# Aster32/GAN-DANet

Hardware: AMD Instinct MI355X
Metric: train samples/sec (G+D step) on 256x256 tiles (higher is better)
Workload: dtype bf16; 1 GPU; full G+D train step, 8ch 256x256 -> 1024x1024 tiles, batch 32/GPU (global 32), perceptual=on, SSIM evaluated, AdamW x2; survey_config=3, per_gpu_batch=32, global_batch=32, tile=256, parallelism=dp1

## Files before the change

### gan-danet_amd/_lib.py

```python
from __future__ import annotations

import ctypes as C
import os

HERE = os.path.dirname(os.path.abspath(__file__))
LIB_PATH = os.path.join(HERE, "lib", "libgandanet_hip.so")

PREC_FP32, PREC_BF16, PREC_X3 = 0, 1, 2
PAM_BWD_K64_ATOMIC, PAM_BWD_K64_PARTS, PAM_BWD_K32_PARTS, PAM_BWD_TWO_KERNEL = 0, 1, 2, 3
ACT_NONE, ACT_RELU, ACT_LEAKY02, ACT_SIGMOID = 0, 1, 2, 3

c_fp = C.c_void_p


class ConvDesc(C.Structure):
    _fields_ = [
        ("B", C.c_int), ("M", C.c_int), ("Mstore", C.c_int), ("Ck", C.c_int), ("ks", C.c_int),
        ("stride", C.c_int), ("pad", C.c_int), ("transposed", C.c_int),
        ("Hi", C.c_int), ("Wi", C.c_int), ("Ho", C.c_int), ("Wo", C.c_int),
        ("a", c_fp), ("a_bs", C.c_long), ("a_sm", C.c_long), ("a_sc", C.c_long), ("a_st", C.c_long),
        ("x", c_fp), ("x_bs", C.c_long),
        ("in_scale", c_fp), ("in_shift", c_fp), ("in_relu", C.c_int),
        ("y", c_fp), ("y_bs", C.c_long),
        ("out_layout", C.c_int), ("out_bf16", C.c_int), ("ldo", C.c_int),
        ("alpha", c_fp), ("bias", c_fp), ("res", c_fp), ("res_bs", C.c_long),
        ("act", C.c_int), ("accumulate", C.c_int), ("precision", C.c_int),
        ("sub_oy", C.c_int), ("sub_ox", C.c_int), ("sub_step", C.c_int),
    ]


class GemmNTDesc(C.Structure):
    _fields_ = [
        ("B", C.c_int), ("M", C.c_int), ("N", C.c_int), ("kseg", C.c_int), ("klen", C.c_long),
        ("a", c_fp), ("a_bs", C.c_long), ("a_ss", C.c_long), ("lda", C.c_long),
        ("bm", c_fp), ("b_bs", C.c_long), ("b_ss", C.c_long), ("ldb", C.c_long),
        ("im2col", C.c_int), ("ks", C.c_int), ("stride", C.c_int), ("pad", C.c_int),
        ("Hi", C.c_int), ("Wi", C.c_int), ("Ho", C.c_int), ("Wo", C.c_int),
        ("in_scale", c_fp), ("in_shift", c_fp), ("in_relu", C.c_int),
        ("c", c_fp), ("c_bs", C.c_long), ("ldc", C.c_long),
        ("alpha", c_fp), ("bias", c_fp),
        ("accumulate", C.c_int), ("splits", C.c_int), ("precision", C.c_int),
    ]


_i, _l, _f, _p, _sz = C.c_int, C.c_long, C.c_float, c_fp, C.c_size_t

SIGNATURES = {
    "gd_version": (_i, []),
    "gd_set_deterministic": (None, [_i]),
    "gd_get_deterministic": (_i, []),
    "gd_set_det_reduce": (_i, [_i]),
    "gd_get_det_reduce": (_i, []),
    "gd_last_error": (_i, [C.c_char_p, _i]),
    "gd_sizeof_conv_desc": (_i, []),
    "gd_sizeof_gemm_nt_desc": (_i, []),
    "gd_conv2d": (_i, [C.POINTER(ConvDesc), _p]),
    "gd_gemm_nt": (_i, [C.POINTER(GemmNTDesc), _p]),
    "gd_gemm_nt_ws": (_i, [C.POINTER(GemmNTDesc), _p, _p, _sz]),
    "gd_gemm_nt_plan": (_i, [C.POINTER(GemmNTDesc), _sz, C.POINTER(_i), C.POINTER(_sz)]),
    "gd_conv3x3_ws_bytes": (_sz, [_i, _i]),
    "gd_conv3x3_eligible": (_i, [C.POINTER(ConvDesc)]),
    "gd_conv3x3": (_i, [C.POINTER(ConvDesc), _p, _sz, _p]),
    "gd_conv3x3_wgrad": (_i, [_p, _l, _p, _p, _l, _p, _i, _p, _p, _i, _i, _i, _i, _i, _i, _i, _i, _p, _p]),
    "gd_conv3x3_wgrad_ws": (_i, [_p, _l, _p, _p, _l, _p, _i, _p, _p, _i, _i, _i, _i, _i, _i, _i, _i, _p, _p, _p, _sz]),
    "gd_conv3x3_wgrad_plan": (_i, [_i, _i, _i, _i, _i, _i, _sz, C.POINTER(_i), C.POINTER(_sz)]),
    "gd_pack_16_split": (_i, [_p, _l, _i, _i, _i, _p, _p, _i, _p, _l, _i, _l, _i, _i, _p, _l, _i, _l, _i, _i, _p]),
    "gd_pack_16_split_masked": (_i, [_p, _l, _i, _i, _i, _p, _p, _i, _p, _l, _i, _l, _i, _i, _p, _l, _i, _l, _i, _i, _p, _l, _p]),
    "gd_split3_weights": (_i, [_p, _l, _l, _l, _p, _p]),
    "gd_bn_stats_ws_floats": (_sz, [_i, _i, _l]),
    "gd_bn_stats": (_i, [_p, _l, _i, _i, _l, _f, _f, _p, _p, _p, _p, _p, _p]),
    "gd_bn_fold": (_i, [_p, _p, _p, _p, _i, _p, _p, _p]),
    "gd_bn_fold_eval": (_i, [_p, _p, _p, _p, _f, _i, _p, _p, _p, _p]),
    "gd_affine_act": (_i, [_p, _l, _p, _p, _i, _i, _l, _i, _p, _l, _p]),
    "gd_bn_act_bwd": (_i, [_p, _l, _p, _l, _p, _p, _p, _p, _p, _i, _i, _l, _i, _i, _p, _p, _p, _l, _i, _p, _p]),
    "gd_bn_stats_local": (_i, [_p, _l, _i, _i, _l, _p, _p, _p]),
    "gd_bn_stats_merge": (_i, [_p, _i, _i, _f, _f, _p, _p, _p, _p, _p]),
    "gd_bn_act_bwd_dx": (_i, [_p, _l, _p, _l, _p, _p, _p, _p, _p, _p, _f, _i, _i, _l, _i, _p, _l, _i, _p]),
    "gd_bicubic_fwd": (_i, [_p, _i, _i, _i, _p, _i, _i, _f, _f, _p]),
    "gd_bicubic_bwd": (_i, [_p, _i, _i, _i, _p, _i, _i, _f, _f, _p]),
    "gd_bilinear_fwd": (_i, [_p, _i, _i, _i, _p, _i, _i, _i, _p, _p]),
    "gd_bilinear_bwd": (_i, [_p, _i, _i, _i, _p, _i, _i, _p]),
    "gd_maxpool2_fwd": (_i, [_p, _i, _i, _i, _p, _p]),
    "gd_maxpool2_bwd": (_i, [_p, _p, _i, _i, _i, _p, _p]),
    "gd_act_fwd": (_i, [_p, _p, _l, _i, _p]),
    "gd_act_bwd": (_i, [_p, _p, _p, _l, _i, _p]),
    "gd_axpby": (_i, [_p, _f, _p, _f, _l, _p]),
    "gd_scale_dev": (_i, [_p, _p, _p, _l, _i, _p]),
    "gd_copy_rows": (_i, [_p, _l, _l, _p, _l, _l, _i, _i, _i, _p]),
    "gd_channel_sum": (_i, [_p, _l, _i, _i, _l, _p, _i, _p, _p]),
    "gd_copy_slab": (_i, [_p, _l, _p, _l, _i, _l, _i, _p]),
    "gd_softmax_rows": (_i, [_p, _p, _l, _i, _f, _p]),
    "gd_softmax_rows_bwd": (_i, [_p, _p, _p, _l, _i, _f, _p]),
    "gd_dot": (_i, [_p, _p, _l, _p, _i, _p, _p]),
    "gd_transpose": (_i, [_p, _p, _i, _i, _i, _p]),
    "gd_add_transpose": (_i, [_p, _p, _i, _i, _p]),
    "gd_bce_logits": (_i, [_p, _l, _f, _p, _p, _p, _p]),
    "gd_bce_logits_target": (_i, [_p, _p, _l, _p, _p, _p, _p, _p]),
    "gd_leaky_fwd": (_i, [_p, _p, _l, _f, _p]),
    "gd_leaky_bwd": (_i, [_p, _p, _p, _l, _f, _p]),
    "gd_mse": (_i, [_p, _p, _l, _p, _p, _p, _p]),
    "gd_l1": (_i, [_p, _p, _l, _p, _p, _p, _p]),
    "gd_tv": (_i, [_p, _i, _i, _i, _i, _f, _p, _p, _p, _p]),
    "gd_ssim": (_i, [_p, _p, _i, _i, _i, _i, _p, _p, _p]),
    "gd_ssim_samples": (_i, [_p, _p, _i, _i, _i, _i, _i, _p, _p, _p]),
    "gd_ssim_bwd": (_i, [_p, _p, _p, _i, _i, _i, _i, _i, _p, _p, _p, _p]),
    "gd_adamw": (_i, [_p, _p, _p, _p, _l, _i, _f, _f, _f, _f, _f, _f, _p]),
    "gd_pam_flash_fwd": (_i, [_p, _p, _p, _i, _i, _i, _i, _i, _i, _i, _p, _p, _l, _p, _l, _p, _p, _p, _p]),
    "gd_pam_key_sqnorm_max": (_i, [_p, _i, _i, _i, _i, _p, _p]),
    "gd_pam_fwd_shift_ws_bytes": (_sz, [_i, _i]),
    "gd_pam_flash_fwd_shift": (_i, [_p, _p, _p, _i, _i, _i, _i, _i, _i, _p, _p, _l, _p, _l, _p, _p, _i, _p, _sz, _p]),
    "gd_pam_flash_bwd": (_i, [_p, _p, _p, _p, _p, _p, _p, _i, _i, _i, _i, _i, _i, _p, _p, _p, _l, _p, _sz, _p]),
    "gd_pam_bwd_scratch_bytes": (_sz, [_i, _i]),
    "gd_pam_wide_fwd": (_i, [_p, _p, _p, _i, _i, _i, _i, _i, _i, _i, _p, _p, _l, _p, _l, _p, _p, _p]),
    "gd_pam_wide_scratch_bytes": (_sz, [_i, _i, _i]),
    "gd_pam_wide_bwd": (_i, [_p, _p, _p, _p, _p, _p, _p, _i, _i, _i, _i, _i, _i, _i, _p, _p, _p, _p, _sz, _p]),
    "gd_pam_f32_fwd": (_i, [_p, _l, _p, _l, _p, _l, _i, _i, _i, _i, _i, _p, _p, _l, _p, _l, _p, _p, _p]),
    "gd_pam_f32_bwd": (_i, [_p, _l, _p, _l, _p, _l, _p, _l, _p, _p, _i, _i, _i, _i, _i, _p, _p, _p, _p]),
    "gd_chan_dot": (_i, [_p, _l, _p, _l, _i, _i, _i, _p, _p, _p, _p]),
    "gd_pam_f16_scale": (_i, [_p, _l, _i, _i, _i, _p, _p, _p, _p, _p]),
    "gd_conv3x3_nhwc_pack": (_i, [_p, _i, _i, _i, _p, _sz, _p]),
    "gd_conv3x3_nhwc": (_i, [_p, _p, _p, _p, _p, _p, _i, _i, _i, _i, _i, _i, _i, _p]),
    "gd_conv3x3_nhwc_f32out": (_i, [_p, _p, _p, _p, _l, _i, _i, _i, _i, _i, _i, _p]),
    "gd_disc_stem_fwd": (_i, [_p, _i, _i, _i, _i, _p, _p, _i, _f, _p, _i, _p]),
    "gd_disc_stem_wgrad": (_i, [_p, _p, _i, _i, _i, _i, _i, _p, _p, _i, _p]),
    "gd_disc_stem_wgrad_ws": (_i, [_p, _p, _i, _i, _i, _i, _i, _p, _p, _i, _p, _p, _sz]),
    "gd_disc_stem_dgrad": (_i, [_p, _i, _i, _i, _i, _p, _i, _p, _i, _p]),
    "gd_conv3x3_nhwc_s2": (_i, [_p, _p, _p, _p, _i, _i, _i, _i, _i, _i, _f, _i, _p]),
    "gd_conv3x3_nhwc_s2_dgrad": (_i, [_p, _p, _p, _f, _p, _i, _i, _i, _i, _i, _i, _p]),
    "gd_nhwc_flatten_fwd": (_i, [_p, _i, _i, _i, _p, _i, _p]),
    "gd_nhwc_flatten_bwd": (_i, [_p, _p, _f, _i, _i, _i, _p, _i, _p]),
    "gd_nhwc_to_nchw16": (_i, [_p, _i, _i, _i, _p, _p, _i, _p]),
    "gd_nhwc_to_nchw16_ws": (_i, [_p, _i, _i, _i, _p, _p, _i, _p, _p, _sz]),
    "gd_nhwc_stem_fwd": (_i, [_p, _i, _i, _i, _i, _p, _p, _i, _i, _p, _i, _p]),
    "gd_nhwc_stem_bwd": (_i, [_p, _i, _i, _i, _i, _p, _i, _p, _i, _p]),
    "gd_nhwc_maxpool2_fwd": (_i, [_p, _i, _i, _i, _i, _p, _i, _p]),
    "gd_nhwc_maxpool2_bwd": (_i, [_p, _p, _i, _i, _i, _i, _i, _p, _i, _p]),
    "gd_nhwc_l1": (_i, [_p, _p, _l, _p, _i, _p, _i, _p]),
    "gd_nhwc_l1_grad": (_i, [_p, _p, _l, _p, _i, _p, _i, _p]),
    "gd_shift_sum9_fwd": (_i, [_p, _p, _p, _i, _i, _i, _p]),
    "gd_shift_sum9_bwd": (_i, [_p, _p, _i, _i, _i, _p]),
    "gd_combine_inputs": (_i, [_p, _i, _i, _i, _f, _p, _i, _i, _i, _f, _p, _i, _i, _i, _p]),
    "gd_hist_match_ws_bytes": (_sz, [_l, _l]),
    "gd_hist_match": (_i, [_p, _p, _i, _l, _l, C.c_double, _p, _p, _sz, _p]),
    "gd_blend_region": (_i, [_p, _p, _p, _i, _i, _i, _i, _i, _i, _i, _p]),
    "gd_augment_d4": (_i, [_p, _p, _i, _i, _i, _i, _p, _p, _f, _p]),
    "gd_bcast_mul": (_i, [_p, _p, _p, _i, _i, _l, _i, _p]),
    "gd_row_dot": (_i, [_p, _p, _p, _l, _l, _p]),
    "gd_chan_maxmean_fwd": (_i, [_p, _p, _p, _i, _i, _l, _p]),
    "gd_chan_maxmean_bwd": (_i, [_p, _p, _p, _i, _i, _l, _p]),
    "gd_comm_unique_id": (_i, [C.c_char_p]),
    "gd_comm_init": (_i, [_i, _i, C.c_char_p]),
    "gd_comm_world": (_i, []),
    "gd_allreduce": (_i, [_p, _sz, _i, _p]),
    "gd_reduce_scatter": (_i, [_p, _p, _sz, _i, _p]),
    "gd_allgather": (_i, [_p, _p, _sz, _i, _p]),
    "gd_comm_destroy": (_i, []),
    "gd_pack_bf16": (_i, [_p, _l, _i, _i, _i, _p, _f, _p, _i, _i, _p, _i, _i, _i, _i, _p]),
    "gd_pack_16": (_i, [_p, _l, _i, _i, _i, _p, _f, _p, _i, _i, _p, _i, _i, _i, _i, _i, _p]),
    "gd_pack_16_affine": (_i, [_p, _l, _i, _i, _i, _p, _p, _i, _p, _i, _i, _p, _i, _i, _i, _p]),
}

_lib = None


class GandanetError(RuntimeError):
    pass


def load() -> C.CDLL:
    global _lib
    if _lib is not None:
        return _lib
    if not os.path.exists(LIB_PATH):
        raise GandanetError(
            f"{LIB_PATH} is missing: the HIP extension is not built (run __graft_entry__.build()). "
            "There is no CPU fallback.")
    lib = C.CDLL(LIB_PATH)
    for name, (res, args) in SIGNATURES.items():
        fn = getattr(lib, name)
        fn.restype = res
        fn.argtypes = args
    if lib.gd_sizeof_conv_desc() != C.sizeof(ConvDesc) or lib.gd_sizeof_gemm_nt_desc() != C.sizeof(GemmNTDesc):
        raise GandanetError("descriptor struct layout differs between _lib.py and libgandanet_hip.so")
    _lib = lib
    return lib


def last_error() -> str:
    buf = C.create_string_buffer(512)
    load().gd_last_error(buf, 512)
    return buf.value.decode()


def check(rc: int, what: str = "") -> None:
    if rc != 0:
        raise GandanetError(f"{what or 'gandanet call'} failed (rc={rc}): {last_error()}")
```

### gan-danet_amd/csrc/gemm_conv.hip

```cpp
#include <stdlib.h>

#include <type_traits>

#include "common.h"
#include "tile_mma.h"
#include "../../include/gandanet.h"

namespace {

using gd::TILE_BK;
using gd::TILE_BN;
constexpr int BN = TILE_BN;
constexpr int BK = TILE_BK;

template <int BM, int MODE>
__global__ __launch_bounds__(256) void conv_nn_kernel(const gd_conv_desc d) {
    constexpr bool BF16 = MODE != gd::MODE_F32;
    constexpr bool X3 = MODE == gd::MODE_X3;
    using P = gd::TilePol<MODE>;
    using elem = typename P::elem;
    constexpr int LD = P::LD;
    constexpr int WAVES_N = gd::TileGeom<BM>::WAVES_N;
    constexpr int TM = gd::TileGeom<BM>::TM;
    constexpr int TN = gd::TileGeom<BM>::TN;
    constexpr int KPT_A = BM / 8;
    constexpr int KPT_B = 16;

    __shared__ __attribute__((aligned(16))) elem As[P::PLANES * BM * LD];
    __shared__ __attribute__((aligned(16))) elem Bs[P::PLANES * BN * LD];

    const int tid = threadIdx.x;
    const int lane = tid & 63, wave = tid >> 6;
    const int r = lane & 31, h = lane >> 5;
    const int wm = wave / WAVES_N, wn = wave % WAVES_N;
    const int b = blockIdx.z;
    const int m0 = blockIdx.y * BM;
    const int n0 = blockIdx.x * BN;
    const long HiWi = (long)d.Hi * d.Wi;
    const int HoWo = d.Ho * d.Wo;

    const int am = tid % BM;
    const int akg = tid / BM;
    const bool a_row_ok = (m0 + am) < d.M;
    const float* a_row = d.a + (long)b * d.a_bs + (long)(m0 + am) * d.a_sm;

    const int bn = tid & (BN - 1);
    const int bkh = tid >> 7;
    const int sstep = d.sub_step > 1 ? d.sub_step : 1;
    const int Ws = (d.Wo - d.sub_ox + sstep - 1) / sstep, Hs = (d.Ho - d.sub_oy + sstep - 1) / sstep;
    const int HsWs = Hs * Ws;
    const int p = n0 + bn;
    const bool p_ok = p < HsWs;
    const int pa = p_ok ? p / Ws : 0;
    const int oy = d.sub_oy + pa * sstep;
    const int ox = d.sub_ox + (p_ok ? p - pa * Ws : 0) * sstep;
    const float* x_img = d.x + (long)b * d.x_bs;

    f32x16_t acc[TM][TN];
#pragma unroll
    for (int i = 0; i < TM; ++i)
#pragma unroll
        for (int j = 0; j < TN; ++j)
#pragma unroll
            for (int e = 0; e < 16; ++e) acc[i][j][e] = 0.f;

    const int ktiles_per_tap = (d.Ck + BK - 1) / BK;
    const int ntaps = d.ks * d.ks;
    const int T = ntaps * ktiles_per_tap;

    float ra[KPT_A];
    float rb[KPT_B];

    auto load_tile = [&](int t) {
        const int tap = t / ktiles_per_tap;
        const int c0 = (t - tap * ktiles_per_tap) * BK;
        const int kh = tap / d.ks, kw = tap - kh * d.ks;
        {
            const float* ap = a_row + (long)tap * d.a_st;
#pragma unroll
            for (int i = 0; i < KPT_A; ++i) {
                const int c = c0 + akg * KPT_A + i;
                ra[i] = (a_row_ok && c < d.Ck) ? ap[(long)c * d.a_sc] : 0.f;
            }
        }
        {
            int iy, ix;
            bool ok = p_ok;
            if (!d.transposed) {
                iy = oy * d.stride - d.pad + kh;
                ix = ox * d.stride - d.pad + kw;
            } else {
                const int ty = oy + d.pad - kh, tx = ox + d.pad - kw;
                ok = ok && ty >= 0 && tx >= 0 && (ty % d.stride == 0) && (tx % d.stride == 0);
                iy = ty / d.stride;
                ix = tx / d.stride;
            }
            ok = ok && iy >= 0 && iy < d.Hi && ix >= 0 && ix < d.Wi;
            const float* xp = x_img + (long)iy * d.Wi + ix;
#pragma unroll
            for (int i = 0; i < KPT_B; ++i) {
                const int c = c0 + bkh * KPT_B + i;
                float v = 0.f;
                if (ok && c < d.Ck) {
                    v = xp[(long)c * HiWi];
                    if (d.in_scale) {
                        v = fmaf(v, d.in_scale[c], d.in_shift[c]);
                        if (d.in_relu) v = fmaxf(v, 0.f);
                    }
                }
                rb[i] = v;
            }
        }
    };

    auto put_row = [&](elem* row, int plane_stride, const float* v, auto nc) {
        constexpr int n = decltype(nc)::value;
        if constexpr (BF16 && n % 8 == 0) {
#pragma unroll
            for (int i = 0; i < n; i += 8) {
                uint4 whi, wlo;
                if constexpr (X3) {
                    gd_split_bf2(v[i + 0], v[i + 1], whi.x, wlo.x);
                    gd_split_bf2(v[i + 2], v[i + 3], whi.y, wlo.y);
                    gd_split_bf2(v[i + 4], v[i + 5], whi.z, wlo.z);
                    gd_split_bf2(v[i + 6], v[i + 7], whi.w, wlo.w);
                    *reinterpret_cast<uint4*>(row + plane_stride + i) = wlo;
                } else {
                    whi.x = gd_pack_bf2(v[i + 0], v[i + 1]);
                    whi.y = gd_pack_bf2(v[i + 2], v[i + 3]);
                    whi.z = gd_pack_bf2(v[i + 4], v[i + 5]);
                    whi.w = gd_pack_bf2(v[i + 6], v[i + 7]);
                }
                *reinterpret_cast<uint4*>(row + i) = whi;
            }
        } else if constexpr (BF16) {
#pragma unroll
            for (int i = 0; i < n; i += 4) {
                uint2 whi, wlo;
                if constexpr (X3) {
                    gd_split_bf2(v[i + 0], v[i + 1], whi.x, wlo.x);
                    gd_split_bf2(v[i + 2], v[i + 3], whi.y, wlo.y);
                    *reinterpret_cast<uint2*>(row + plane_stride + i) = wlo;
                } else {
                    whi.x = gd_pack_bf2(v[i + 0], v[i + 1]);
                    whi.y = gd_pack_bf2(v[i + 2], v[i + 3]);
                }
                *reinterpret_cast<uint2*>(row + i) = whi;
            }
        } else {
#pragma unroll
            for (int i = 0; i < n; ++i) row[i] = v[i];
        }
    };
    auto store_tile = [&]() {
        put_row(As + am * LD + akg * KPT_A, BM * LD, ra, std::integral_constant<int, KPT_A>{});
        put_row(Bs + bn * LD + bkh * KPT_B, BN * LD, rb, std::integral_constant<int, KPT_B>{});
    };

    auto compute_tile = [&]() { gd::tile_mma<BM, MODE>(As, Bs, wm, wn, r, h, acc); };

    auto tile_live = [&](int t) -> bool {
        if (!d.transposed || sstep == 1) return true;
        const int tap = t / ktiles_per_tap;
        const int kh = tap / d.ks, kw = tap - kh * d.ks;
        return ((d.sub_oy + d.pad - kh) % d.stride == 0) && ((d.sub_ox + d.pad - kw) % d.stride == 0);
    };
    auto next_live = [&](int t) -> int {
        while (t < T && !tile_live(t)) ++t;
        return t;
    };
    int t = next_live(0);
    if (t < T) {
        load_tile(t);
        store_tile();
    }
    __syncthreads();
    while (t < T) {
        const int tn = next_live(t + 1);
        if (tn < T) load_tile(tn);
        compute_tile();
        __syncthreads();
        if (tn < T) {
            store_tile();
            __syncthreads();
        }
        t = tn;
    }

    const float alpha = d.alpha ? *d.alpha : 1.f;
#pragma unroll
    for (int i = 0; i < TM; ++i) {
#pragma unroll
        for (int j = 0; j < TN; ++j) {
            const int ps = n0 + wn * TN * 32 + j * 32 + r;
            if (ps >= HsWs) continue;
            const int qa = ps / Ws;
            const int pn = (d.sub_oy + qa * sstep) * d.Wo + d.sub_ox + (ps - qa * Ws) * sstep;
            float rsv[16], oldv[16];
#pragma unroll
            for (int e = 0; e < 16; ++e) {
                const int m = m0 + wm * TM * 32 + i * 32 + gd::acc_row(e, h);
                rsv[e] = (d.res && m < d.M) ? d.res[(long)b * d.res_bs + (long)m * HoWo + pn] : 0.f;
            }
#pragma unroll
            for (int e = 0; e < 16; ++e) {
                const int m = m0 + wm * TM * 32 + i * 32 + gd::acc_row(e, h);
                const long idx = d.out_layout == 0 ? (long)b * d.y_bs + (long)m * HoWo + pn
                                                   : (long)b * d.y_bs + (long)pn * d.ldo + m;
                oldv[e] = (d.accumulate && !d.out_bf16 && m < d.Mstore) ? reinterpret_cast<const float*>(d.y)[idx] : 0.f;
            }
#pragma unroll
            for (int e = 0; e < 16; ++e) {
                const int m = m0 + wm * TM * 32 + i * 32 + gd::acc_row(e, h);
                if (m >= d.Mstore) continue;
                float v = acc[i][j][e] * alpha;
                if (m < d.M) {
                    if (d.bias) v += d.bias[m];
                    v += rsv[e];
                }
                if (d.act == GD_ACT_RELU) v = fmaxf(v, 0.f);
                else if (d.act == GD_ACT_LEAKY02) v = v >= 0.f ? v : 0.2f * v;
                const long idx = d.out_layout == 0 ? (long)b * d.y_bs + (long)m * HoWo + pn
                                                   : (long)b * d.y_bs + (long)pn * d.ldo + m;
                if (d.out_bf16) reinterpret_cast<unsigned short*>(d.y)[idx] = gd_f2bf(v);
                else reinterpret_cast<float*>(d.y)[idx] = v + oldv[e];
            }
        }
    }
}

typedef short s16x4_t __attribute__((ext_vector_type(4)));
constexpr int XLD = BN + 32;

template <int BM, int NS, bool X3 = false>
__global__ __launch_bounds__(256) void conv1x1_tr_kernel(const gd_conv_desc d) {
    constexpr int LDA = BK + 8;
    constexpr int PL = X3 ? 2 : 1, A_PL = BM * LDA, X_PL = NS * BK * XLD;
    constexpr int WAVES_N = gd::TileGeom<BM>::WAVES_N;
    constexpr int TM = gd::TileGeom<BM>::TM;
    constexpr int TN = gd::TileGeom<BM>::TN;
    constexpr int KPT_A = BM / 8;
    __shared__ __attribute__((aligned(16))) unsigned short As[PL * A_PL];
    __shared__ __attribute__((aligned(16))) unsigned short Xs[PL * X_PL];

    const int tid = threadIdx.x, lane = tid & 63, wave = tid >> 6;
    const int r = lane & 31, h = lane >> 5;
    const int wm = wave / WAVES_N, wn = wave % WAVES_N;
    const int b = blockIdx.z, m0 = blockIdx.y * BM, n0 = blockIdx.x * (BN * NS);
    const int HW = d.Ho * d.Wo;

    const int am = tid % BM, akg = tid / BM;
    const bool a_row_ok = (m0 + am) < d.M;
    const float* a_row = d.a + (long)b * d.a_bs + (long)(m0 + am) * d.a_sm;

    const int xq = tid & 31, xr0 = tid >> 5;
    const float* x_img = d.x + (long)b * d.x_bs;

    f32x16_t acc[NS][TM][TN];
#pragma unroll
    for (int sb = 0; sb < NS; ++sb)
#pragma unroll
        for (int i = 0; i < TM; ++i)
#pragma unroll
            for (int j = 0; j < TN; ++j)
#pragma unroll
                for (int e = 0; e < 16; ++e) acc[sb][i][j][e] = 0.f;

    float ra[KPT_A];
    float4 rx[NS][4];
    const int T = (d.Ck + BK - 1) / BK;
    auto load_tile = [&](int t) {
        const int c0 = t * BK;
#pragma unroll
        for (int i = 0; i < KPT_A; ++i) {
            const int c = c0 + akg * KPT_A + i;
            ra[i] = (a_row_ok && c < d.Ck) ? a_row[(long)c * d.a_sc] : 0.f;
        }
#pragma unroll
        for (int i = 0; i < 4; ++i) {
            const int c = c0 + xr0 + 8 * i;
            float sc = 1.f, sh = 0.f;
            if (d.in_scale && c < d.Ck) { sc = d.in_scale[c]; sh = d.in_shift[c]; }
#pragma unroll
            for (int sb = 0; sb < NS; ++sb) {
                const int pq = n0 + sb * BN + xq * 4;
                const bool q_full = pq + 3 < HW;
                float4 v = make_float4(0.f, 0.f, 0.f, 0.f);
                if (c < d.Ck && pq < HW) {
                    const float* p = x_img + (long)c * HW + pq;
                    if (q_full) {
                        v = *reinterpret_cast<const float4*>(p);
                    } else {
                        if (pq + 0 < HW) v.x = p[0];
                        if (pq + 1 < HW) v.y = p[1];
                        if (pq + 2 < HW) v.z = p[2];
                    }
                    if (d.in_scale) {
                        v.x = fmaf(v.x, sc, sh); v.y = fmaf(v.y, sc, sh); v.z = fmaf(v.z, sc, sh); v.w = fmaf(v.w, sc, sh);
                        if (d.in_relu) {
                            v.x = fmaxf(v.x, 0.f); v.y = fmaxf(v.y, 0.f); v.z = fmaxf(v.z, 0.f); v.w = fmaxf(v.w, 0.f);
                        }
                        if (!q_full) {
                            if (pq + 0 >= HW) v.x = 0.f;
                            if (pq + 1 >= HW) v.y = 0.f;
                            if (pq + 2 >= HW) v.z = 0.f;
                            v.w = 0.f;
                        }
                    }
                }
                rx[sb][i] = v;
            }
        }
    };
    auto store_tile = [&]() {
        if constexpr (X3) {
        unsigned short* ap = As + am * LDA + akg * KPT_A;
        if constexpr (KPT_A >= 8) {
#pragma unroll
            for (int i = 0; i < KPT_A; i += 8) {
                uint4 whi, wlo;
                if constexpr (X3) {
                    gd_split_bf2(ra[i + 0], ra[i + 1], whi.x, wlo.x);
                    gd_split_bf2(ra[i + 2], ra[i + 3], whi.y, wlo.y);
                    gd_split_bf2(ra[i + 4], ra[i + 5], whi.z, wlo.z);
                    gd_split_bf2(ra[i + 6], ra[i + 7], whi.w, wlo.w);
                    *reinterpret_cast<uint4*>(ap + A_PL + i) = wlo;
                } else {
                    whi.x = gd_pack_bf2(ra[i + 0], ra[i + 1]);
                    whi.y = gd_pack_bf2(ra[i + 2], ra[i + 3]);
                    whi.z = gd_pack_bf2(ra[i + 4], ra[i + 5]);
                    whi.w = gd_pack_bf2(ra[i + 6], ra[i + 7]);
                }
                *reinterpret_cast<uint4*>(ap + i) = whi;
            }
        } else {
            uint2 whi, wlo;
            if constexpr (X3) {
                gd_split_bf2(ra[0], ra[1], whi.x, wlo.x);
                gd_split_bf2(ra[2], ra[3], whi.y, wlo.y);
                *reinterpret_cast<uint2*>(ap + A_PL) = wlo;
            } else {
                whi.x = gd_pack_bf2(ra[0], ra[1]);
                whi.y = gd_pack_bf2(ra[2], ra[3]);
            }
            *reinterpret_cast<uint2*>(ap) = whi;
        }
#pragma unroll
        for (int sb = 0; sb < NS; ++sb)
#pragma unroll
            for (int i = 0; i < 4; ++i) {
                uint2 whi, wlo;
                unsigned short* xp = Xs + sb * (BK * XLD) + (xr0 + 8 * i) * XLD + xq * 4;
                if constexpr (X3) {
                    gd_split_bf2(rx[sb][i].x, rx[sb][i].y, whi.x, wlo.x);
                    gd_split_bf2(rx[sb][i].z, rx[sb][i].w, whi.y, wlo.y);
                    *reinterpret_cast<uint2*>(xp + X_PL) = wlo;
                } else {
                    whi.x = gd_pack_bf2(rx[sb][i].x, rx[sb][i].y);
                    whi.y = gd_pack_bf2(rx[sb][i].z, rx[sb][i].w);
                }
                *reinterpret_cast<uint2*>(xp) = whi;
            }
        } else {
        unsigned short* ap = As + am * LDA + akg * KPT_A;
        if constexpr (KPT_A >= 8) {
#pragma unroll
            for (int i = 0; i < KPT_A; i += 8) {
                uint4 w;
                w.x = gd_pack_bf2(ra[i + 0], ra[i + 1]);
                w.y = gd_pack_bf2(ra[i + 2], ra[i + 3]);
                w.z = gd_pack_bf2(ra[i + 4], ra[i + 5]);
                w.w = gd_pack_bf2(ra[i + 6], ra[i + 7]);
                *reinterpret_cast<uint4*>(ap + i) = w;
            }
        } else {
            uint2 w;
            w.x = gd_pack_bf2(ra[0], ra[1]);
            w.y = gd_pack_bf2(ra[2], ra[3]);
            *reinterpret_cast<uint2*>(ap) = w;
        }
#pragma unroll
        for (int sb = 0; sb < NS; ++sb)
#pragma unroll
            for (int i = 0; i < 4; ++i) {
                uint2 w;
                w.x = gd_pack_bf2(rx[sb][i].x, rx[sb][i].y);
                w.y = gd_pack_bf2(rx[sb][i].z, rx[sb][i].w);
                *reinterpret_cast<uint2*>(Xs + sb * (BK * XLD) + (xr0 + 8 * i) * XLD + xq * 4) = w;
            }
        }
    };
    const int li = lane & 15, tq = li >> 2, tp = li & 3, tg = (lane >> 4) & 1;
    auto mma = [&](f32x16_t& c, const bf16x8_t& a, const bf16x8_t& bb) {
        c = __builtin_amdgcn_mfma_f32_32x32x16_bf16(__builtin_bit_cast(gd::bf16x8_native_t, a),
                                                    __builtin_bit_cast(gd::bf16x8_native_t, bb), c, 0, 0, 0);
    };
    auto compute_tile = [&]() {
        if constexpr (X3) {
#pragma unroll
        for (int ks = 0; ks < BK / 16; ++ks) {
            bf16x8_t fa[PL][TM];
#pragma unroll
            for (int pl = 0; pl < PL; ++pl)
#pragma unroll
                for (int i = 0; i < TM; ++i)
                    fa[pl][i] = *reinterpret_cast<const bf16x8_t*>(As + pl * A_PL + (wm * TM * 32 + i * 32 + r) * LDA + ks * 16 + 8 * h);
#pragma unroll
            for (int sb = 0; sb < NS; ++sb) {
                bf16x8_t fb[PL][TN];
#pragma unroll
                for (int pl = 0; pl < PL; ++pl)
#pragma unroll
                    for (int j = 0; j < TN; ++j) {
                        const unsigned short* p = Xs + pl * X_PL + sb * (BK * XLD) + (ks * 16 + 8 * h + tq) * XLD + (wn * TN + j) * 32 + 16 * tg + 4 * tp;
                        const s16x4_t lo = __builtin_amdgcn_ds_read_tr16_b64_v4i16((__attribute__((address_space(3))) s16x4_t*)p);
                        const s16x4_t hi = __builtin_amdgcn_ds_read_tr16_b64_v4i16(
                            (__attribute__((address_space(3))) s16x4_t*)(p + 4 * XLD));
                        fb[pl][j] = bf16x8_t{lo.x, lo.y, lo.z, lo.w, hi.x, hi.y, hi.z, hi.w};
                    }
#pragma unroll
                for (int i = 0; i < TM; ++i)
#pragma unroll
                    for (int j = 0; j < TN; ++j) {
                        if constexpr (X3) {
                            mma(acc[sb][i][j], fa[1][i], fb[0][j]);
                            mma(acc[sb][i][j], fa[0][i], fb[1][j]);
                        }
                        mma(acc[sb][i][j], fa[0][i], fb[0][j]);
                    }
            }
        }
        } else {
#pragma unroll
        for (int ks = 0; ks < BK / 16; ++ks) {
            bf16x8_t fa[TM];
#pragma unroll
            for (int i = 0; i < TM; ++i)
                fa[i] = *reinterpret_cast<const bf16x8_t*>(As + (wm * TM * 32 + i * 32 + r) * LDA + ks * 16 + 8 * h);
#pragma unroll
            for (int sb = 0; sb < NS; ++sb) {
                bf16x8_t fb[TN];
#pragma unroll
                for (int j = 0; j < TN; ++j) {
                    const unsigned short* p = Xs + sb * (BK * XLD) + (ks * 16 + 8 * h + tq) * XLD + (wn * TN + j) * 32 + 16 * tg + 4 * tp;
                    const s16x4_t lo = __builtin_amdgcn_ds_read_tr16_b64_v4i16((__attribute__((address_space(3))) s16x4_t*)p);
                    const s16x4_t hi = __builtin_amdgcn_ds_read_tr16_b64_v4i16(
                        (__attribute__((address_space(3))) s16x4_t*)(p + 4 * XLD));
                    fb[j] = bf16x8_t{lo.x, lo.y, lo.z, lo.w, hi.x, hi.y, hi.z, hi.w};
                }
#pragma unroll
                for (int i = 0; i < TM; ++i)
#pragma unroll
                    for (int j = 0; j < TN; ++j)
                        acc[sb][i][j] = __builtin_amdgcn_mfma_f32_32x32x16_bf16(
                            __builtin_bit_cast(gd::bf16x8_native_t, fa[i]), __builtin_bit_cast(gd::bf16x8_native_t, fb[j]),
                            acc[sb][i][j], 0, 0, 0);
            }
        }
        }
    };

    load_tile(0);
    store_tile();
    __syncthreads();
    for (int t = 0; t < T; ++t) {
        if (t + 1 < T) load_tile(t + 1);
        compute_tile();
        __syncthreads();
        if (t + 1 < T) {
            store_tile();
            __syncthreads();
        }
    }

    const float alpha = d.alpha ? *d.alpha : 1.f;
#pragma unroll
    for (int sb = 0; sb < NS; ++sb)
#pragma unroll
    for (int i = 0; i < TM; ++i)
#pragma unroll
        for (int j = 0; j < TN; ++j) {
            const int pn = n0 + sb * BN + wn * TN * 32 + j * 32 + r;
            if (pn >= HW) continue;
            float rsv[16], oldv[16];
#pragma unroll
            for (int e = 0; e < 16; ++e) {
                const int m = m0 + wm * TM * 32 + i * 32 + gd::acc_row(e, h);
                rsv[e] = (d.res && m < d.M) ? d.res[(long)b * d.res_bs + (long)m * HW + pn] : 0.f;
            }
#pragma unroll
            for (int e = 0; e < 16; ++e) {
                const int m = m0 + wm * TM * 32 + i * 32 + gd::acc_row(e, h);
                oldv[e] = (d.accumulate && m < d.M) ? reinterpret_cast<const float*>(d.y)[(long)b * d.y_bs + (long)m * HW + pn] : 0.f;
            }
#pragma unroll
            for (int e = 0; e < 16; ++e) {
                const int m = m0 + wm * TM * 32 + i * 32 + gd::acc_row(e, h);
                if (m >= d.M) continue;
                float v = acc[sb][i][j][e] * alpha + rsv[e];
                if (d.bias) v += d.bias[m];
                if (d.act == GD_ACT_RELU) v = fmaxf(v, 0.f);
                else if (d.act == GD_ACT_LEAKY02) v = v >= 0.f ? v : 0.2f * v;
                reinterpret_cast<float*>(d.y)[(long)b * d.y_bs + (long)m * HW + pn] = v + oldv[e];
            }
        }
}

template <int BM, bool X3 = false>
__global__ __launch_bounds__(256) void conv1x1_tr_plain_kernel(const gd_conv_desc d) {
    constexpr int LDA = BK + 8;
    constexpr int A_PL = BM * LDA, X_PL = BK * XLD;
    constexpr int WAVES_N = gd::TileGeom<BM>::WAVES_N;
    constexpr int TM = gd::TileGeom<BM>::TM;
    constexpr int TN = gd::TileGeom<BM>::TN;
    constexpr int KPT_A = BM / 8;
    __shared__ __attribute__((aligned(16))) unsigned short As[(X3 ? 2 : 1) * BM * LDA];
    __shared__ __attribute__((aligned(16))) unsigned short Xs[(X3 ? 2 : 1) * BK * XLD];

    const int tid = threadIdx.x, lane = tid & 63, wave = tid >> 6;
    const int r = lane & 31, h = lane >> 5;
    const int wm = wave / WAVES_N, wn = wave % WAVES_N;
    const int b = blockIdx.z, m0 = blockIdx.y * BM, n0 = blockIdx.x * BN;
    const int HW = d.Ho * d.Wo;

    const int am = tid % BM, akg = tid / BM;
    const bool a_row_ok = (m0 + am) < d.M;
    const float* a_row = d.a + (long)b * d.a_bs + (long)(m0 + am) * d.a_sm;

    const int xq = tid & 31, xr0 = tid >> 5;
    const float* x_img = d.x + (long)b * d.x_bs;
    const int pq = n0 + xq * 4;
    const bool q_full = pq + 3 < HW;

    f32x16_t acc[TM][TN];
#pragma unroll
    for (int i = 0; i < TM; ++i)
#pragma unroll
        for (int j = 0; j < TN; ++j)
#pragma unroll
            for (int e = 0; e < 16; ++e) acc[i][j][e] = 0.f;

    float ra[KPT_A];
    float4 rx[4];
    const int T = (d.Ck + BK - 1) / BK;
    auto load_tile = [&](int t) {
        const int c0 = t * BK;
#pragma unroll
        for (int i = 0; i < KPT_A; ++i) {
            const int c = c0 + akg * KPT_A + i;
            ra[i] = (a_row_ok && c < d.Ck) ? a_row[(long)c * d.a_sc] : 0.f;
        }
#pragma unroll
        for (int i = 0; i < 4; ++i) {
            const int c = c0 + xr0 + 8 * i;
            float4 v = make_float4(0.f, 0.f, 0.f, 0.f);
            if (c < d.Ck) {
                const float* p = x_img + (long)c * HW + pq;
                if (q_full) {
                    v = *reinterpret_cast<const float4*>(p);
                } else {
                    if (pq + 0 < HW) v.x = p[0];
                    if (pq + 1 < HW) v.y = p[1];
                    if (pq + 2 < HW) v.z = p[2];
                }
                if (d.in_scale) {
                    const float sc = d.in_scale[c], sh = d.in_shift[c];
                    v.x = fmaf(v.x, sc, sh); v.y = fmaf(v.y, sc, sh); v.z = fmaf(v.z, sc, sh); v.w = fmaf(v.w, sc, sh);
                    if (d.in_relu) {
                        v.x = fmaxf(v.x, 0.f); v.y = fmaxf(v.y, 0.f); v.z = fmaxf(v.z, 0.f); v.w = fmaxf(v.w, 0.f);
                    }
                    if (!q_full) {
                        if (pq + 0 >= HW) v.x = 0.f;
                        if (pq + 1 >= HW) v.y = 0.f;
                        if (pq + 2 >= HW) v.z = 0.f;
                        v.w = 0.f;
                    }
                }
            }
            rx[i] = v;
        }
    };
    auto store_tile = [&]() {
        unsigned short* ap = As + am * LDA + akg * KPT_A;
        if constexpr (X3) {
#pragma unroll
            for (int i = 0; i < KPT_A; i += 4) {
                uint2 whi, wlo;
                gd_split_bf2(ra[i + 0], ra[i + 1], whi.x, wlo.x);
                gd_split_bf2(ra[i + 2], ra[i + 3], whi.y, wlo.y);
                *reinterpret_cast<uint2*>(ap + i) = whi;
                *reinterpret_cast<uint2*>(ap + A_PL + i) = wlo;
            }
#pragma unroll
            for (int i = 0; i < 4; ++i) {
                uint2 whi, wlo;
                gd_split_bf2(rx[i].x, rx[i].y, whi.x, wlo.x);
                gd_split_bf2(rx[i].z, rx[i].w, whi.y, wlo.y);
                *reinterpret_cast<uint2*>(Xs + (xr0 + 8 * i) * XLD + xq * 4) = whi;
                *reinterpret_cast<uint2*>(Xs + X_PL + (xr0 + 8 * i) * XLD + xq * 4) = wlo;
            }
            return;
        }
        if constexpr (KPT_A >= 8) {
#pragma unroll
            for (int i = 0; i < KPT_A; i += 8) {
                uint4 w;
                w.x = gd_pack_bf2(ra[i + 0], ra[i + 1]);
                w.y = gd_pack_bf2(ra[i + 2], ra[i + 3]);
                w.z = gd_pack_bf2(ra[i + 4], ra[i + 5]);
                w.w = gd_pack_bf2(ra[i + 6], ra[i + 7]);
                *reinterpret_cast<uint4*>(ap + i) = w;
            }
        } else {
            uint2 w;
            w.x = gd_pack_bf2(ra[0], ra[1]);
            w.y = gd_pack_bf2(ra[2], ra[3]);
            *reinterpret_cast<uint2*>(ap) = w;
        }
#pragma unroll
        for (int i = 0; i < 4; ++i) {
            uint2 w;
            w.x = gd_pack_bf2(rx[i].x, rx[i].y);
            w.y = gd_pack_bf2(rx[i].z, rx[i].w);
            *reinterpret_cast<uint2*>(Xs + (xr0 + 8 * i) * XLD + xq * 4) = w;
        }
    };
    const int li = lane & 15, tq = li >> 2, tp = li & 3, tg = (lane >> 4) & 1;
    auto compute_tile = [&]() {
        if constexpr (X3) {
#pragma unroll
            for (int ks = 0; ks < BK / 16; ++ks) {
                bf16x8_t fa[2][TM], fb[2][TN];
#pragma unroll
                for (int pl = 0; pl < 2; ++pl) {
#pragma unroll
                    for (int i = 0; i < TM; ++i)
                        fa[pl][i] = *reinterpret_cast<const bf16x8_t*>(As + pl * A_PL + (wm * TM * 32 + i * 32 + r) * LDA + ks * 16 + 8 * h);
#pragma unroll
                    for (int j = 0; j < TN; ++j) {
                        const unsigned short* p = Xs + pl * X_PL + (ks * 16 + 8 * h + tq) * XLD + (wn * TN + j) * 32 + 16 * tg + 4 * tp;
                        const s16x4_t lo = __builtin_amdgcn_ds_read_tr16_b64_v4i16((__attribute__((address_space(3))) s16x4_t*)p);
                        const s16x4_t hi = __builtin_amdgcn_ds_read_tr16_b64_v4i16(
                            (__attribute__((address_space(3))) s16x4_t*)(p + 4 * XLD));
                        fb[pl][j] = bf16x8_t{lo.x, lo.y, lo.z, lo.w, hi.x, hi.y, hi.z, hi.w};
                    }
                }
#pragma unroll
                for (int i = 0; i < TM; ++i)
#pragma unroll
                    for (int j = 0; j < TN; ++j) {
                        acc[i][j] = __builtin_amdgcn_mfma_f32_32x32x16_bf16(__builtin_bit_cast(gd::bf16x8_native_t, fa[1][i]),
                                                                           __builtin_bit_cast(gd::bf16x8_native_t, fb[0][j]), acc[i][j], 0, 0, 0);
                        acc[i][j] = __builtin_amdgcn_mfma_f32_32x32x16_bf16(__builtin_bit_cast(gd::bf16x8_native_t, fa[0][i]),
                                                                           __builtin_bit_cast(gd::bf16x8_native_t, fb[1][j]), acc[i][j], 0, 0, 0);
                        acc[i][j] = __builtin_amdgcn_mfma_f32_32x32x16_bf16(__builtin_bit_cast(gd::bf16x8_native_t, fa[0][i]),
                                                                           __builtin_bit_cast(gd::bf16x8_native_t, fb[0][j]), acc[i][j], 0, 0, 0);
                    }
            }
            return;
        }
#pragma unroll
        for (int ks = 0; ks < BK / 16; ++ks) {
            bf16x8_t fa[TM], fb[TN];
#pragma unroll
            for (int i = 0; i < TM; ++i)
                fa[i] = *reinterpret_cast<const bf16x8_t*>(As + (wm * TM * 32 + i * 32 + r) * LDA + ks * 16 + 8 * h);
#pragma unroll
            for (int j = 0; j < TN; ++j) {
                const unsigned short* p = Xs + (ks * 16 + 8 * h + tq) * XLD + (wn * TN + j) * 32 + 16 * tg + 4 * tp;
                const s16x4_t lo = __builtin_amdgcn_ds_read_tr16_b64_v4i16((__attribute__((address_space(3))) s16x4_t*)p);
                const s16x4_t hi = __builtin_amdgcn_ds_read_tr16_b64_v4i16(
                    (__attribute__((address_space(3))) s16x4_t*)(p + 4 * XLD));
                fb[j] = bf16x8_t{lo.x, lo.y, lo.z, lo.w, hi.x, hi.y, hi.z, hi.w};
            }
#pragma unroll
            for (int i = 0; i < TM; ++i)
#pragma unroll
                for (int j = 0; j < TN; ++j)
                    acc[i][j] = __builtin_amdgcn_mfma_f32_32x32x16_bf16(
                        __builtin_bit_cast(gd::bf16x8_native_t, fa[i]), __builtin_bit_cast(gd::bf16x8_native_t, fb[j]),
                        acc[i][j], 0, 0, 0);
        }
    };

    load_tile(0);
    store_tile();
    __syncthreads();
    for (int t = 0; t < T; ++t) {
        if (t + 1 < T) load_tile(t + 1);
        compute_tile();
        __syncthreads();
        if (t + 1 < T) {
            store_tile();
            __syncthreads();
        }
    }

    const float alpha = d.alpha ? *d.alpha : 1.f;
#pragma unroll
    for (int i = 0; i < TM; ++i)
#pragma unroll
        for (int j = 0; j < TN; ++j) {
            const int pn = n0 + wn * TN * 32 + j * 32 + r;
            if (pn >= HW) continue;
            float rsv[16], oldv[16];
#pragma unroll
            for (int e = 0; e < 16; ++e) {
                const int m = m0 + wm * TM * 32 + i * 32 + gd::acc_row(e, h);
                rsv[e] = (d.res && m < d.M) ? d.res[(long)b * d.res_bs + (long)m * HW + pn] : 0.f;
            }
#pragma unroll
            for (int e = 0; e < 16; ++e) {
                const int m = m0 + wm * TM * 32 + i * 32 + gd::acc_row(e, h);
                oldv[e] = (d.accumulate && m < d.M) ? reinterpret_cast<const float*>(d.y)[(long)b * d.y_bs + (long)m * HW + pn] : 0.f;
            }
#pragma unroll
            for (int e = 0; e < 16; ++e) {
                const int m = m0 + wm * TM * 32 + i * 32 + gd::acc_row(e, h);
                if (m >= d.M) continue;
                float v = acc[i][j][e] * alpha + rsv[e];
                if (d.bias) v += d.bias[m];
                if (d.act == GD_ACT_RELU) v = fmaxf(v, 0.f);
                else if (d.act == GD_ACT_LEAKY02) v = v >= 0.f ? v : 0.2f * v;
                reinterpret_cast<float*>(d.y)[(long)b * d.y_bs + (long)m * HW + pn] = v + oldv[e];
            }
        }
}

static bool conv1x1_tr_eligible(const gd_conv_desc& d) {
    const long HW = (long)d.Ho * d.Wo;
    return d.ks == 1 && d.stride == 1 && d.pad == 0 && (d.precision == GD_PREC_BF16 || d.precision == GD_PREC_X3) && d.out_layout == 0 && !d.out_bf16 &&
           (d.Mstore == 0 || d.Mstore == d.M) && d.Hi == d.Ho && d.Wi == d.Wo && HW % 4 == 0 && d.x_bs % 4 == 0 &&
           ((uintptr_t)d.x % 16) == 0;
}

template <int BM>
int launch(const gd_conv_desc& d, hipStream_t s) {
    const int sstep = d.sub_step > 1 ? d.sub_step : 1;
    const long hs = (d.Ho - d.sub_oy + sstep - 1) / sstep, ws = (d.Wo - d.sub_ox + sstep - 1) / sstep;
    if (hs <= 0 || ws <= 0) return 0;
    dim3 grid(gd_cdiv(hs * ws, BN), gd_cdiv(d.Mstore, BM), d.B);
    if (d.precision == GD_PREC_BF16)
        hipLaunchKernelGGL((conv_nn_kernel<BM, gd::MODE_BF16>), grid, dim3(256), 0, s, d);
    else if (d.precision == GD_PREC_X3)
        hipLaunchKernelGGL((conv_nn_kernel<BM, gd::MODE_X3>), grid, dim3(256), 0, s, d);
    else
        hipLaunchKernelGGL((conv_nn_kernel<BM, gd::MODE_F32>), grid, dim3(256), 0, s, d);
    GD_LAUNCH_CHECK();
    return 0;
}

}

extern "C" int gd_conv2d(const gd_conv_desc* dp, void* stream) {
    GD_CHECK_ARG(dp != nullptr, "gd_conv2d: null descriptor");
    gd_conv_desc d = *dp;
    if (d.Mstore < d.M) d.Mstore = d.M;
    GD_CHECK_ARG(d.B > 0 && d.M > 0 && d.Ck > 0 && d.ks > 0 && d.stride > 0 && d.pad >= 0, "gd_conv2d: bad sizes");
    GD_CHECK_ARG(d.Hi > 0 && d.Wi > 0 && d.Ho > 0 && d.Wo > 0, "gd_conv2d: bad spatial sizes");
    GD_CHECK_ARG(d.a && d.x && d.y, "gd_conv2d: null tensor");
    GD_CHECK_ARG((d.in_scale == nullptr) == (d.in_shift == nullptr), "gd_conv2d: in_scale/in_shift must come together");
    GD_CHECK_ARG(d.precision == GD_PREC_FP32 || d.precision == GD_PREC_BF16 || d.precision == GD_PREC_X3, "gd_conv2d: bad precision");
    GD_CHECK_ARG(d.out_layout == 0 || (d.out_layout == 1 && d.ldo >= d.Mstore), "gd_conv2d: bad output layout");
    GD_CHECK_ARG(!(d.out_bf16 && d.accumulate), "gd_conv2d: accumulate needs an fp32 output");
    GD_CHECK_ARG((long)d.Ho * d.Wo < (1L << 31) && d.B <= 65535, "gd_conv2d: image too large for one launch");
    GD_CHECK_ARG(d.sub_step >= 0 && d.sub_oy >= 0 && d.sub_ox >= 0 && (d.sub_step > 1 || (d.sub_oy == 0 && d.sub_ox == 0)),
                 "gd_conv2d: bad output sub-lattice");
    if (!d.transposed) {
        GD_CHECK_ARG((d.Hi + 2 * d.pad - d.ks) / d.stride + 1 == d.Ho && (d.Wi + 2 * d.pad - d.ks) / d.stride + 1 == d.Wo,
                     "gd_conv2d: Ho/Wo do not match Hi/Wi, ks, stride, pad");
    } else {
        GD_CHECK_ARG((d.Ho + 2 * d.pad - d.ks) / d.stride + 1 == d.Hi && (d.Wo + 2 * d.pad - d.ks) / d.stride + 1 == d.Wi,
                     "gd_conv2d: transposed geometry mismatch");
    }
    hipStream_t s = (hipStream_t)stream;
    static const int tr_env = getenv("GD_CONV1X1_TR") ? atoi(getenv("GD_CONV1X1_TR")) : 1;
    if (tr_env && conv1x1_tr_eligible(d)) {
        const int bm = d.M <= 32 ? 32 : (d.M <= 64 || (d.M % 128 != 0 && d.M % 128 <= 64)) ? 64 : 128;
        static const int ns_env = getenv("GD_CONV1X1_NS") ? atoi(getenv("GD_CONV1X1_NS")) : 1;
        const long HWl = (long)d.Ho * d.Wo;
        int ns = (HWl * d.B >= (1L << 18) && d.precision == GD_PREC_BF16) ? ns_env : 1;
        if (bm == 128 && ns > 2) ns = 2;
        if (ns != 1 && ns != 2 && ns != 4) ns = 1;
        dim3 grid(gd_cdiv(HWl, BN * ns), gd_cdiv(d.M, bm), d.B);
#define GD_C1X1(BM_, NS_) hipLaunchKernelGGL((conv1x1_tr_kernel<BM_, NS_>), grid, dim3(256), 0, s, d)
        if (d.precision == GD_PREC_X3) {
            if (bm == 32) hipLaunchKernelGGL((conv1x1_tr_plain_kernel<32, true>), grid, dim3(256), 0, s, d);
            else if (bm == 64) hipLaunchKernelGGL((conv1x1_tr_plain_kernel<64, true>), grid, dim3(256), 0, s, d);
            else hipLaunchKernelGGL((conv1x1_tr_plain_kernel<128, true>), grid, dim3(256), 0, s, d);
        } else if (ns == 1) {
            if (bm == 32) hipLaunchKernelGGL((conv1x1_tr_plain_kernel<32>), grid, dim3(256), 0, s, d);
            else if (bm == 64) hipLaunchKernelGGL((conv1x1_tr_plain_kernel<64>), grid, dim3(256), 0, s, d);
            else hipLaunchKernelGGL((conv1x1_tr_plain_kernel<128>), grid, dim3(256), 0, s, d);
        } else
        if (bm == 32) { if (ns == 4) GD_C1X1(32, 4); else if (ns == 2) GD_C1X1(32, 2); else GD_C1X1(32, 1); }
        else if (bm == 64) { if (ns == 4) GD_C1X1(64, 4); else if (ns == 2) GD_C1X1(64, 2); else GD_C1X1(64, 1); }
        else { if (ns == 2) GD_C1X1(128, 2); else GD_C1X1(128, 1); }
#undef GD_C1X1
        GD_LAUNCH_CHECK();
        return 0;
    }
    auto run = [&](const gd_conv_desc& dd) -> int {
        if (dd.Mstore <= 32) return launch<32>(dd, s);
        if (dd.Mstore <= 64 || (dd.Mstore % 128 != 0 && dd.Mstore % 128 <= 64)) return launch<64>(dd, s);
        return launch<128>(dd, s);
    };
    if (d.transposed && d.stride > 1 && d.sub_step <= 1) {
        for (int py = 0; py < d.stride; ++py)
            for (int px = 0; px < d.stride; ++px) {
                gd_conv_desc dd = d;
                dd.sub_oy = py; dd.sub_ox = px; dd.sub_step = d.stride;
                const int rc = run(dd);
                if (rc) return rc;
            }
        return 0;
    }
    return run(d);
}
```

### gan-danet_amd/csrc/pointwise.hip

```cpp
#include "common.h"
#include "../../include/gandanet.h"

#include <math.h>

namespace {

constexpr int RED_BLOCKS = 1024;

static inline int grid_for(long n, int per_block = 256 * 4) {
    long g = (n + per_block - 1) / per_block;
    if (g < 1) g = 1;
    if (g > 8192) g = 8192;
    return (int)g;
}

__device__ __forceinline__ float act_f(float v, int act) {
    if (act == GD_ACT_RELU) return fmaxf(v, 0.f);
    if (act == GD_ACT_LEAKY02) return v >= 0.f ? v : 0.2f * v;
    if (act == GD_ACT_SIGMOID) return 1.f / (1.f + __expf(-v));
    return v;
}

__global__ void act_fwd_kernel(const float* __restrict__ x, float* __restrict__ y, long n, int act) {
    for (long i = (long)blockIdx.x * blockDim.x + threadIdx.x; i < n; i += (long)gridDim.x * blockDim.x)
// ... 272 lines not shown
                    const float a = row_scale[r], sh = row_shift[r];
                    v.x = fmaf(v.x, a, sh); v.y = fmaf(v.y, a, sh); v.z = fmaf(v.z, a, sh); v.w = fmaf(v.w, a, sh);
                }
                if (relu) { v.x = fmaxf(v.x, 0.f); v.y = fmaxf(v.y, 0.f); v.z = fmaxf(v.z, 0.f); v.w = fmaxf(v.w, 0.f); }
                if (mp) {
                    const float4 m = *reinterpret_cast<const float4*>(mp + (long)r * Cc + c);
                    v.x = m.x > 0.f ? v.x : 0.f; v.y = m.y > 0.f ? v.y : 0.f; v.z = m.z > 0.f ? v.z : 0.f; v.w = m.w > 0.f ? v.w : 0.f;
                }
            }
            uint2 hi;
            hi.x = gd_pack_bf2(v.x, v.y);
            hi.y = gd_pack_bf2(v.z, v.w);
            uint2 lo;
            lo.x = gd_pack_bf2(v.x - gd_bf2f((unsigned short)(hi.x & 0xFFFFu)), v.y - gd_bf2f((unsigned short)(hi.x >> 16)));
            lo.y = gd_pack_bf2(v.z - gd_bf2f((unsigned short)(hi.y & 0xFFFFu)), v.w - gd_bf2f((unsigned short)(hi.y >> 16)));
            *reinterpret_cast<uint2*>(tile[0] + rl * TLD + cg) = hi;
            *reinterpret_cast<uint2*>(tile[1] + rl * TLD + cg) = lo;
        }
    }
    __syncthreads();
    if (plain) {
#pragma unroll
        for (int kk = 0; kk < 2; ++kk) {
            const int it = tid + 256 * kk;
            const int rl = it >> 3, g = it & 7;
            const int r = r0 + rl, c = c0 + 8 * g;
            if (r < R && c < ldp) {
                for (int j = 0; j < p_n; ++j) {
                    const uint4 o = *reinterpret_cast<const uint4*>(tile[(p_pat >> j) & 1] + rl * TLD + 8 * g);
                    *reinterpret_cast<uint4*>(plain + (long)j * p_cs + (long)b * p_bs + (long)r * ldp + c) = o;
                }
            }
        }
    }
    if (tr) {
#pragma unroll
        for (int kk = 0; kk < 2; ++kk) {
            const int it = tid + 256 * kk;
            const int cl = it >> 3, rg = (it & 7) * 8;
            const int c = c0 + cl, r = r0 + rg;
            if (c < Cc && r < R) {
                for (int j = 0; j < t_n; ++j) {
                    const unsigned short* tl = tile[(t_pat >> j) & 1];
                    unsigned int w[4];
#pragma unroll
                    for (int q = 0; q < 4; ++q)
                        w[q] = (unsigned int)tl[(rg + 2 * q) * TLD + cl] | ((unsigned int)tl[(rg + 2 * q + 1) * TLD + cl] << 16);
                    *reinterpret_cast<uint4*>(tr + (long)j * t_cs + (long)b * t_bs + (long)c * ldt + r) = make_uint4(w[0], w[1], w[2], w[3]);
                }
            }
        }
    }
}
__global__ __launch_bounds__(256) void split3_weights_kernel(const float* __restrict__ w, long A, long Bn, long Cn,
                                                            float* __restrict__ out) {
    const long total = A * Bn * Cn;
    for (long i = (long)blockIdx.x * 256 + threadIdx.x; i < total; i += (long)gridDim.x * 256) {
        const long a = i / (Bn * Cn), rem = i - a * (Bn * Cn);
        const float v = w[i];
        const float hi = gd_bf2f((unsigned short)(gd_pack_bf2(v, 0.f) & 0xFFFFu));
        float* o = out + a * 3 * Bn * Cn + rem;
        o[0] = hi;
        o[Bn * Cn] = hi;
        o[2 * Bn * Cn] = v - hi;
    }
}

__global__ void augment_d4_kernel(const float* __restrict__ src, float* __restrict__ dst, int C, int H, int W,
                                  const int* __restrict__ ops, const float* __restrict__ noise, float scale, long total) {
#pragma clang fp contract(off)
    const long plane = (long)H * W;
    for (long i = (long)blockIdx.x * blockDim.x + threadIdx.x; i < total; i += (long)gridDim.x * blockDim.x) {
        const long bc = i / plane;
        const int rem = (int)(i - bc * plane);
        const int op = ops[bc / C];
        const int k = (op >> 2) & 3;
        const int y = rem / W, x = rem - y * W;
        int ry, rx;
        if (k == 0) { ry = y; rx = x; }
        else if (k == 1) { ry = x; rx = W - 1 - y; }
        else if (k == 2) { ry = H - 1 - y; rx = W - 1 - x; }
        else { ry = H - 1 - x; rx = y; }
        if (op & 2) ry = H - 1 - ry;
        if (op & 1) rx = W - 1 - rx;
        float v = src[bc * plane + (long)ry * W + rx];
        if (noise && (op & 16)) v = v + scale * noise[i];
        dst[i] = v;
    }
}

__global__ void bcast_mul_kernel(const float* __restrict__ x, const float* __restrict__ att, float* __restrict__ y, int C,
                                 long HW, int mode, long total) {
    for (long i = (long)blockIdx.x * blockDim.x + threadIdx.x; i < total; i += (long)gridDim.x * blockDim.x) {
        const long bc = i / HW;
        const float a = mode == 0 ? att[bc] : att[(bc / C) * HW + (i - bc * HW)];
        y[i] = x[i] * a;
    }
}
__global__ __launch_bounds__(256) void row_dot_kernel(const float* __restrict__ a, const float* __restrict__ b,
                                                     float* __restrict__ out, long rows, long n) {
    __shared__ float red[4];
    for (long row = blockIdx.x; row < rows; row += gridDim.x) {
        const float* ap = a + row * n;
        const float* bp = b + row * n;
        float s = 0.f;
        for (long j = threadIdx.x; j < n; j += 256) s = fmaf(ap[j], bp[j], s);
        s = gd_block_sum(s, red);
        if (threadIdx.x == 0) out[row] = s;
    }
}
__global__ void chan_maxmean_fwd_kernel(const float* __restrict__ x, float* __restrict__ y, int* __restrict__ idx, int C,
                                        long HW, long total) {
    for (long i = (long)blockIdx.x * blockDim.x + threadIdx.x; i < total; i += (long)gridDim.x * blockDim.x) {
        const long b = i / HW, p = i - b * HW;
        const float* xp = x + b * C * HW + p;
        float mx = xp[0], sum = xp[0];
        int am = 0;
        for (int c = 1; c < C; ++c) {
            const float v = xp[(long)c * HW];
            sum += v;
            if (v > mx) { mx = v; am = c; }
        }
        y[b * 2 * HW + p] = mx;
        y[b * 2 * HW + HW + p] = sum / (float)C;
        idx[i] = am;
    }
}
__global__ void chan_maxmean_bwd_kernel(const float* __restrict__ dy, const int* __restrict__ idx, float* __restrict__ dx,
                                        int C, long HW, long total) {
    const float inv_c = 1.f / (float)C;
    for (long i = (long)blockIdx.x * blockDim.x + threadIdx.x; i < total; i += (long)gridDim.x * blockDim.x) {
        const long bc = i / HW, p = i - bc * HW;
        const long b = bc / C;
        const int c = (int)(bc - b * C);
        const float gmax = dy[b * 2 * HW + p], gmean = dy[b * 2 * HW + HW + p];
        dx[i] = gmean * inv_c + (idx[b * HW + p] == c ? gmax : 0.f);
    }
}

__global__ __launch_bounds__(256) void chan_dot_kernel(const float* __restrict__ a, long a_bs, const float* __restrict__ o,
                                                      long o_bs, int C, int N, const float* __restrict__ gamma,
                                                      float* __restrict__ draw, float* __restrict__ delta) {
    const int b = blockIdx.y;
    const int i = blockIdx.x * 256 + threadIdx.x;
    if (i >= N) return;
    const float* ap = a + (long)b * a_bs + i;
    const float* op = o + (long)b * o_bs + i;
    float s = 0.f;
    for (int c = 0; c < C; ++c) s = fmaf(ap[(long)c * N], op[(long)c * N], s);
    draw[(long)b * N + i] = s;
    delta[(long)b * N + i] = s * (*gamma);
}

__global__ __launch_bounds__(256) void absmax_kernel(const float* __restrict__ a, long a_bs, long chw, float* __restrict__ ws) {
    __shared__ float red[8];
    const float* ap = a + (long)blockIdx.y * a_bs;
    float m = 0.f;
    for (long i = (long)blockIdx.x * 256 + threadIdx.x; i < chw; i += (long)gridDim.x * 256) {
        const float v = fabsf(ap[i]);
        m = v > m ? v : m;
    }
    m = gd_block_max(m, red);
    if (threadIdx.x == 0) ws[blockIdx.y * gridDim.x + blockIdx.x] = m;
}
__global__ __launch_bounds__(256) void f16_scale_kernel(const float* __restrict__ ws, int nparts, const float* __restrict__ gamma,
                                                       float* __restrict__ delta, long n, float* __restrict__ scales) {
    __shared__ float red[8];
    __shared__ float s_up;
    float m = 0.f;
    for (int i = threadIdx.x; i < nparts; i += 256) m = fmaxf(m, ws[i]);
    m = gd_block_max(m, red);
    if (threadIdx.x == 0) {
        const float g = *gamma;
        const float t = m * fabsf(g);
        int e = 0;
        if (t > 0.f && t < 3.0e38f) frexpf(t, &e);
        e = e > 100 ? 100 : (e < -100 ? -100 : e);
        s_up = ldexpf(1.f, -e);
        if (blockIdx.x == 0) {
            scales[0] = g * s_up;
            scales[1] = ldexpf(1.f, e);
        }
    }
    __syncthreads();
    const float up = s_up;
    for (long i = (long)blockIdx.x * 256 + threadIdx.x; i < n; i += (long)gridDim.x * 256) delta[i] *= up;
}

__global__ __launch_bounds__(256) void bce_kernel(const float* __restrict__ z, long n, float label, float inv_n,
                                                 float* __restrict__ dz, float* __restrict__ ws) {
    __shared__ float red[8];
    float s = 0.f;
    for (long i = (long)blockIdx.x * 256 + threadIdx.x; i < n; i += (long)gridDim.x * 256) {
        const float v = z[i];
        s += fmaxf(v, 0.f) - v * label + log1pf(expf(-fabsf(v)));
        if (dz) dz[i] = (1.f / (1.f + expf(-v)) - label) * inv_n;
    }
    s = gd_block_sum(s, red);
    if (threadIdx.x == 0) ws[blockIdx.x] = s;
}
__global__ __launch_bounds__(256) void bce_target_kernel(const float* __restrict__ z, const float* __restrict__ t, long n,
                                                        float inv_n, float* __restrict__ dz, float* __restrict__ dt,
                                                        float* __restrict__ ws) {
    __shared__ float red[8];
    float s = 0.f;
    for (long i = (long)blockIdx.x * 256 + threadIdx.x; i < n; i += (long)gridDim.x * 256) {
        const float v = z[i], y = t[i];
        s += fmaxf(v, 0.f) - v * y + log1pf(expf(-fabsf(v)));
        if (dz) dz[i] = (1.f / (1.f + expf(-v)) - y) * inv_n;
        if (dt) dt[i] = -v * inv_n;
    }
    s = gd_block_sum(s, red);
    if (threadIdx.x == 0) ws[blockIdx.x] = s;
}
__global__ void leaky_fwd_kernel(const float* __restrict__ x, float* __restrict__ y, long n, float slope) {
    for (long i = (long)blockIdx.x * blockDim.x + threadIdx.x; i < n; i += (long)gridDim.x * blockDim.x) {
        const float v = x[i];
        y[i] = v >= 0.f ? v : slope * v;
    }
}
__global__ void leaky_bwd_kernel(const float* __restrict__ x, const float* __restrict__ dy, float* __restrict__ dx, long n,
                                 float slope) {
    for (long i = (long)blockIdx.x * blockDim.x + threadIdx.x; i < n; i += (long)gridDim.x * blockDim.x)
        dx[i] = x[i] >= 0.f ? dy[i] : slope * dy[i];
}
template <bool L1>
__global__ __launch_bounds__(256) void diff_loss_kernel(const float* __restrict__ a, const float* __restrict__ b, long n,
                                                       float inv_n, float* __restrict__ da, float* __restrict__ ws) {
    __shared__ float red[8];
    float s = 0.f;
    for (long i = (long)blockIdx.x * 256 + threadIdx.x; i < n; i += (long)gridDim.x * 256) {
        const float dv = a[i] - b[i];
        if (L1) {
            s += fabsf(dv);
            if (da) da[i] = dv > 0.f ? inv_n : (dv < 0.f ? -inv_n : 0.f);
        } else {
            s = fmaf(dv, dv, s);
            if (da) da[i] = 2.f * dv * inv_n;
        }
    }
    s = gd_block_sum(s, red);
    if (threadIdx.x == 0) ws[blockIdx.x] = s;
}
__global__ __launch_bounds__(256) void tv_kernel(const float* __restrict__ x, long planes, int H, int W, float kh, float kw,
                                                float* __restrict__ dx, float* __restrict__ ws_h, float* __restrict__ ws_w) {
    __shared__ float red[8];
    const long total = planes * H * W;
    float sh = 0.f, sw = 0.f;
    for (long i = (long)blockIdx.x * 256 + threadIdx.x; i < total; i += (long)gridDim.x * 256) {
        const int xx = (int)(i % W);
        const int yy = (int)((i / W) % H);
        const float v = x[i];
        float g = 0.f;
        if (yy + 1 < H) { const float d = x[i + W] - v; sh = fmaf(d, d, sh); g -= 2.f * kh * d; }
        if (yy > 0) { const float d = v - x[i - W]; g += 2.f * kh * d; }
        if (xx + 1 < W) { const float d = x[i + 1] - v; sw = fmaf(d, d, sw); g -= 2.f * kw * d; }
        if (xx > 0) { const float d = v - x[i - 1]; g += 2.f * kw * d; }
        if (dx) dx[i] = g;
    }
    sh = gd_block_sum(sh, red);
    sw = gd_block_sum(sw, red);
    if (threadIdx.x == 0) { ws_h[blockIdx.x] = sh; ws_w[blockIdx.x] = sw; }
}
__global__ __launch_bounds__(256) void tv_final_kernel(const float* __restrict__ ws_h, const float* __restrict__ ws_w,
                                                      int nparts, float kh, float kw, float* __restrict__ out) {
    __shared__ double redd[8];
    double a = 0, b = 0;
    for (int i = threadIdx.x; i < nparts; i += 256) { a += ws_h[i]; b += ws_w[i]; }
    a = gd_wave_sum_d(a);
    b = gd_wave_sum_d(b);
    if ((threadIdx.x & 63) == 0) { redd[threadIdx.x >> 6] = a; redd[4 + (threadIdx.x >> 6)] = b; }
    __syncthreads();
    if (threadIdx.x == 0)
        out[0] = (float)((redd[0] + redd[1] + redd[2] + redd[3]) * (double)kh + (redd[4] + redd[5] + redd[6] + redd[7]) * (double)kw);
}

struct SsimWin { float g[16]; int n; };
__global__ __launch_bounds__(256) void ssim_kernel(const float* __restrict__ a, const float* __restrict__ b, int H, int W,
                                                  SsimWin win, float* __restrict__ ws) {
    __shared__ float red[8];
    const long plane = blockIdx.y;
    const float* pa = a + plane * (long)H * W;
    const float* pb = b + plane * (long)H * W;
    const int half = win.n / 2;
    float s = 0.f;
    for (long i = (long)blockIdx.x * 256 + threadIdx.x; i < (long)H * W; i += (long)gridDim.x * 256) {
        const int yy = (int)(i / W), xx = (int)(i - (long)yy * W);
        float m1 = 0, m2 = 0, s11 = 0, s22 = 0, s12 = 0;
        for (int dy = 0; dy < win.n; ++dy) {
            const int y2 = yy + dy - half;
            if (y2 < 0 || y2 >= H) continue;
            for (int dx = 0; dx < win.n; ++dx) {
                const int x2 = xx + dx - half;
                if (x2 < 0 || x2 >= W) continue;
                const float w = win.g[dy] * win.g[dx];
                const float u = pa[(long)y2 * W + x2], v = pb[(long)y2 * W + x2];
                m1 = fmaf(w, u, m1); m2 = fmaf(w, v, m2);
                s11 = fmaf(w, u * u, s11); s22 = fmaf(w, v * v, s22); s12 = fmaf(w, u * v, s12);
            }
        }
        const float c1 = 0.01f * 0.01f, c2 = 0.03f * 0.03f;
        const float m1s = m1 * m1, m2s = m2 * m2, m12 = m1 * m2;
        const float v1 = s11 - m1s, v2 = s22 - m2s, v12 = s12 - m12;
        s += ((2.f * m12 + c1) * (2.f * v12 + c2)) / ((m1s + m2s + c1) * (v1 + v2 + c2));
    }
    s = gd_block_sum(s, red);
// ... 161 lines not shown
    hipLaunchKernelGGL(softmax_rows_bwd_kernel, dim3((unsigned)rows), dim3(256), 0, GD_S, p, dp, dx, cols, sign);
    GD_LAUNCH_CHECK();
    return 0;
}
extern "C" int gd_dot(const float* a, const float* b, long n, float* out, int accumulate, float* ws, void* stream) {
    GD_CHECK_ARG(a && out && ws && n > 0, "gd_dot: bad arguments");
    const int g = grid_for(n) > RED_BLOCKS ? RED_BLOCKS : grid_for(n);
    hipLaunchKernelGGL(dot_kernel, dim3(g), dim3(256), 0, GD_S, a, b, n, ws);
    hipLaunchKernelGGL(reduce_final_kernel, dim3(1), dim3(256), 0, GD_S, ws, g, 1.f, out, accumulate);
    GD_LAUNCH_CHECK();
    return 0;
}
extern "C" int gd_transpose(const float* s, float* t, int B, int R, int Cc, void* stream) {
    GD_CHECK_ARG(s && t && B > 0 && B <= 65535 && R > 0 && Cc > 0, "gd_transpose: bad arguments");
    GD_CHECK_ARG(gd_cdiv(R, 32) <= 65535, "gd_transpose: too many rows");
    hipLaunchKernelGGL(transpose_kernel, dim3(gd_cdiv(Cc, 32), gd_cdiv(R, 32), B), dim3(256), 0, GD_S, s, t, R, Cc);
    GD_LAUNCH_CHECK();
    return 0;
}
extern "C" int gd_add_transpose(const float* a, float* out, int B, int n, void* stream) {
    GD_CHECK_ARG(a && out && a != out && B > 0 && B <= 65535 && n > 0, "gd_add_transpose: bad arguments");
    hipLaunchKernelGGL(add_transpose_kernel, dim3(grid_for((long)n * n), B), dim3(256), 0, GD_S, a, out, n);
    GD_LAUNCH_CHECK();
    return 0;
}
extern "C" int gd_pack_16(const float* s, long s_bs, int B, int R, int Cc, const float* scale_dev, float scale_imm,
                          void* plain, int Rp_plain, int ld_plain, void* transposed, int Ccp_t, int ld_t, int perm16,
                          int ones_row, int f16, void* stream) {
    GD_CHECK_ARG(s && (plain || transposed) && B > 0 && B <= 65535 && R > 0 && Cc > 0, "gd_pack_16: bad arguments");
    GD_CHECK_ARG(!plain || (Rp_plain >= R && ld_plain >= Cc), "gd_pack_16: plain padding smaller than the data");
    GD_CHECK_ARG(!perm16 || (plain && ld_plain % 16 == 0), "gd_pack_16: perm16 needs a plain output with ld % 16 == 0");
    GD_CHECK_ARG(!transposed || (Ccp_t >= Cc && ld_t >= R), "gd_pack_16: transposed padding smaller than the data");
    GD_CHECK_ARG(ones_row < 0 || (ones_row >= R && (!plain || ones_row < Rp_plain) && (!transposed || ones_row < ld_t)),
                 "gd_pack_16: ones_row must be a padding row");
    int rows = R, cols = Cc;
    if (plain) { rows = rows > Rp_plain ? rows : Rp_plain; cols = cols > ld_plain ? cols : ld_plain; }
    if (transposed) { rows = rows > ld_t ? rows : ld_t; cols = cols > Ccp_t ? cols : Ccp_t; }
    GD_CHECK_ARG(gd_cdiv(rows, 32) <= 65535, "gd_pack_16: too many rows");
    const bool aligned = Cc % 4 == 0 && s_bs % 4 == 0 && ((uintptr_t)s % 16) == 0 && (!plain || (ld_plain % 8 == 0 && (uintptr_t)plain % 16 == 0)) &&
                         (!transposed || (ld_t % 8 == 0 && (uintptr_t)transposed % 16 == 0));
    if (aligned)
        hipLaunchKernelGGL(pack16_tile64_kernel, dim3(gd_cdiv(cols, 64), gd_cdiv(rows, 64), B), dim3(256), 0, GD_S, s, s_bs, R, Cc,
                           scale_dev, scale_imm, (const float*)nullptr, (const float*)nullptr, 0, (unsigned short*)plain, Rp_plain,
                           ld_plain, (unsigned short*)transposed, Ccp_t, ld_t, perm16, ones_row, f16);
    else
        hipLaunchKernelGGL(pack_bf16_kernel, dim3(gd_cdiv(cols, 32), gd_cdiv(rows, 32), B), dim3(256), 0, GD_S, s, s_bs, R, Cc,
                           scale_dev, scale_imm, (unsigned short*)plain, Rp_plain, ld_plain, (unsigned short*)transposed, Ccp_t,
                           ld_t, perm16, ones_row, f16);
    GD_LAUNCH_CHECK();
    return 0;
}
extern "C" int gd_pack_16_affine(const float* s, long s_bs, int B, int R, int Cc, const float* row_scale, const float* row_shift,
                                 int relu, void* plain, int Rp_plain, int ld_plain, void* transposed, int Ccp_t, int ld_t,
                                 int f16, void* stream) {
    GD_CHECK_ARG(s && (plain || transposed) && B > 0 && B <= 65535 && R > 0 && Cc > 0, "gd_pack_16_affine: bad arguments");
    GD_CHECK_ARG((row_scale == nullptr) == (row_shift == nullptr), "gd_pack_16_affine: row_scale / row_shift come together");
    GD_CHECK_ARG(!plain || (Rp_plain >= R && ld_plain >= Cc), "gd_pack_16_affine: plain padding smaller than the data");
    GD_CHECK_ARG(!transposed || (Ccp_t >= Cc && ld_t >= R), "gd_pack_16_affine: transposed padding smaller than the data");
    GD_CHECK_ARG(Cc % 4 == 0 && s_bs % 4 == 0 && ((uintptr_t)s % 16) == 0 && (!plain || (ld_plain % 8 == 0 && (uintptr_t)plain % 16 == 0)) &&
                     (!transposed || (ld_t % 8 == 0 && (uintptr_t)transposed % 16 == 0)),
                 "gd_pack_16_affine: needs Cc % 4 == 0, leading dimensions % 8 == 0 and 16-byte aligned pointers");
    int rows = R, cols = Cc;
    if (plain) { rows = rows > Rp_plain ? rows : Rp_plain; cols = cols > ld_plain ? cols : ld_plain; }
    if (transposed) { rows = rows > ld_t ? rows : ld_t; cols = cols > Ccp_t ? cols : Ccp_t; }
    GD_CHECK_ARG(gd_cdiv(rows, 64) <= 65535, "gd_pack_16_affine: too many rows");
    hipLaunchKernelGGL(pack16_tile64_kernel, dim3(gd_cdiv(cols, 64), gd_cdiv(rows, 64), B), dim3(256), 0, GD_S, s, s_bs, R, Cc,
                       (const float*)nullptr, 1.f, row_scale, row_shift, relu, (unsigned short*)plain, Rp_plain, ld_plain,
                       (unsigned short*)transposed, Ccp_t, ld_t, 0, -1, f16);
    GD_LAUNCH_CHECK();
    return 0;
}
extern "C" int gd_pack_16_split_masked(const float* s, long s_bs, int B, int R, int Cc, const float* row_scale, const float* row_shift,
                                       int relu, void* plain, long p_bs, int ldp, long p_cs, int p_ncopy, int p_pattern, void* tr,
                                       long t_bs, int ldt, long t_cs, int t_ncopy, int t_pattern, const float* mask, long m_bs,
                                       void* stream) {
    GD_CHECK_ARG(s && (plain || tr) && B > 0 && B <= 65535 && R > 0 && Cc > 0, "gd_pack_16_split: bad arguments");
    GD_CHECK_ARG((row_scale == nullptr) == (row_shift == nullptr), "gd_pack_16_split: row_scale / row_shift come together");
    GD_CHECK_ARG(Cc % 8 == 0 && R % 8 == 0 && s_bs % 4 == 0 && ((uintptr_t)s % 16) == 0, "gd_pack_16_split: R, Cc must be multiples of 8");
    GD_CHECK_ARG(!plain || (ldp == Cc && p_ncopy >= 1 && p_ncopy <= 3 && p_cs % 8 == 0 && p_bs % 8 == 0 && (uintptr_t)plain % 16 == 0),
                 "gd_pack_16_split: plain output needs ldp == Cc, 1..3 copies, 16-byte aligned strides");
    GD_CHECK_ARG(!tr || (ldt >= R && ldt % 8 == 0 && t_ncopy >= 1 && t_ncopy <= 3 && t_cs % 8 == 0 && t_bs % 8 == 0 && (uintptr_t)tr % 16 == 0),
                 "gd_pack_16_split: transposed output needs ldt >= R, ldt % 8 == 0, 1..3 copies, 16-byte aligned strides");
    GD_CHECK_ARG(gd_cdiv(R, 64) <= 65535, "gd_pack_16_split: too many rows");
    GD_CHECK_ARG(!mask || (m_bs % 4 == 0 && ((uintptr_t)mask % 16) == 0), "gd_pack_16_split: mask must be 16-byte aligned");
    hipLaunchKernelGGL(pack16_split_kernel, dim3(gd_cdiv(Cc, 64), gd_cdiv(R, 64), B), dim3(256), 0, GD_S, s, s_bs, R, Cc, row_scale,
                       row_shift, relu, (unsigned short*)plain, p_bs, ldp, p_cs, p_ncopy, p_pattern, (unsigned short*)tr, t_bs, ldt,
                       t_cs, t_ncopy, t_pattern, mask, m_bs);
    GD_LAUNCH_CHECK();
    return 0;
}
extern "C" int gd_pack_16_split(const float* s, long s_bs, int B, int R, int Cc, const float* row_scale, const float* row_shift,
                                int relu, void* plain, long p_bs, int ldp, long p_cs, int p_ncopy, int p_pattern, void* tr,
                                long t_bs, int ldt, long t_cs, int t_ncopy, int t_pattern, void* stream) {
    return gd_pack_16_split_masked(s, s_bs, B, R, Cc, row_scale, row_shift, relu, plain, p_bs, ldp, p_cs, p_ncopy, p_pattern, tr,
                                   t_bs, ldt, t_cs, t_ncopy, t_pattern, nullptr, 0, stream);
}
extern "C" int gd_split3_weights(const float* w, long A, long Bn, long Cn, float* out, void* stream) {
    GD_CHECK_ARG(w && out && A > 0 && Bn > 0 && Cn > 0, "gd_split3_weights: bad arguments");
    const long total = A * Bn * Cn;
    hipLaunchKernelGGL(split3_weights_kernel, dim3(grid_for(total) > 4096 ? 4096 : grid_for(total)), dim3(256), 0, GD_S, w, A, Bn, Cn, out);
    GD_LAUNCH_CHECK();
    return 0;
}
extern "C" int gd_pack_bf16(const float* s, long s_bs, int B, int R, int Cc, const float* scale_dev, float scale_imm,
                            void* plain, int Rp_plain, int ld_plain, void* transposed, int Ccp_t, int ld_t, int perm16,
                            int ones_row, void* stream) {
    return gd_pack_16(s, s_bs, B, R, Cc, scale_dev, scale_imm, plain, Rp_plain, ld_plain, transposed, Ccp_t, ld_t, perm16,
                      ones_row, 0, stream);
}
extern "C" int gd_augment_d4(const float* src, float* dst, int B, int C, int H, int W, const int* ops, const float* noise,
                             float noise_scale, void* stream) {
    GD_CHECK_ARG(src && dst && ops && src != dst && B > 0 && C > 0 && H > 0 && W > 0, "gd_augment_d4: bad arguments");
    const long total = (long)B * C * H * W;
    hipLaunchKernelGGL(augment_d4_kernel, dim3(grid_for(total)), dim3(256), 0, GD_S, src, dst, C, H, W, ops, noise,
                       noise_scale, total);
    GD_LAUNCH_CHECK();
    return 0;
}
extern "C" int gd_bcast_mul(const float* x, const float* att, float* y, int B, int C, long HW, int mode, void* stream) {
    GD_CHECK_ARG(x && att && y && B > 0 && C > 0 && HW > 0 && (mode == 0 || mode == 1), "gd_bcast_mul: bad arguments");
    const long total = (long)B * C * HW;
    hipLaunchKernelGGL(bcast_mul_kernel, dim3(grid_for(total)), dim3(256), 0, GD_S, x, att, y, C, HW, mode, total);
    GD_LAUNCH_CHECK();
    return 0;
}
extern "C" int gd_row_dot(const float* a, const float* b, float* out, long rows, long n, void* stream) {
    GD_CHECK_ARG(a && b && out && rows > 0 && n > 0, "gd_row_dot: bad arguments");
    hipLaunchKernelGGL(row_dot_kernel, dim3((unsigned)(rows < 8192 ? rows : 8192)), dim3(256), 0, GD_S, a, b, out, rows, n);
    GD_LAUNCH_CHECK();
    return 0;
}
extern "C" int gd_chan_maxmean_fwd(const float* x, float* y, int* idx, int B, int C, long HW, void* stream) {
    GD_CHECK_ARG(x && y && idx && B > 0 && C > 0 && HW > 0, "gd_chan_maxmean_fwd: bad arguments");
    const long total = (long)B * HW;
    hipLaunchKernelGGL(chan_maxmean_fwd_kernel, dim3(grid_for(total, 256)), dim3(256), 0, GD_S, x, y, idx, C, HW, total);
    GD_LAUNCH_CHECK();
    return 0;
}
extern "C" int gd_chan_maxmean_bwd(const float* dy, const int* idx, float* dx, int B, int C, long HW, void* stream) {
    GD_CHECK_ARG(dy && idx && dx && B > 0 && C > 0 && HW > 0, "gd_chan_maxmean_bwd: bad arguments");
    const long total = (long)B * C * HW;
    hipLaunchKernelGGL(chan_maxmean_bwd_kernel, dim3(grid_for(total)), dim3(256), 0, GD_S, dy, idx, dx, C, HW, total);
    GD_LAUNCH_CHECK();
    return 0;
}
extern "C" int gd_chan_dot(const float* a, long a_bs, const float* o, long o_bs, int B, int C, int N, const float* gamma,
                           float* d_raw, float* delta, void* stream) {
    GD_CHECK_ARG(a && o && gamma && d_raw && delta && B > 0 && B <= 65535 && C > 0 && N > 0, "gd_chan_dot: bad arguments");
    hipLaunchKernelGGL(chan_dot_kernel, dim3(gd_cdiv(N, 256), B), dim3(256), 0, GD_S, a, a_bs, o, o_bs, C, N, gamma, d_raw,
                       delta);
    GD_LAUNCH_CHECK();
    return 0;
}

extern "C" int gd_pam_f16_scale(const float* dout, long dout_bs, int B, int C, int N, const float* gamma, float* delta,
                                float* scales, float* ws, void* stream) {
    GD_CHECK_ARG(dout && gamma && delta && scales && ws && B > 0 && B <= 65535 && C > 0 && N > 0, "gd_pam_f16_scale: bad arguments");
    const long chw = (long)C * N;
    int g = grid_for(chw);
    g = g > RED_BLOCKS / B ? RED_BLOCKS / B : g;
    g = g < 1 ? 1 : g;
    GD_CHECK_ARG((long)g * B <= RED_BLOCKS, "gd_pam_f16_scale: batch larger than the reduction workspace (1024 parts)");
    hipLaunchKernelGGL(absmax_kernel, dim3(g, B), dim3(256), 0, GD_S, dout, dout_bs, chw, ws);
    const long n = (long)B * N;
    hipLaunchKernelGGL(f16_scale_kernel, dim3(grid_for(n) > 256 ? 256 : grid_for(n)), dim3(256), 0, GD_S, ws, g * B, gamma, delta, n,
                       scales);
    GD_LAUNCH_CHECK();
    return 0;
}

extern "C" int gd_bce_logits(const float* z, long n, float label, float* out, float* dz, float* ws, void* stream) {
    GD_CHECK_ARG(z && out && ws && n > 0, "gd_bce_logits: bad arguments");
    const int g = grid_for(n) > RED_BLOCKS ? RED_BLOCKS : grid_for(n);
    hipLaunchKernelGGL(bce_kernel, dim3(g), dim3(256), 0, GD_S, z, n, label, 1.f / (float)n, dz, ws);
    hipLaunchKernelGGL(reduce_final_kernel, dim3(1), dim3(256), 0, GD_S, ws, g, 1.f / (float)n, out, 0);
    GD_LAUNCH_CHECK();
    return 0;
}
extern "C" int gd_bce_logits_target(const float* z, const float* t, long n, float* out, float* dz, float* dt, float* ws,
                                    void* stream) {
    GD_CHECK_ARG(z && t && out && ws && n > 0, "gd_bce_logits_target: bad arguments");
    const int g = grid_for(n) > RED_BLOCKS ? RED_BLOCKS : grid_for(n);
    hipLaunchKernelGGL(bce_target_kernel, dim3(g), dim3(256), 0, GD_S, z, t, n, 1.f / (float)n, dz, dt, ws);
    hipLaunchKernelGGL(reduce_final_kernel, dim3(1), dim3(256), 0, GD_S, ws, g, 1.f / (float)n, out, 0);
    GD_LAUNCH_CHECK();
    return 0;
}
extern "C" int gd_leaky_fwd(const float* x, float* y, long n, float slope, void* stream) {
    GD_CHECK_ARG(x && y && n > 0, "gd_leaky_fwd: bad arguments");
    hipLaunchKernelGGL(leaky_fwd_kernel, dim3(grid_for(n)), dim3(256), 0, GD_S, x, y, n, slope);
    GD_LAUNCH_CHECK();
    return 0;
}
extern "C" int gd_leaky_bwd(const float* x, const float* dy, float* dx, long n, float slope, void* stream) {
    GD_CHECK_ARG(x && dy && dx && n > 0, "gd_leaky_bwd: bad arguments");
    hipLaunchKernelGGL(leaky_bwd_kernel, dim3(grid_for(n)), dim3(256), 0, GD_S, x, dy, dx, n, slope);
    GD_LAUNCH_CHECK();
    return 0;
}
extern "C" int gd_mse(const float* a, const float* b, long n, float* out, float* da, float* ws, void* stream) {
    GD_CHECK_ARG(a && b && out && ws && n > 0, "gd_mse: bad arguments");
    const int g = grid_for(n) > RED_BLOCKS ? RED_BLOCKS : grid_for(n);
    hipLaunchKernelGGL((diff_loss_kernel<false>), dim3(g), dim3(256), 0, GD_S, a, b, n, 1.f / (float)n, da, ws);
    hipLaunchKernelGGL(reduce_final_kernel, dim3(1), dim3(256), 0, GD_S, ws, g, 1.f / (float)n, out, 0);
    GD_LAUNCH_CHECK();
    return 0;
}
extern "C" int gd_l1(const float* a, const float* b, long n, float* out, float* da, float* ws, void* stream) {
    GD_CHECK_ARG(a && b && out && ws && n > 0, "gd_l1: bad arguments");
    const int g = grid_for(n) > RED_BLOCKS ? RED_BLOCKS : grid_for(n);
    hipLaunchKernelGGL((diff_loss_kernel<true>), dim3(g), dim3(256), 0, GD_S, a, b, n, 1.f / (float)n, da, ws);
    hipLaunchKernelGGL(reduce_final_kernel, dim3(1), dim3(256), 0, GD_S, ws, g, 1.f / (float)n, out, 0);
    GD_LAUNCH_CHECK();
    return 0;
}
extern "C" int gd_tv(const float* x, int B, int C, int H, int W, float weight, float* out, float* dx, float* ws,
                     void* stream) {
    GD_CHECK_ARG(x && out && ws && B > 0 && C > 0 && H > 1 && W > 1, "gd_tv: bad arguments");
    const long planes = (long)B * C;
    const double count_h = (double)planes * (H - 1) * W, count_w = (double)planes * H * (W - 1);
    const float kh = (float)(weight * 2.0 / count_h / B), kw = (float)(weight * 2.0 / count_w / B);
    const long n = planes * H * W;
    const int g = grid_for(n) > RED_BLOCKS ? RED_BLOCKS : grid_for(n);
    hipLaunchKernelGGL(tv_kernel, dim3(g), dim3(256), 0, GD_S, x, planes, H, W, kh, kw, dx, ws, ws + RED_BLOCKS);
    hipLaunchKernelGGL(tv_final_kernel, dim3(1), dim3(256), 0, GD_S, ws, ws + RED_BLOCKS, g, kh, kw, out);
    GD_LAUNCH_CHECK();
    return 0;
}
static int ssim_window(int window, SsimWin* win) {
    if (!(window > 0 && window <= 15 && (window & 1))) return -1;
    win->n = window;
    float tmp[16], sum = 0.f;
    for (int i = 0; i < window; ++i) {
        const float d = (float)(i - window / 2);
        tmp[i] = expf(-(d * d) / (2.f * 1.5f * 1.5f));
        sum += tmp[i];
    }
    for (int i = 0; i < 16; ++i) win->g[i] = i < window ? tmp[i] / sum : 0.f;
    return 0;
}
static int ssim_gx(int H, int W, int BC) {
    int gx = (int)(((long)H * W + 255) / 256);
    if (gx > 64) gx = 64;
    while ((long)gx * BC > 2048 && gx > 1) gx >>= 1;
    return gx;
}
extern "C" int gd_ssim(const float* a, const float* b, int BC, int H, int W, int window, float* out, float* ws,
                       void* stream) {
    GD_CHECK_ARG(a && b && out && ws && BC > 0 && H > 0 && W > 0, "gd_ssim: bad arguments");
    SsimWin win;
    GD_CHECK_ARG(ssim_window(window, &win) == 0, "gd_ssim: window must be odd and <= 15");
    const int gx = ssim_gx(H, W, BC);
    GD_CHECK_ARG((long)gx * BC <= 2048 && BC <= 65535, "gd_ssim: too many planes for the workspace");
    hipLaunchKernelGGL(ssim_kernel, dim3(gx, BC), dim3(256), 0, GD_S, a, b, H, W, win, ws);
    hipLaunchKernelGGL(reduce_final_kernel, dim3(1), dim3(256), 0, GD_S, ws, gx * BC, 1.f / ((float)BC * (float)H * (float)W),
                       out, 0);
    GD_LAUNCH_CHECK();
    return 0;
}
extern "C" int gd_ssim_samples(const float* a, const float* b, int B, int C, int H, int W, int window, float* out,
                               float* ws, void* stream) {
    GD_CHECK_ARG(a && b && out && ws && B > 0 && C > 0 && H > 0 && W > 0, "gd_ssim_samples: bad arguments");
    SsimWin win;
    GD_CHECK_ARG(ssim_window(window, &win) == 0, "gd_ssim_samples: window must be odd and <= 15");
    const int BC = B * C, gx = ssim_gx(H, W, BC);
    GD_CHECK_ARG((long)gx * BC <= 2048 && BC <= 65535, "gd_ssim_samples: too many planes for the workspace");
    hipLaunchKernelGGL(ssim_kernel, dim3(gx, BC), dim3(256), 0, GD_S, a, b, H, W, win, ws);
    hipLaunchKernelGGL(reduce_rows_kernel, dim3(B), dim3(256), 0, GD_S, ws, gx * C, 1.f / ((float)C * (float)H * (float)W), out);
    GD_LAUNCH_CHECK();
    return 0;
}
extern "C" int gd_ssim_bwd(const float* a, const float* b, const float* gscale, int B, int C, int H, int W, int window,
                           float* coef_ws, float* da, float* db, void* stream) {
    GD_CHECK_ARG(a && b && gscale && coef_ws && (da || db) && B > 0 && C > 0 && H > 0 && W > 0, "gd_ssim_bwd: bad arguments");
    SsimWin win;
    GD_CHECK_ARG(ssim_window(window, &win) == 0, "gd_ssim_bwd: window must be odd and <= 15");
    GD_CHECK_ARG((long)B * C <= 65535, "gd_ssim_bwd: too many planes");
    int gx = (int)(((long)H * W + 255) / 256);
    if (gx > 256) gx = 256;
    hipLaunchKernelGGL(ssim_bwd_coef_kernel, dim3(gx, B * C), dim3(256), 0, GD_S, a, b, C, H, W, win, gscale, coef_ws);
    hipLaunchKernelGGL(ssim_bwd_filter_kernel, dim3(gx, B * C), dim3(256), 0, GD_S, a, b, H, W, win, coef_ws, da, db);
    GD_LAUNCH_CHECK();
    return 0;
}
extern "C" int gd_blend_region(float* gen, const float* grace, const float* mask, int BC, int H, int W, int sr, int er,
                               int sc, int ec, void* stream) {
    GD_CHECK_ARG(gen && grace && mask && BC > 0 && H > 0 && W > 0, "gd_blend_region: bad arguments");
    GD_CHECK_ARG(0 <= sr && sr < er && er <= H && 0 <= sc && sc < ec && ec <= W, "gd_blend_region: region outside the image");
    const long total = (long)BC * (er - sr) * (ec - sc);
    hipLaunchKernelGGL(blend_region_kernel, dim3(grid_for(total)), dim3(256), 0, GD_S, gen, grace, mask, H, W, sr, sc, er - sr,
                       ec - sc, total);
    GD_LAUNCH_CHECK();
    return 0;
}
extern "C" int gd_adamw(float* p, const float* g, float* m, float* v, long n, int step, float lr, float beta1,
                        float beta2, float eps, float weight_decay, float grad_scale, void* stream) {
    GD_CHECK_ARG(p && g && m && v && n > 0 && step >= 1, "gd_adamw: bad arguments");
    const double bc1 = 1.0 - pow((double)beta1, step), bc2 = 1.0 - pow((double)beta2, step);
    hipLaunchKernelGGL(adamw_kernel, dim3(grid_for(n)), dim3(256), 0, GD_S, p, g, m, v, n, lr, beta1, beta2, eps,
                       weight_decay, grad_scale, (float)(1.0 / bc1), (float)(1.0 / sqrt(bc2)));
    GD_LAUNCH_CHECK();
    return 0;
}
```

### gan-danet_amd/kern.py

```python
from __future__ import annotations

import ctypes as C
import math
import os
from typing import Optional, Tuple

import torch

from . import _lib as L

Tensor = torch.Tensor


def _stream() -> int:
    return torch.cuda.current_stream().cuda_stream


def _ptr(t: Optional[Tensor]):
    return None if t is None else t.data_ptr()


def _chk(t: Tensor, name: str = "tensor", dtype=torch.float32) -> None:
    if not t.is_cuda:
        raise L.GandanetError(f"{name}: expected a GPU tensor (there is no CPU fallback in the product path)")
    if t.dtype != dtype:
        raise L.GandanetError(f"{name}: expected {dtype}, got {t.dtype}")


def _dense(t: Tensor, name: str = "tensor") -> Tensor:
    _chk(t, name)
    if not t.is_contiguous():
        raise L.GandanetError(f"{name}: expected a contiguous tensor, got strides {t.stride()}")
    return t


def _bview(t: Tensor, name: str = "tensor") -> int:
    _chk(t, name)
    if t.dim() == 4:
        b, c, h, w = t.shape
        ok = t.stride(3) == 1 and t.stride(2) == w and t.stride(1) == h * w
        inner = c * h * w
    elif t.dim() == 3:
        b, c, n = t.shape
        ok = t.stride(2) == 1 and t.stride(1) == n
        inner = c * n
    else:
        raise L.GandanetError(f"{name}: expected a 3-D or 4-D tensor")
    if not ok:
        raise L.GandanetError(f"{name}: per-image block must be dense, got strides {t.stride()}")
    bs = t.stride(0) if b > 1 else inner
    if b > 1 and bs < inner:
        raise L.GandanetError(f"{name}: overlapping batch stride")
    return bs


def lib():
    return L.load()


WGRAD_X_NHWC = os.environ.get("GD_WGRAD_X_NHWC", "1") != "0"
USE_CONV3X3_FAST = True


PROFILE_ON = False
PROFILE_CONV = os.environ.get("GD_PROFILE_CONV", "0") == "1"
PROFILE: list = []


class _Bracket:

    def __init__(self, name: str, flops: float, nbytes: float = 0.0):
        self.name, self.flops, self.nbytes = name, flops, nbytes

    def __enter__(self):
        if PROFILE_ON:
            self.e0 = torch.cuda.Event(enable_timing=True)
            self.e1 = torch.cuda.Event(enable_timing=True)
            self.e0.record()
        return self

    def __exit__(self, *exc):
        if PROFILE_ON:
            self.e1.record()
            PROFILE.append((self.name, self.e0, self.e1, self.flops, self.nbytes))
        return False


class _ConvBracket(_Bracket):

    def __init__(self, kind, k, stride, cin, cout, ho, wo, b):
        super().__init__(f"conv_{kind}_k{k}s{stride}_{cin}->{cout}@{ho}x{wo}", 2.0 * k * k * cin * cout * ho * wo * b)

    def __enter__(self):
        return super().__enter__() if PROFILE_CONV else self

    def __exit__(self, *exc):
        return super().__exit__(*exc) if PROFILE_CONV else False


def profile_summary():
    torch.cuda.synchronize()
    agg = {}
    for name, e0, e1, fl, nb in PROFILE:
        a = agg.setdefault(name, [0, 0.0, 0.0, 0.0])
        a[0] += 1
        a[1] += e0.elapsed_time(e1)
        a[2] += fl
        a[3] += nb
    return {k: (v[0], v[1] / v[0], v[2] / v[0], v[3] / v[0]) for k, v in agg.items()}


def conv_nn(*, B: int, M: int, Ck: int, ks: int, stride: int, pad: int, transposed: bool, Hi: int, Wi: int,
            Ho: int, Wo: int, a: Tensor, a_bs: int, a_sm: int, a_sc: int, a_st: int, x: Tensor, x_bs: int,
            y: Tensor, y_bs: int, precision: int, Mstore: int = 0, in_scale: Optional[Tensor] = None,
            in_shift: Optional[Tensor] = None, in_relu: bool = False, out_layout: int = 0, out_bf16: bool = False,
            ldo: int = 0, alpha: Optional[Tensor] = None, bias: Optional[Tensor] = None,
            res: Optional[Tensor] = None, res_bs: int = 0, act: int = 0, accumulate: bool = False) -> None:
    d = L.ConvDesc()
    d.B, d.M, d.Mstore, d.Ck, d.ks, d.stride, d.pad = B, M, max(M, Mstore), Ck, ks, stride, pad
    d.transposed = int(transposed)
    d.Hi, d.Wi, d.Ho, d.Wo = Hi, Wi, Ho, Wo
    d.a, d.a_bs, d.a_sm, d.a_sc, d.a_st = _ptr(a), a_bs, a_sm, a_sc, a_st
    d.x, d.x_bs = _ptr(x), x_bs
    d.in_scale, d.in_shift, d.in_relu = _ptr(in_scale), _ptr(in_shift), int(in_relu)
    d.y, d.y_bs = _ptr(y), y_bs
    d.out_layout, d.out_bf16, d.ldo = out_layout, int(out_bf16), ldo
    d.alpha, d.bias, d.res, d.res_bs = _ptr(alpha), _ptr(bias), _ptr(res), res_bs
    d.act, d.accumulate, d.precision = act, int(accumulate), precision
    if USE_CONV3X3_FAST and lib().gd_conv3x3_eligible(C.byref(d)):
        nbytes = int(lib().gd_conv3x3_ws_bytes(M, Ck))
        ws = torch.empty(nbytes // 2, device=x.device, dtype=torch.bfloat16)
        L.check(lib().gd_conv3x3(C.byref(d), _ptr(ws), nbytes, _stream()), "gd_conv3x3")
        return
    L.check(lib().gd_conv2d(C.byref(d), _stream()), "gd_conv2d")


def conv_out_size(h: int, k: int, stride: int, pad: int) -> int:
    return (h + 2 * pad - k) // stride + 1


def conv2d_fwd(x: Tensor, w: Tensor, bias: Optional[Tensor], stride: int, pad: int, precision: int, *,
               act: int = 0, out: Optional[Tensor] = None, in_scale=None, in_shift=None, in_relu=False,
               accumulate: bool = False) -> Tensor:
    xbs = _bview(x, "conv input")
    _dense(w, "conv weight")
    B, Cin, Hi, Wi = x.shape
    Cout, Cin_w, k, k2 = w.shape
    if Cin_w != Cin or k != k2:
        raise L.GandanetError(f"conv2d: weight {tuple(w.shape)} does not match input {tuple(x.shape)}")
    Ho, Wo = conv_out_size(Hi, k, stride, pad), conv_out_size(Wi, k, stride, pad)
    if out is None:
        out = torch.empty(B, Cout, Ho, Wo, device=x.device, dtype=torch.float32)
    elif tuple(out.shape) != (B, Cout, Ho, Wo):
        raise L.GandanetError("conv2d: bad out shape")
    with _ConvBracket("fwd", k, stride, Cin, Cout, Ho, Wo, B):
        conv_nn(B=B, M=Cout, Ck=Cin, ks=k, stride=stride, pad=pad, transposed=False, Hi=Hi, Wi=Wi, Ho=Ho, Wo=Wo,
                a=w, a_bs=0, a_sm=Cin * k * k, a_sc=k * k, a_st=1, x=x, x_bs=xbs, y=out, y_bs=_bview(out, "conv out"),
                precision=precision, in_scale=in_scale, in_shift=in_shift, in_relu=in_relu, bias=bias, act=act,
                accumulate=accumulate)
    return out


def conv2d_dgrad(dy: Tensor, w: Tensor, in_hw: Tuple[int, int], stride: int, pad: int, precision: int, *,
                 out: Optional[Tensor] = None, accumulate: bool = False, alpha: Optional[Tensor] = None) -> Tensor:
    dbs = _bview(dy, "conv dy")
    B, Cout, Ho, Wo = dy.shape
    Cout_w, Cin, k, _ = w.shape
    Hi, Wi = in_hw
    if Cout_w != Cout:
        raise L.GandanetError("conv2d_dgrad: weight/out-channel mismatch")
    if out is None:
        out = torch.empty(B, Cin, Hi, Wi, device=dy.device, dtype=torch.float32)
    with _ConvBracket("dgrad", k, stride, Cin, Cout, Ho, Wo, B):
        conv_nn(B=B, M=Cin, Ck=Cout, ks=k, stride=stride, pad=pad, transposed=True, Hi=Ho, Wi=Wo, Ho=Hi, Wo=Wi,
                a=w, a_bs=0, a_sm=k * k, a_sc=Cin * k * k, a_st=1, x=dy, x_bs=dbs, y=out, y_bs=_bview(out, "conv dx"),
                precision=precision, accumulate=accumulate, alpha=alpha)
    return out


def gemm_nt(*, B: int, M: int, N: int, kseg: int, klen: int, a: Tensor, a_bs: int, a_ss: int, lda: int,
            bm: Tensor, b_bs: int, b_ss: int, ldb: int, c: Tensor, c_bs: int, ldc: int, precision: int,
            im2col=None, in_scale=None, in_shift=None, in_relu=False, alpha=None, bias=None,
            accumulate: bool = False, splits: int = 0) -> None:
    d = L.GemmNTDesc()
    d.B, d.M, d.N, d.kseg, d.klen = B, M, N, kseg, klen
    d.a, d.a_bs, d.a_ss, d.lda = _ptr(a), a_bs, a_ss, lda
    d.bm, d.b_bs, d.b_ss, d.ldb = _ptr(bm), b_bs, b_ss, ldb
    if im2col is not None:
        d.im2col = 1
        d.ks, d.stride, d.pad, d.Hi, d.Wi, d.Ho, d.Wo = im2col
    d.in_scale, d.in_shift, d.in_relu = _ptr(in_scale), _ptr(in_shift), int(in_relu)
    d.c, d.c_bs, d.ldc = _ptr(c), c_bs, ldc
    d.alpha, d.bias = _ptr(alpha), _ptr(bias)
    d.accumulate, d.splits, d.precision = int(accumulate), splits, precision
    L.check(lib().gd_gemm_nt_ws(C.byref(d), _stream(), *det_ws()), "gd_gemm_nt")


def conv2d_wgrad(dy: Tensor, x: Tensor, k: int, stride: int, pad: int, precision: int, *, in_scale=None,
                 in_shift=None, in_relu=False, alpha: Optional[Tensor] = None, splits: int = 0) -> Tensor:
    if alpha is not None and not (k == 1 and stride == 1 and pad == 0):
        raise L.GandanetError("conv2d_wgrad: alpha is supported for 1x1 convs only")
    dbs, xbs = _bview(dy, "wgrad dy"), _bview(x, "wgrad x")
    B, Cout, Ho, Wo = dy.shape
    _, Cin, Hi, Wi = x.shape
    dw = torch.empty(Cout, Cin, k, k, device=dy.device, dtype=torch.float32)
    with _ConvBracket("wgrad", k, stride, Cin, Cout, Ho, Wo, B):
        return _conv2d_wgrad(dy, x, k, stride, pad, precision, in_scale, in_shift, in_relu, dw, dbs, xbs, B, Cout, Cin, Hi,
                             Wi, Ho, Wo, alpha, splits)


def _conv2d_wgrad(dy, x, k, stride, pad, precision, in_scale, in_shift, in_relu, dw, dbs, xbs, B, Cout, Cin, Hi, Wi, Ho, Wo,
                  alpha=None, splits=0):
    if USE_CONV3X3_FAST and k == 3 and stride in (1, 2) and pad == 1 and precision == L.PREC_BF16:
        dy16 = x16 = None
        x_ld = 0
        if Cout > 32 and Cin >= 4 * 32:
            dy16, _ = pack_bf16(dy.view(B, Cout, Ho * Wo), Cout, Ho * Wo, plain_shape=(Cout, Ho * Wo))
            if WGRAD_X_NHWC and in_scale is None and x.dim() == 4:
                x_ld = (Cin + 7) // 8 * 8
                _, x16 = pack_bf16(x, Cin, Hi * Wi, t_shape=(Hi * Wi, x_ld))
        L.check(lib().gd_conv3x3_wgrad_ws(_ptr(dy), dbs, _ptr(dy16), _ptr(x), xbs, _ptr(x16), x_ld, _ptr(in_scale),
                                       _ptr(in_shift), int(in_relu), B, Cout, Cin, Hi, Wi, stride, 0, _ptr(dw), _stream(),
                                          *det_ws()), "gd_conv3x3_wgrad")
        return dw
    if k == 1 and stride == 1 and pad == 0:
        gemm_nt(B=1, M=Cout, N=Cin, kseg=B, klen=Ho * Wo, a=dy, a_bs=0, a_ss=dbs, lda=Ho * Wo, bm=x, b_bs=0, b_ss=xbs,
                ldb=Hi * Wi, c=dw, c_bs=0, ldc=Cin, precision=precision, in_scale=in_scale, in_shift=in_shift,
                in_relu=in_relu, alpha=alpha, splits=splits)
        return dw
    gemm_nt(B=1, M=Cout, N=Cin * k * k, kseg=B, klen=Ho * Wo, a=dy, a_bs=0, a_ss=dbs, lda=Ho * Wo, bm=x, b_bs=0,
            b_ss=xbs, ldb=0, c=dw, c_bs=0, ldc=Cin * k * k, precision=precision,
            im2col=(k, stride, pad, Hi, Wi, Ho, Wo), in_scale=in_scale, in_shift=in_shift, in_relu=in_relu)
    return dw


def bn_ws(B: int, Cn: int, HW: int, device) -> Tensor:
    n = lib().gd_bn_stats_ws_floats(B, Cn, HW)
    return torch.empty(max(int(n), 1), device=device, dtype=torch.float32)


def channel_sum(x: Tensor, out: Optional[Tensor] = None, accumulate: bool = False) -> Tensor:
    bs = _bview(x, "channel_sum input")
    B, Cn = x.shape[0], x.shape[1]
    HW = x[0, 0].numel()
    if out is None:
        out = torch.empty(Cn, device=x.device, dtype=torch.float32)
    L.check(lib().gd_channel_sum(_ptr(x), bs, B, Cn, HW, _ptr(out), int(accumulate), _ptr(bn_ws(B, Cn, HW, x.device)),
                                 _stream()), "gd_channel_sum")
    return out


def bn_stats(x: Tensor, eps: float, momentum: float, running_mean: Optional[Tensor],
             running_var: Optional[Tensor]) -> Tuple[Tensor, Tensor]:
    bs = _bview(x, "bn input")
    B, Cn = x.shape[0], x.shape[1]
    HW = x[0, 0].numel()
    mean = torch.empty(Cn, device=x.device, dtype=torch.float32)
    invstd = torch.empty_like(mean)
    L.check(lib().gd_bn_stats(_ptr(x), bs, B, Cn, HW, eps, momentum, _ptr(mean), _ptr(invstd), _ptr(running_mean),
                              _ptr(running_var), _ptr(bn_ws(B, Cn, HW, x.device)), _stream()), "gd_bn_stats")
    return mean, invstd


def bn_stats_local(x: Tensor) -> Tensor:
    bs = _bview(x, "bn input")
    B, Cn = x.shape[0], x.shape[1]
    HW = x[0, 0].numel()
    stats = torch.empty(Cn, 3, device=x.device, dtype=torch.float32)
    L.check(lib().gd_bn_stats_local(_ptr(x), bs, B, Cn, HW, _ptr(stats), _ptr(bn_ws(B, Cn, HW, x.device)), _stream()),
            "gd_bn_stats_local")
    return stats


def bn_stats_merge(stats_all: Tensor, eps: float, momentum: float, running_mean: Optional[Tensor],
                   running_var: Optional[Tensor]) -> Tuple[Tensor, Tensor]:
    _dense(stats_all, "gathered BN records")
    world, Cn, _ = stats_all.shape
    mean = torch.empty(Cn, device=stats_all.device, dtype=torch.float32)
    invstd = torch.empty_like(mean)
    L.check(lib().gd_bn_stats_merge(_ptr(stats_all), world, Cn, eps, momentum, _ptr(mean), _ptr(invstd), _ptr(running_mean),
                                    _ptr(running_var), _stream()), "gd_bn_stats_merge")
# ... 294 lines not shown
def leaky_bwd(x: Tensor, dy: Tensor, slope: float) -> Tensor:
    _dense(x), _dense(dy)
    dx = torch.empty_like(x)
    L.check(lib().gd_leaky_bwd(_ptr(x), _ptr(dy), _ptr(dx), x.numel(), float(slope), _stream()), "gd_leaky_bwd")
    return dx


def diff_loss(kind: str, a: Tensor, b: Tensor, want_grad: bool):
    _dense(a), _dense(b)
    if a.shape != b.shape:
        raise L.GandanetError(f"{kind}: shape mismatch {tuple(a.shape)} vs {tuple(b.shape)}")
    out = torch.empty(1, device=a.device, dtype=torch.float32)
    da = torch.empty_like(a) if want_grad else None
    fn = lib().gd_mse if kind == "mse" else lib().gd_l1
    L.check(fn(_ptr(a), _ptr(b), a.numel(), _ptr(out), _ptr(da), _ptr(_red_ws(a.device)), _stream()), f"gd_{kind}")
    return out, da


def tv(x: Tensor, weight: float, want_grad: bool):
    _dense(x)
    B, Cn, H, W = x.shape
    out = torch.empty(1, device=x.device, dtype=torch.float32)
    dx = torch.empty_like(x) if want_grad else None
    L.check(lib().gd_tv(_ptr(x), B, Cn, H, W, weight, _ptr(out), _ptr(dx), _ptr(_red_ws(x.device)), _stream()), "gd_tv")
    return out, dx


def ssim(a: Tensor, b: Tensor, window: int) -> Tensor:
    _dense(a), _dense(b)
    B, Cn, H, W = a.shape
    out = torch.empty(1, device=a.device, dtype=torch.float32)
    L.check(lib().gd_ssim(_ptr(a), _ptr(b), B * Cn, H, W, window, _ptr(out), _ptr(_red_ws(a.device)), _stream()),
            "gd_ssim")
    return out


def ssim_samples(a: Tensor, b: Tensor, window: int) -> Tensor:
    _dense(a), _dense(b)
    B, Cn, H, W = a.shape
    out = torch.empty(B, device=a.device, dtype=torch.float32)
    L.check(lib().gd_ssim_samples(_ptr(a), _ptr(b), B, Cn, H, W, window, _ptr(out), _ptr(_red_ws(a.device)), _stream()),
            "gd_ssim_samples")
    return out


def ssim_bwd(a: Tensor, b: Tensor, gscale: Tensor, window: int, need_a: bool = True, need_b: bool = True):
    _dense(a), _dense(b), _dense(gscale)
    B, Cn, H, W = a.shape
    coef = torch.empty(4 * a.numel(), device=a.device, dtype=torch.float32)
    da = torch.empty_like(a) if need_a else None
    db = torch.empty_like(b) if need_b else None
    L.check(lib().gd_ssim_bwd(_ptr(a), _ptr(b), _ptr(gscale), B, Cn, H, W, window, _ptr(coef), _ptr(da), _ptr(db),
                              _stream()), "gd_ssim_bwd")
    return da, db


def adamw(p: Tensor, g: Tensor, m: Tensor, v: Tensor, step: int, lr: float, beta1: float, beta2: float, eps: float,
          weight_decay: float, grad_scale: float = 1.0) -> None:
    for t in (p, g, m, v):
        _dense(t, "adamw tensor")
    L.check(lib().gd_adamw(_ptr(p), _ptr(g), _ptr(m), _ptr(v), p.numel(), step, lr, beta1, beta2, eps, weight_decay,
                           grad_scale, _stream()), "gd_adamw")


LOG2E = 1.4426950408889634


def pack_bf16(s: Tensor, R: int, Cc: int, *, scale: Optional[Tensor] = None, scale_imm: float = 1.0, plain_shape=None,
              t_shape=None, perm16: bool = False, ones_row: int = -1, f16: bool = False):
    sbs = _bview(s, "pack input")
    B = s.shape[0]
    plain = tr = None
    rp = ldp = ccp = ldt = 0
    dt = torch.float16 if f16 else torch.bfloat16
    if plain_shape is not None:
        rp, ldp = plain_shape
        plain = torch.empty(B, rp, ldp, device=s.device, dtype=dt)
    if t_shape is not None:
        ccp, ldt = t_shape
        tr = torch.empty(B, ccp, ldt, device=s.device, dtype=dt)
    L.check(lib().gd_pack_16(_ptr(s), sbs, B, R, Cc, _ptr(scale), float(scale_imm), _ptr(plain), rp, ldp, _ptr(tr),
                             ccp, ldt, int(perm16), int(ones_row), int(f16), _stream()), "gd_pack_16")
    return plain, tr


def pack_nhwc16_affine(x: Tensor, scale: Optional[Tensor], shift: Optional[Tensor], relu: bool) -> Tensor:
    sbs = _bview(x, "pack input")
    B, Cn, H, W = x.shape
    out = torch.empty(B, H * W, Cn, device=x.device, dtype=torch.bfloat16)
    L.check(lib().gd_pack_16_affine(_ptr(x), sbs, B, Cn, H * W, _ptr(scale), _ptr(shift), int(relu), None, 0, 0, _ptr(out),
                                    H * W, Cn, 0, _stream()), "gd_pack_16_affine")
    return out


def augment_d4(x: Tensor, ops: Tensor, noise: Optional[Tensor] = None, noise_scale: float = 0.05) -> Tensor:
    _dense(x, "augment input")
    _chk(ops, "augment ops", torch.int32)
    B, Cn, H, W = x.shape
    if ops.numel() != B or (noise is not None and _dense(noise, "noise").shape != x.shape):
        raise L.GandanetError("augment_d4: ops must hold one word per sample and noise must match the batch")
    y = torch.empty_like(x)
    L.check(lib().gd_augment_d4(_ptr(x), _ptr(y), B, Cn, H, W, _ptr(ops), _ptr(noise), float(noise_scale), _stream()),
            "gd_augment_d4")
    return y


def bcast_mul(x: Tensor, att: Tensor, mode: int) -> Tensor:
    _dense(x), _dense(att)
    B, Cn = x.shape[0], x.shape[1]
    HW = x[0, 0].numel()
    if att.numel() != (B * Cn if mode == 0 else B * HW):
        raise L.GandanetError(f"bcast_mul: gate of {att.numel()} elements does not match x {tuple(x.shape)} (mode {mode})")
    y = torch.empty_like(x)
    L.check(lib().gd_bcast_mul(_ptr(x), _ptr(att), _ptr(y), B, Cn, HW, mode, _stream()), "gd_bcast_mul")
    return y


def row_dot(a: Tensor, b: Tensor, rows: int) -> Tensor:
    _dense(a), _dense(b)
    n = a.numel() // rows
    out = torch.empty(rows, device=a.device, dtype=torch.float32)
    L.check(lib().gd_row_dot(_ptr(a), _ptr(b), _ptr(out), rows, n, _stream()), "gd_row_dot")
    return out


def chan_maxmean_fwd(x: Tensor):
    _dense(x)
    B, Cn, H, W = x.shape
    y = torch.empty(B, 2, H, W, device=x.device, dtype=torch.float32)
    idx = torch.empty(B, H * W, device=x.device, dtype=torch.int32)
    L.check(lib().gd_chan_maxmean_fwd(_ptr(x), _ptr(y), _ptr(idx), B, Cn, H * W, _stream()), "gd_chan_maxmean_fwd")
    return y, idx


def chan_maxmean_bwd(dy: Tensor, idx: Tensor, Cn: int) -> Tensor:
    _dense(dy)
    B, _, H, W = dy.shape
    dx = torch.empty(B, Cn, H, W, device=dy.device, dtype=torch.float32)
    L.check(lib().gd_chan_maxmean_bwd(_ptr(dy), _ptr(idx), _ptr(dx), B, Cn, H * W, _stream()), "gd_chan_maxmean_bwd")
    return dx


def chan_dot(a: Tensor, o: Tensor, gamma: Tensor):
    abs_, obs = _bview(a), _bview(o)
    B, Cn = a.shape[0], a.shape[1]
    N = a[0, 0].numel()
    d_raw = torch.empty(B, N, device=a.device, dtype=torch.float32)
    delta = torch.empty_like(d_raw)
    L.check(lib().gd_chan_dot(_ptr(a), abs_, _ptr(o), obs, B, Cn, N, _ptr(gamma), _ptr(d_raw), _ptr(delta), _stream()),
            "gd_chan_dot")
    return d_raw, delta


def pam_f16_scale(dout: Tensor, gamma: Tensor, delta: Tensor) -> Tensor:
    bs = _bview(dout, "dOut")
    B, Cn = dout.shape[0], dout.shape[1]
    N = dout[0, 0].numel()
    scales = torch.empty(2, device=dout.device, dtype=torch.float32)
    L.check(lib().gd_pam_f16_scale(_ptr(dout), bs, B, Cn, N, _ptr(gamma), _ptr(_dense(delta)), _ptr(scales),
                                   _ptr(_red_ws(dout.device)), _stream()), "gd_pam_f16_scale")
    return scales


PAM_NOMAX = os.environ.get("GD_PAM_NOMAX", "1") != "0"


def pam_key_sqnorm_max(kt: Tensor, N: int, f16: bool = False) -> Tensor:
    B, Npad = kt.shape[0], kt.shape[1]
    out = torch.empty(B, device=kt.device, dtype=torch.float32)
    L.check(lib().gd_pam_key_sqnorm_max(_ptr(kt), B, N, Npad, int(f16), _ptr(out), _stream()), "gd_pam_key_sqnorm_max")
    return out


def pam_flash_fwd(qt, kt, v, B, N, Npad, Cn, Cp, gamma, x, out, o_attn, lse, r_alg: int = 32, v_ones: bool = False,
                  f16: bool = False, k_sqmax: Optional[Tensor] = None):
    with _Bracket("pam_flash_fwd", 2.0 * N * N * (r_alg + Cn) * B):
        L.check(lib().gd_pam_flash_fwd(_ptr(qt), _ptr(kt), _ptr(v), B, N, Npad, Cn, Cp, int(v_ones), int(f16),
                                       _ptr(gamma), _ptr(x), _bview(x), _ptr(out), _bview(out), _ptr(o_attn), _ptr(lse),
                                       _ptr(k_sqmax), _stream()), "gd_pam_flash_fwd")


PAM_SHIFT = os.environ.get("GD_PAM_SHIFT", "0") != "0"
PAM_SHIFT_SAMPLES = int(os.environ.get("GD_PAM_SHIFT_SAMPLES", "256"))


def pam_flash_fwd_shift(qt, kt, v, B, N, Npad, Cn, Cp, gamma, x, out, o_attn, lse, r_alg: int = 32, v_ones: bool = False,
                        nsample: Optional[int] = None, return_flags: bool = False):
    _bf(qt, "qt"), _bf(kt, "kt")
    nbytes = int(lib().gd_pam_fwd_shift_ws_bytes(B, Npad))
    ws = torch.empty(nbytes // 4, device=qt.device, dtype=torch.int32)
    with _Bracket("pam_flash_fwd", 2.0 * N * N * (r_alg + Cn) * B):
        L.check(lib().gd_pam_flash_fwd_shift(_ptr(qt), _ptr(kt), _ptr(v), B, N, Npad, Cn, Cp, int(v_ones), _ptr(gamma), _ptr(x),
                                             _bview(x), _ptr(out), _bview(out), _ptr(o_attn), _ptr(lse),
                                             int(nsample or PAM_SHIFT_SAMPLES), _ptr(ws), nbytes, _stream()),
                "gd_pam_flash_fwd_shift")
    if return_flags:
        return ws[B * Npad:].clone()
    return None


PAM_BWD_FORM = int(os.environ.get("GD_PAM_BWD", "0"))
PAM_SCRATCH_CAP = 40 << 30
DETERMINISTIC = False
DET_REDUCE = "unsplit"
_DET_REDUCE_MODES = {"unsplit": 0, "ordered": 1}
DET_WS_BYTES: Optional[int] = None
_DET_WS: dict = {}


def set_deterministic(on: bool, reduce: Optional[str] = None) -> None:
    global DETERMINISTIC, DET_REDUCE
    if reduce is not None and reduce not in _DET_REDUCE_MODES:
        raise L.GandanetError(f"set_deterministic: reduce must be one of {sorted(_DET_REDUCE_MODES)}, got {reduce!r}")
    DETERMINISTIC = bool(on)
    lib().gd_set_deterministic(int(DETERMINISTIC))
    if reduce is not None:
        L.check(lib().gd_set_det_reduce(_DET_REDUCE_MODES[reduce]), "gd_set_det_reduce")
        DET_REDUCE = reduce


def det_ws_bytes() -> int:
    return int(DET_WS_BYTES) if DET_WS_BYTES is not None else int(os.environ.get("GD_DET_WS_MB", "256")) << 20


def det_ws() -> Tuple[Optional[int], int]:
    if not (DETERMINISTIC and DET_REDUCE == "ordered"):
        return None, 0
    nbytes = det_ws_bytes()
    if nbytes <= 0:
        return None, 0
    key = (torch.cuda.current_device(), _stream())
    t = _DET_WS.get(key)
    if t is None or t.numel() != nbytes:
        t = _DET_WS[key] = torch.empty(nbytes, device=torch.device("cuda", key[0]), dtype=torch.uint8)
    return t.data_ptr(), nbytes


def conv3x3_wgrad_plan(B: int, Cout: int, Cin: int, H: int, W: int, stride: int = 1, ws_bytes: Optional[int] = None):
    sp, need = C.c_int(0), C.c_size_t(0)
    nb = det_ws_bytes() if ws_bytes is None else ws_bytes
    L.check(lib().gd_conv3x3_wgrad_plan(B, Cout, Cin, H, W, stride, nb, C.byref(sp), C.byref(need)), "gd_conv3x3_wgrad_plan")
    return sp.value, need.value


def gemm_nt_plan(*, B: int, M: int, N: int, kseg: int, klen: int, splits: int = 0, precision: int = L.PREC_FP32,
                 ws_bytes: Optional[int] = None):
    d = L.GemmNTDesc()
    d.B, d.M, d.N, d.kseg, d.klen, d.splits, d.precision = B, M, N, kseg, klen, splits, precision
    sp, need = C.c_int(0), C.c_size_t(0)
    nb = det_ws_bytes() if ws_bytes is None else ws_bytes
    L.check(lib().gd_gemm_nt_plan(C.byref(d), nb, C.byref(sp), C.byref(need)), "gd_gemm_nt_plan")
    return sp.value, need.value


def pam_bwd_form() -> int:
    return L.PAM_BWD_K64_PARTS if (DETERMINISTIC and PAM_BWD_FORM == 0) else PAM_BWD_FORM


def pam_flash_bwd(qt, kt, kn, vt, dot_, lse, delta, B, N, Npad, Cp, dqn, dkn, dv, r_alg: int = 32, c_alg: int = 0,
                  f16: bool = False, form: Optional[int] = None, out_bs: int = 0):
    form = pam_bwd_form() if form is None else form
    scratch, scratch_bytes = None, 0
    per_image = int(lib().gd_pam_bwd_scratch_bytes(Npad, form))
    if per_image:
        nslices = -(-(B * per_image) // PAM_SCRATCH_CAP)
        images = max(1, -(-B // nslices))
        scratch_bytes = per_image * images
        scratch = torch.empty(scratch_bytes, device=dqn.device, dtype=torch.uint8)
    with _Bracket("pam_flash_bwd", 4.0 * N * N * (r_alg + (c_alg or Cp)) * B):
        L.check(lib().gd_pam_flash_bwd(_ptr(qt), _ptr(kt), _ptr(kn), _ptr(vt), _ptr(dot_), _ptr(lse), _ptr(delta), B,
                                       N, Npad, Cp, int(f16), int(form), _ptr(dqn), _ptr(dkn), _ptr(dv), int(out_bs),
                                       _ptr(scratch), scratch_bytes, _stream()), "gd_pam_flash_bwd")


PAM_WIDE = os.environ.get("GD_PAM_WIDE", "1") != "0"


def pam_wide_slots(r: int) -> int:
    return 32 if r <= 31 else 64


def pam_wide_fwd(qt, kt, v, B, N, Npad, Cn, Cp, D, gamma, x, out, o_attn, lse, r_alg: int, f16: bool = False):
    with _Bracket("pam_wide_fwd", 2.0 * N * N * (r_alg + Cn) * B):
        L.check(lib().gd_pam_wide_fwd(_ptr(qt), _ptr(kt), _ptr(v), B, N, Npad, Cn, Cp, D, int(f16), _ptr(gamma), _ptr(x),
                                      _bview(x), _ptr(out), _bview(out), _ptr(o_attn), _ptr(lse), _stream()),
                "gd_pam_wide_fwd")


def pam_wide_bwd(qt, kt, kn, vt, dot_, lse, delta, B, N, Npad, Cp, D, dqn, dkn, dv, r_alg: int, c_alg: int,
                 f16: bool = False, deterministic: Optional[bool] = None):
    det = DETERMINISTIC if deterministic is None else bool(deterministic)
    scratch, scratch_bytes = None, 0
    per_image = int(lib().gd_pam_wide_scratch_bytes(Npad, D, int(det)))
    if per_image:
        nslices = -(-(B * per_image) // PAM_SCRATCH_CAP)
        scratch_bytes = per_image * max(1, -(-B // nslices))
        scratch = torch.empty(scratch_bytes, device=dqn.device, dtype=torch.uint8)
    with _Bracket("pam_wide_bwd", 4.0 * N * N * (r_alg + c_alg) * B):
        L.check(lib().gd_pam_wide_bwd(_ptr(qt), _ptr(kt), _ptr(kn), _ptr(vt), _ptr(dot_), _ptr(lse), _ptr(delta), B, N,
                                      Npad, Cp, D, int(f16), int(det), _ptr(dqn), _ptr(dkn), _ptr(dv), _ptr(scratch),
                                      scratch_bytes, _stream()), "gd_pam_wide_bwd")


_f32_flash = os.environ.get("GD_PAM_F32_FLASH", "")
PAM_F32_FLASH: Optional[bool] = True if _f32_flash == "1" else False if _f32_flash == "0" else None
PAM_F32_AUTO_ELEMS = 1 << 31
# ... 293 lines not shown
```

### gan-danet_amd/ops.py

```python
from __future__ import annotations

import os
from typing import List, Optional

import torch
from torch.autograd import Function

from . import _lib as L
from . import kern as K
from .config import config, operand_mode, sixteen_bit

ACT_NONE, ACT_RELU, ACT_LEAKY, ACT_SIGMOID = L.ACT_NONE, L.ACT_RELU, L.ACT_LEAKY02, L.ACT_SIGMOID


def _prec(layer: str = "other") -> int:
    mode = operand_mode(layer)
    return L.PREC_BF16 if mode == "16" else L.PREC_X3 if mode == "x3" else L.PREC_FP32


def _x3(layer: str) -> bool:
    return operand_mode(layer) == "x3"


def _x3_eligible(x, w, stride, pad, act) -> bool:
    return (x.dim() == 4 and tuple(w.shape[2:]) == (3, 3) and stride == 1 and pad == 1 and act in (ACT_NONE, ACT_RELU)
            and w.shape[1] >= 32 and w.shape[1] % 8 == 0 and w.shape[0] % 8 == 0 and (x.shape[2] * x.shape[3]) % 8 == 0
            and x.shape[2] * x.shape[3] * 3 * max(w.shape[0], w.shape[1]) < (1 << 31))


def _pam_f16() -> bool:
    return config.precision in ("fp16", "mixed")


def _c(t: torch.Tensor) -> torch.Tensor:
    return t if t.is_contiguous() else t.contiguous()


DISC_NHWC = os.environ.get("GD_DISC_NHWC", "1") != "0"


def disc1_trunk_eligible(x: torch.Tensor, ws) -> bool:
    return (DISC_NHWC and (sixteen_bit("disc") or _x3("disc")) and (not K.DETERMINISTIC or K.DET_REDUCE == "ordered")
            and x.dim() == 4 and x.shape[1] <= 4
            and ws[0].shape[0] == 64 and all(w.shape[0] % 8 == 0 and w.shape[2:] == (3, 3) for w in ws))


class Disc1TrunkFn(Function):

    SLOPE = 0.2

    @staticmethod
    def forward(ctx, x, w1, b1, w2, b2, w3, b3, w4, b4):
        x = _c(x)
        sp = _x3("disc")
        ws, bs = (w1, w2, w3, w4), (b1, b2, b3, b4)
        acts = [K.disc_stem_fwd(x, _c(w1), b1, Disc1TrunkFn.SLOPE, split=sp)]
        for w, b in zip(ws[1:], bs[1:]):
            acts.append(K.conv3x3_nhwc_s2(acts[-1], K.conv3x3_operator(_c(w), "fwd", sp), b, w.shape[0], 2, Disc1TrunkFn.SLOPE,
                                          split=sp))
        ctx.save_for_backward(x, *ws, *acts)
        ctx.has_bias = tuple(b is not None for b in bs)
        ctx.split = sp
        return K.nhwc_flatten_fwd(acts[-1], split=sp)

    @staticmethod
    def backward(ctx, df):
        x, *rest = ctx.saved_tensors
        ws, acts = rest[:4], rest[4:]
        need = ctx.needs_input_grad
        sp = ctx.split
        grads = [None] * 9
        g = K.nhwc_flatten_bwd(_c(df), acts[3], Disc1TrunkFn.SLOPE, split=sp)
        for l in (3, 2, 1):
            if need[1 + 2 * l] or need[2 + 2 * l]:
                dw, db = K.conv3x3_wgrad_nhwc(g, acts[l - 1], 2, ctx.has_bias[l] and need[2 + 2 * l], split=sp)
                grads[1 + 2 * l], grads[2 + 2 * l] = (dw if need[1 + 2 * l] else None), db
            g = K.conv3x3_nhwc_s2_dgrad(g, K.conv3x3_operator(_c(ws[l]), "dgrad_s2", sp), acts[l - 1], Disc1TrunkFn.SLOPE,
                                        split=sp)
        if need[1] or need[2]:
            dw, db = K.disc_stem_wgrad(g, x, ctx.has_bias[0] and need[2], split=sp)
            grads[1], grads[2] = (dw if need[1] else None), db
        if need[0]:
            grads[0] = K.disc_stem_dgrad(g, _c(ws[0]), x.shape[2], x.shape[3], split=sp)
        return tuple(grads)


CONV_WIDE_NHWC = os.environ.get("GD_CONV_WIDE_NHWC", "1") != "0"
DENSE_NHWC = os.environ.get("GD_DENSE_NHWC", "1") != "0"
PAM_CAT = os.environ.get("GD_PAM_CAT", "1") != "0"
WIDE_MIN_CIN = int(os.environ.get("GD_WIDE_MIN_CIN", "128"))


def _wide3x3(x, w, stride, pad, act, prec) -> bool:
    return (CONV_WIDE_NHWC and prec == L.PREC_BF16 and x.dim() == 4 and tuple(w.shape[2:]) == (3, 3) and stride == 1
            and pad == 1 and act in (ACT_NONE, ACT_RELU) and w.shape[1] >= WIDE_MIN_CIN and w.shape[1] % 8 == 0 and w.shape[0] > 32
            and w.shape[0] % 8 == 0 and (x.shape[2] * x.shape[3]) % 8 == 0)


def _pack3x3_x(x, split, scale=None, shift=None, relu=False):
    if split:
        return K.pack_split(x, scale=scale, shift=shift, relu=relu)[1]
    if scale is not None:
        return K.pack_nhwc16_affine(x, scale, shift, relu)
    B, Cin, H, W = x.shape
    return K.pack_bf16(x, Cin, H * W, t_shape=(H * W, Cin))[1]


def _packed3x3_fwd(x16, w, bias, H, W, split, relu=False, out=None):
    return K.conv3x3_nhwc_f32out(x16, K.conv3x3_operator(_c(w), "fwd", split), bias, w.shape[0], H, W, relu=relu, out=out)


def _packed3x3_bwd(dy, x16, w, H, W, split, need_dx, need_dw, mask=None, dw_first=False):
    if not (need_dx or need_dw):
        return None, None
    Cout, N = dy.shape[1], H * W
    if split:
        dyp, dyt = K.pack_split(_as3(dy), want_plain=need_dw, want_tr=need_dx, mask=None if mask is None else _as3(mask))
    else:
        dyp, dyt = K.pack_bf16(_as3(dy), Cout, N, plain_shape=(Cout, N) if need_dw else None,
                               t_shape=(N, Cout) if need_dx else None)

    def wgrad():
        return K.conv3x3_wgrad16(dyp, x16, H, W, split=split, tag="wgrad_x3" if split else "wgrad_packed")

    dx = dw = None
    if need_dw and dw_first:
        dw = wgrad()
    if need_dx:
        dx = K.conv3x3_nhwc_f32out(dyt, K.conv3x3_operator(_c(w), "dgrad", split), None, w.shape[1], H, W)
    if need_dw and not dw_first:
        dw = wgrad()
    return dx, dw


class Conv2dFn(Function):
    @staticmethod
    def forward(ctx, x, w, bias, stride: int, pad: int, act: int, prec=None, layer: str = "other"):
        split = prec is None and _x3(layer) and _x3_eligible(x, w, stride, pad, act)
        prec = _prec(layer) if prec is None else prec
        if split or _wide3x3(x, w, stride, pad, act, prec):
            H, W = x.shape[2:]
            x = _pack3x3_x(x, split)
            y = _packed3x3_fwd(x, w, bias, H, W, split, relu=act == ACT_RELU)
            ctx.packed = (H, W, split)
        else:
            y = K.conv2d_fwd(x, w, bias, stride, pad, prec, act=act)
            ctx.packed = None
        ctx.save_for_backward(x, w, y if act != ACT_NONE else None)
        ctx.cfg = (stride, pad, act, prec, bias is not None)
        return y

    @staticmethod
    def backward(ctx, dy):
        x, w, y = ctx.saved_tensors
        stride, pad, act, prec, has_bias = ctx.cfg
        need_dx, need_dw = ctx.needs_input_grad[:2]
        need_db = has_bias and ctx.needs_input_grad[2]
        dy = _c(dy)
        fuse_mask = ctx.packed is not None and ctx.packed[2] and act == ACT_RELU and not need_dw and not need_db
        if act != ACT_NONE and not fuse_mask:
            dy = K.act_bwd(y, dy, act)
        dx = dw = None
        if ctx.packed is not None:
            dx, dw = _packed3x3_bwd(dy, x, w, *ctx.packed, need_dx, need_dw, mask=y if fuse_mask else None)
        else:
            if need_dx:
                dx = K.conv2d_dgrad(dy, w, (x.shape[2], x.shape[3]), stride, pad, prec)
            if need_dw:
                dw = K.conv2d_wgrad(dy, x, w.shape[2], stride, pad, prec)
        db = K.channel_sum(dy) if need_db else None
        return dx, dw, db, None, None, None, None, None


def conv2d(x, w, bias=None, stride=1, pad=0, act=ACT_NONE, prec=None, layer="other"):
    return Conv2dFn.apply(x, w, bias, stride, pad, act, prec, layer)


class ActFn(Function):

    @staticmethod
    def forward(ctx, x, act: int):
        y = K.act_fwd(_c(x), act)
        ctx.save_for_backward(y)
        ctx.act = act
        return y

    @staticmethod
    def backward(ctx, dy):
        (y,) = ctx.saved_tensors
        return K.act_bwd(y, _c(dy), ctx.act), None


def activation(x, act: int):
    return ActFn.apply(x, act)


def _sync_bn_active() -> bool:
    if not config.sync_bn:
        return False
    from .parallel import is_distributed
    return is_distributed()


def _all_gather_records(stats: torch.Tensor) -> torch.Tensor:
    import torch.distributed as dist
    world = dist.get_world_size()
    out = torch.empty((world,) + tuple(stats.shape), device=stats.device, dtype=stats.dtype)
    if dist.get_backend() == "gloo":
        dist.all_gather([out[r] for r in range(world)], stats)
    else:
        dist.all_gather_into_tensor(out, stats)
    return out


def _bn_prepare(x, gamma, beta, rmean, rvar, training, momentum, eps):
    if training and _sync_bn_active():
        mean, invstd = K.bn_stats_merge(_all_gather_records(K.bn_stats_local(x)), eps, momentum, rmean, rvar)
        scale, shift = K.bn_fold(gamma, beta, mean, invstd)
    elif training:
        mean, invstd = K.bn_stats(x, eps, momentum, rmean, rvar)
        scale, shift = K.bn_fold(gamma, beta, mean, invstd)
    else:
        scale, shift, invstd = K.bn_fold_eval(gamma, beta, rmean, rvar, eps)
        mean = rmean
    return scale, shift, mean, invstd


def _bn_bwd(dy, x, scale, shift, mean, invstd, act, training, sync, dx=None, accumulate_dx=False):
    if not (sync and training):
        return K.bn_act_bwd(dy, x, scale, shift, mean, invstd, act, training, dx=dx, accumulate_dx=accumulate_dx)
    import torch.distributed as dist
    Cn = x.shape[1]
    sums = torch.empty(2, Cn, device=x.device, dtype=torch.float32)
    K.bn_act_bwd(dy, x, scale, shift, mean, invstd, act, training, want_dx=False, sums_out=sums)
    local = torch.empty_like(sums)
    K.copy_slab(sums.view(1, 2 * Cn, 1), local.view(1, 2 * Cn, 1))
    dist.all_reduce(sums, op=dist.ReduceOp.SUM)
    n_global = x.shape[0] * x[0, 0].numel() * dist.get_world_size()
    dx = K.bn_act_bwd_dx(dy, x, scale, shift, mean, invstd, sums[0], sums[1], 1.0 / n_global, act, dx=dx,
                         accumulate_dx=accumulate_dx)
    return local[0], local[1], dx

# ... 5 lines not shown
        y = K.affine_act(x, scale, shift, act)
        ctx.save_for_backward(x, scale, shift, mean, invstd)
        ctx.cfg = (act, training, training and _sync_bn_active())
        return y

    @staticmethod
    def backward(ctx, dy):
        x, scale, shift, mean, invstd = ctx.saved_tensors
        act, training, sync = ctx.cfg
        dgamma, dbeta, dx = _bn_bwd(_c(dy), x, scale, shift, mean, invstd, act, training, sync)
        return dx, dgamma, dbeta, None, None, None, None, None, None


def batch_norm_act(x, gamma, beta, rmean, rvar, training, momentum, eps, act=ACT_NONE):
    return BnActFn.apply(x, gamma, beta, rmean, rvar, training, momentum, eps, act)


class BnReluConvFn(Function):

    @staticmethod
    def forward(ctx, x, gamma, beta, rmean, rvar, w, bias, training, momentum, eps, pad):
        prec = _prec("conv1x1" if w.shape[2] == 1 else "other")
        scale, shift, mean, invstd = _bn_prepare(x, gamma, beta, rmean, rvar, training, momentum, eps)
        y = K.conv2d_fwd(x, w, bias, 1, pad, prec, in_scale=scale, in_shift=shift, in_relu=True)
        ctx.save_for_backward(x, scale, shift, mean, invstd, w)
        ctx.cfg = (training, prec, pad, bias is not None, training and _sync_bn_active())
        return y

    @staticmethod
    def backward(ctx, dy):
        x, scale, shift, mean, invstd, w = ctx.saved_tensors
        training, prec, pad, has_bias, sync = ctx.cfg
        dy = _c(dy)
        dw = K.conv2d_wgrad(dy, x, w.shape[2], 1, pad, prec, in_scale=scale, in_shift=shift, in_relu=True)
        db = K.channel_sum(dy) if has_bias else None
        dxt = K.conv2d_dgrad(dy, w, (x.shape[2], x.shape[3]), 1, pad, prec)
        dgamma, dbeta, dx = _bn_bwd(dxt, x, scale, shift, mean, invstd, ACT_RELU, training, sync)
        return dx, dgamma, dbeta, None, None, dw, db, None, None, None, None


class DenseBlockFn(Function):

    @staticmethod
    def forward(ctx, x, training: bool, momentum: float, eps: float, *params):
        prec = _prec("dense3x3")
        nl = len(params) // 6
        B, C0, H, W = x.shape
        g = params[4].shape[0]
        slab = torch.empty(B, C0 + nl * g, H, W, device=x.device, dtype=torch.float32)
        K.copy_slab(x, slab[:, :C0])
        saved: List[torch.Tensor] = []
        aligned = ((H * W) % 8 == 0 and g % 8 == 0 and all((C0 + l * g) % 8 == 0 for l in range(nl))
                   and tuple(params[4].shape[2:]) == (3, 3))
        split = prec == L.PREC_X3 and aligned and C0 >= 32 and H * W * 3 * (C0 + nl * g) < (1 << 31)
        packed = split or (DENSE_NHWC and prec == L.PREC_BF16 and aligned)
        packs: List[torch.Tensor] = []
        for l in range(nl):
            bw, bb, rm, rv, cw, cb = params[6 * l: 6 * l + 6]
            cl = C0 + l * g
            xin = slab[:, :cl]
            scale, shift, mean, invstd = _bn_prepare(xin, bw, bb, rm, rv, training, momentum, eps)
            if packed:
                packs.append(_pack3x3_x(xin, split, scale, shift, relu=True))
                _packed3x3_fwd(packs[-1], cw, cb, H, W, split, out=slab[:, cl:cl + g])
            else:
                K.conv2d_fwd(xin, cw, cb, 1, 1, prec, in_scale=scale, in_shift=shift, in_relu=True,
                             out=slab[:, cl:cl + g])
            saved += [scale, shift, mean, invstd, cw]
        ctx.save_for_backward(slab, *saved, *packs)
        ctx.cfg = (nl, C0, g, training, prec, [p is not None for p in params[5::6]], packed, split, training and _sync_bn_active())
        return slab

    @staticmethod
    def backward(ctx, dslab_in):
        slab, *saved = ctx.saved_tensors
        nl, C0, g, training, prec, has_bias, packed, split, sync = ctx.cfg
        packs = saved[5 * nl:]
        B, _, H, W = slab.shape
        dslab = torch.empty(slab.shape, device=slab.device, dtype=torch.float32)
        K.copy_slab(_c(dslab_in), dslab)
        grads: List[Optional[torch.Tensor]] = [None] * (6 * nl)
        for l in reversed(range(nl)):
            scale, shift, mean, invstd, cw = saved[5 * l: 5 * l + 5]
            cl = C0 + l * g
            xin = slab[:, :cl]
            dy = dslab[:, cl:cl + g]
            if packed:
                dxt, grads[6 * l + 4] = _packed3x3_bwd(dy, packs[l], cw, H, W, split, True, True, dw_first=True)
            else:
                grads[6 * l + 4] = K.conv2d_wgrad(dy, xin, 3, 1, 1, prec, in_scale=scale, in_shift=shift, in_relu=True)
                dxt = K.conv2d_dgrad(dy, cw, (H, W), 1, 1, prec)
            if has_bias[l]:
                grads[6 * l + 5] = K.channel_sum(dy)
            dgamma, dbeta, _ = _bn_bwd(dxt, xin, scale, shift, mean, invstd, ACT_RELU, training, sync,
                                       dx=dslab[:, :cl], accumulate_dx=True)
            grads[6 * l + 0], grads[6 * l + 1] = dgamma, dbeta
        dx = torch.empty(B, C0, H, W, device=slab.device, dtype=torch.float32)
        K.copy_slab(dslab[:, :C0], dx)
        return (dx, None, None, None, *grads)


def _npad(n: int) -> int:
    return (n + 255) // 256 * 256


def _cp(c: int) -> int:
    return (c + 31) // 32 * 32


def _pam_wide(Cn: int, r: int) -> bool:
    return K.PAM_WIDE and sixteen_bit("pam") and 192 < Cn <= 511 and r <= 63


def _pam_f32(B: int, Cn: int, r: int, N: int) -> bool:
    if operand_mode("pam") != "exact" or not (1 <= Cn <= 511 and 1 <= r <= 63):
        return False
    if K.PAM_F32_FLASH is None:
        return B * N * N > K.PAM_F32_AUTO_ELEMS
    return bool(K.PAM_F32_FLASH)


def _pad_plane(t: torch.Tensor, N: int, Np: int) -> torch.Tensor:
    if N == Np:
        return t
    B, R = t.shape[0], t.shape[1]
    out = torch.zeros(B, R, Np, device=t.device, dtype=torch.float32)
    K.copy_rows(t, K._bview(t), N, out, R * Np, Np, B, R, N)
    return out


def _pam_pack16(q, k, v, r, Cn, N, D, ones_row, f16):
    Np, Cp = _npad(N), _cp(Cn)
    _, qt = K.pack_bf16(q, r, N, scale_imm=K.LOG2E, t_shape=(Np, D), f16=f16)
    kn, kt = K.pack_bf16(k, r, N, plain_shape=(D, Np), t_shape=(Np, D), perm16=True, ones_row=D - 1, f16=f16)
    vn, vt = K.pack_bf16(v, Cn, N, plain_shape=(Cp, Np), t_shape=(Np, Cp), perm16=True, ones_row=ones_row, f16=f16)
    return qt, kt, kn, vn, vt


def _pam_route(B: int, Cn: int, r: int, N: int) -> str:
    if sixteen_bit("pam") and Cn <= 192 and r <= 31:
        return "narrow"
    if _pam_wide(Cn, r):
        return "wide"
    return "f32" if _pam_f32(B, Cn, r, N) else "chain"


def _pam_forward(x, wq, bq, wk, bk, wv, bv, gamma_p, out3, prec):
    B, Cn, H, W = x.shape
    N = H * W
    r = wq.shape[0]
    x3 = x.view(B, Cn, N)
    route = _pam_route(B, Cn, r, N)
    if route != "chain" and PAM_CAT and (bq is None) == (bk is None) == (bv is None):
        wc = torch.empty(2 * r + Cn, Cn, 1, 1, device=x.device, dtype=torch.float32)
        for w_, lo in ((wq, 0), (wk, r), (wv, 2 * r)):
            K.copy_slab(_c(w_).view(1, w_.shape[0], Cn), wc.view(1, 2 * r + Cn, Cn)[:, lo:lo + w_.shape[0]])
        bc = None
        if bq is not None:
            bc = torch.empty(2 * r + Cn, device=x.device, dtype=torch.float32)
            for b_, lo in ((bq, 0), (bk, r), (bv, 2 * r)):
                K.copy_slab(b_.view(1, -1, 1), bc.view(1, -1, 1)[:, lo:lo + b_.numel()])
        y3 = K.conv2d_fwd(x, wc, bc, 1, 0, prec).view(B, 2 * r + Cn, N)
        q, k, v = y3[:, :r], y3[:, r:2 * r], y3[:, 2 * r:]
    else:
        q = K.conv2d_fwd(x, wq, bq, 1, 0, prec).view(B, r, N)
        k = K.conv2d_fwd(x, wk, bk, 1, 0, prec).view(B, r, N)
        v = K.conv2d_fwd(x, wv, bv, 1, 0, prec).view(B, Cn, N)
    if route in ("narrow", "wide"):
        Np, Cp = _npad(N), _cp(Cn)
        f16 = _pam_f16()
        D = 32 if route == "narrow" else K.pam_wide_slots(r)
        ones = Cp - 1 if route == "narrow" and Cn < Cp else -1
        qt, kt, kn, vn, vt = _pam_pack16(q, k, v, r, Cn, N, D, ones, f16)
        del q, k, v
        y3 = None
        o_attn = torch.empty(B, Cn, N, device=x.device, dtype=torch.float32)
        lse = torch.empty(B, N, device=x.device, dtype=torch.float32)
        if route == "wide":
            K.pam_wide_fwd(qt, kt, vn, B, N, Np, Cn, Cp, D, gamma_p, x3, out3, o_attn, lse, r_alg=r, f16=f16)
        elif K.PAM_SHIFT and not f16:
            K.pam_flash_fwd_shift(qt, kt, vn, B, N, Np, Cn, Cp, gamma_p, x3, out3, o_attn, lse, r_alg=r, v_ones=ones >= 0)
        else:
            k_sqmax = K.pam_key_sqnorm_max(kt, N, f16) if K.PAM_NOMAX else None
            K.pam_flash_fwd(qt, kt, vn, B, N, Np, Cn, Cp, gamma_p, x3, out3, o_attn, lse, r_alg=r, v_ones=ones >= 0, f16=f16,
                            k_sqmax=k_sqmax)
        return route, (qt, kt, kn, vt, o_attn, lse)
    if route == "f32":
        Np = _npad(N)
        q, k, v = _pad_plane(q, N, Np), _pad_plane(k, N, Np), _pad_plane(v, N, Np)
        o_attn = torch.empty(B, Cn, N, device=x.device, dtype=torch.float32)
        lse = torch.empty(B, N, device=x.device, dtype=torch.float32)
        K.pam_f32_fwd(q, k, v, B, N, Np, Cn, r, gamma_p, x3, out3, o_attn, lse)
        return route, (q, k, v, o_attn, lse)
    prec = prec if sixteen_bit("pam") else L.PREC_FP32
    return route, _pam_chain_fwd(q, k, v, x3, gamma_p, out3, prec)


def _pam_chain_fwd(q, k, v, x3, gamma_p, out3, prec):
    B, r, N = q.shape
    Cn = v.shape[1]
    qt_, kt_ = K.transpose(q), K.transpose(k)
    s = torch.empty(B, N, N, device=q.device, dtype=torch.float32)
    K.gemm_nt(B=B, M=N, N=N, kseg=1, klen=r, a=qt_, a_bs=N * r, a_ss=0, lda=r, bm=kt_, b_bs=N * r, b_ss=0,
              ldb=r, c=s, c_bs=N * N, ldc=N, precision=prec, splits=1)
    p = K.softmax_rows(s, 1.0, out=s)
    o_attn = torch.empty(B, Cn, N, device=q.device, dtype=torch.float32)
    K.gemm_nt(B=B, M=Cn, N=N, kseg=1, klen=N, a=v, a_bs=Cn * N, a_ss=0, lda=N, bm=p, b_bs=N * N, b_ss=0,
              ldb=N, c=o_attn, c_bs=Cn * N, ldc=N, precision=prec, splits=1)
    K.copy_slab(x3, out3)
    _axpy_dev3(o_attn, gamma_p, out3)
    return qt_, kt_, v, p, o_attn


def _pam_chain_bwd(pam_saved, gamma_p, d_pam, pprec):
    qt_, kt_, v, p, o_attn = pam_saved
    B, N, r = qt_.shape
    Cn = v.shape[1]
    dev = v.device
    dop = torch.empty(B, Cn, N, device=dev, dtype=torch.float32)
    K.copy_slab(d_pam, dop)
    dgamma_p = K.dot(dop, o_attn)
    K.scale_dev(dop, gamma_p, out=dop)
    dp = torch.empty(B, N, N, device=dev, dtype=torch.float32)
    K.conv_nn(B=B, M=N, Ck=Cn, ks=1, stride=1, pad=0, transposed=False, Hi=1, Wi=N, Ho=1, Wo=N, a=dop,
              a_bs=Cn * N, a_sm=1, a_sc=N, a_st=0, x=v, x_bs=Cn * N, y=dp, y_bs=N * N, precision=pprec)
    ds = K.softmax_rows_bwd(p, dp, 1.0)
    del dp
    dv = torch.empty(B, Cn, N, device=dev, dtype=torch.float32)
    K.conv_nn(B=B, M=Cn, Ck=N, ks=1, stride=1, pad=0, transposed=False, Hi=1, Wi=N, Ho=1, Wo=N, a=dop,
              a_bs=Cn * N, a_sm=N, a_sc=1, a_st=0, x=p, x_bs=N * N, y=dv, y_bs=Cn * N, precision=pprec)
    dqt = torch.empty(B, N, r, device=dev, dtype=torch.float32)
    dkt = torch.empty(B, N, r, device=dev, dtype=torch.float32)
    K.conv_nn(B=B, M=N, Ck=N, ks=1, stride=1, pad=0, transposed=False, Hi=1, Wi=r, Ho=1, Wo=r, a=ds,
              a_bs=N * N, a_sm=N, a_sc=1, a_st=0, x=kt_, x_bs=N * r, y=dqt, y_bs=N * r, precision=pprec)
    K.conv_nn(B=B, M=N, Ck=N, ks=1, stride=1, pad=0, transposed=False, Hi=1, Wi=r, Ho=1, Wo=r, a=ds,
              a_bs=N * N, a_sm=1, a_sc=N, a_st=0, x=qt_, x_bs=N * r, y=dkt, y_bs=N * r, precision=pprec)
    return K.transpose(dqt), K.transpose(dkt), dv, dgamma_p


def _pam_backward(route, pam_saved, x, wq, wk, wv, gamma_p, d_pam, dx, prec, has_bias):
    B, Cn, H, W = x.shape
    N = H * W
    r = wq.shape[0]
    if route == "f32":
        q, k, v, o_attn, lse = pam_saved
        Np = q.shape[2]
        d_raw, delta = K.chan_dot(d_pam, o_attn, gamma_p)
        dgamma_p = K.dot(d_raw, None)
        if Np == N:
            gdo = torch.empty(B, Cn, N, device=x.device, dtype=torch.float32)
            K.copy_slab(d_pam, gdo)
        else:
            gdo = _pad_plane(d_pam, N, Np)
        K.scale_dev(gdo, gamma_p, out=gdo)
        dq = torch.empty(B, r, N, device=x.device, dtype=torch.float32)
        dk = torch.empty(B, r, N, device=x.device, dtype=torch.float32)
        dv = torch.empty(B, Cn, N, device=x.device, dtype=torch.float32)
        K.pam_f32_bwd(q, k, v, gdo, lse, delta, B, N, Np, Cn, r, dq, dk, dv)
    elif route in ("narrow", "wide"):
        qt, kt, kn, vt, o_attn, lse = pam_saved
        Np, Cp = _npad(N), _cp(Cn)
        d_raw, delta = K.chan_dot(d_pam, o_attn, gamma_p)
        dgamma_p = K.dot(d_raw, None)
        f16 = qt.dtype == torch.float16
        s_up, s_inv = gamma_p, None
        if f16:
            scales = K.pam_f16_scale(d_pam, gamma_p, delta)
            s_up, s_inv = scales[0:1], scales[1:2]
        _, dot_ = K.pack_bf16(d_pam, Cn, N, scale=s_up, t_shape=(Np, Cp), f16=f16)
        if route == "wide":
            D = qt.shape[2]
            dqn = torch.empty(B, D, Np, device=x.device, dtype=torch.float32)
            dkn = torch.empty(B, D, Np, device=x.device, dtype=torch.float32)
            dvp = torch.empty(B, Cp, Np, device=x.device, dtype=torch.float32)
            K.pam_wide_bwd(qt, kt, kn, vt, dot_, lse, delta, B, N, Np, Cp, D, dqn, dkn, dvp, r_alg=r, c_alg=Cn, f16=f16)
        elif PAM_CAT and Np == N and K.pam_bwd_form() == L.PAM_BWD_K64_ATOMIC:
            R = 64 + Cp
            dcat = torch.empty(B, R, Np, device=x.device, dtype=torch.float32)
            K.pam_flash_bwd(qt, kt, kn, vt, dot_, lse, delta, B, N, Np, Cp, dcat[:, 0:32], dcat[:, 32:64], dcat[:, 64:],
                            r_alg=r, c_alg=Cn, f16=f16, out_bs=R * Np)
            wcat = torch.zeros(R, Cn, 1, 1, device=x.device, dtype=torch.float32)
            for w_, lo in ((wq, 0), (wk, 32), (wv, 64)):
                K.copy_slab(_c(w_).view(1, w_.shape[0], Cn), wcat.view(1, R, Cn)[:, lo:lo + w_.shape[0]])
            dcat4 = dcat.view(B, R, H, W)
            dwc = K.conv2d_wgrad(dcat4, x, 1, 1, 0, prec, alpha=s_inv)
            dbc = K.channel_sum(dcat4) if any(has_bias) else None
            if dbc is not None and s_inv is not None:
                K.scale_dev(dbc, s_inv, out=dbc)
            K.conv2d_dgrad(dcat4, wcat, (H, W), 1, 0, prec, out=dx.view(B, Cn, H, W), accumulate=True, alpha=s_inv)
            grads = []
            for (lo, n), hb in zip(((0, r), (32, r), (64, Cn)), has_bias):
                grads.append(dwc[lo:lo + n])
                grads.append(dbc[lo:lo + n] if hb else None)
            return (*grads, dgamma_p)
        else:
            dqn = torch.empty(B, 32, Np, device=x.device, dtype=torch.float32)
            dkn = torch.empty(B, 32, Np, device=x.device, dtype=torch.float32)
            dvp = torch.empty(B, Cp, Np, device=x.device, dtype=torch.float32)
            K.pam_flash_bwd(qt, kt, kn, vt, dot_, lse, delta, B, N, Np, Cp, dqn, dkn, dvp, r_alg=r, c_alg=Cn, f16=f16)
        if s_inv is not None:
            for t in (dqn, dkn, dvp):
                K.scale_dev(t, s_inv, out=t)
        dq, dk, dv = _compact(dqn, r, N), _compact(dkn, r, N), _compact(dvp, Cn, N)
    else:
        pprec = prec if sixteen_bit("pam") else L.PREC_FP32
        dq, dk, dv, dgamma_p = _pam_chain_bwd(pam_saved, gamma_p, d_pam, pprec)
    grads = []
    splits = 1 if route == "f32" else 0
    for dy3, w, hb in ((dq, wq, has_bias[0]), (dk, wk, has_bias[1]), (dv, wv, has_bias[2])):
        dy4 = dy3.view(B, dy3.shape[1], H, W)
        grads.append(K.conv2d_wgrad(dy4, x, 1, 1, 0, prec, splits=splits))
        grads.append(K.channel_sum(dy4) if hb else None)
        K.conv2d_dgrad(dy4, w, (H, W), 1, 0, prec, out=dx.view(B, Cn, H, W), accumulate=True)
    return (*grads, dgamma_p)


def _cam_forward(x, gamma_c, out3, prec=L.PREC_FP32):
    B, Cn, H, W = x.shape
    N = H * W
    x3 = x.view(B, Cn, N)
    e = torch.empty(B, Cn, Cn, device=x.device, dtype=torch.float32)
    K.gemm_nt(B=B, M=Cn, N=Cn, kseg=1, klen=N, a=x3, a_bs=Cn * N, a_ss=0, lda=N, bm=x3, b_bs=Cn * N, b_ss=0,
              ldb=N, c=e, c_bs=Cn * Cn, ldc=Cn, precision=L.PREC_FP32)
    att = K.softmax_rows(e, -1.0, out=e)
    K.conv_nn(B=B, M=Cn, Ck=Cn, ks=1, stride=1, pad=0, transposed=False, Hi=1, Wi=N, Ho=1, Wo=N, a=att,
              a_bs=Cn * Cn, a_sm=Cn, a_sc=1, a_st=0, x=x3, x_bs=Cn * N, y=out3, y_bs=K._bview(out3),
              precision=prec, alpha=gamma_c, res=x3, res_bs=Cn * N)
    return att


def _cam_backward(att, x, gamma_c, d_cam, dx, prec=L.PREC_FP32):
    B, Cn, H, W = x.shape
    N = H * W
    x3 = x.view(B, Cn, N)
    d_bs = K._bview(d_cam)
    da = torch.empty(B, Cn, Cn, device=x.device, dtype=torch.float32)
    K.gemm_nt(B=B, M=Cn, N=Cn, kseg=1, klen=N, a=d_cam, a_bs=d_bs, a_ss=0, lda=N, bm=x3, b_bs=Cn * N, b_ss=0,
              ldb=N, c=da, c_bs=Cn * Cn, ldc=Cn, precision=L.PREC_FP32)
    dgamma_c = K.dot(att, da)
    de = K.softmax_rows_bwd(att, da, -1.0)
    sym = K.add_transpose(de)
    K.conv_nn(B=B, M=Cn, Ck=Cn, ks=1, stride=1, pad=0, transposed=False, Hi=1, Wi=N, Ho=1, Wo=N, a=att,
              a_bs=Cn * Cn, a_sm=1, a_sc=Cn, a_st=0, x=d_cam, x_bs=d_bs, y=dx, y_bs=Cn * N,
              precision=prec, alpha=gamma_c, accumulate=True)
    K.conv_nn(B=B, M=Cn, Ck=Cn, ks=1, stride=1, pad=0, transposed=False, Hi=1, Wi=N, Ho=1, Wo=N, a=sym,
              a_bs=Cn * Cn, a_sm=Cn, a_sc=1, a_st=0, x=x3, x_bs=Cn * N, y=dx, y_bs=Cn * N,
              precision=prec, alpha=gamma_c, accumulate=True)
    return dgamma_c


class PamFn(Function):

    @staticmethod
    def forward(ctx, x, wq, bq, wk, bk, wv, bv, gamma_p):
        x = _c(x)
        prec = _prec("conv1x1")
        out = torch.empty_like(x)
        route, saved = _pam_forward(x, wq, bq, wk, bk, wv, bv, gamma_p, _as3(out), prec)
        ctx.save_for_backward(x, wq, wk, wv, gamma_p, *saved)
        ctx.cfg = (prec, route, (bq is not None, bk is not None, bv is not None))
        return out

    @staticmethod
    def backward(ctx, dout):
        x, wq, wk, wv, gamma_p, *saved = ctx.saved_tensors
        prec, route, has_bias = ctx.cfg
        B, Cn, H, W = x.shape
        d3 = _as3(_c(dout))
        dx = torch.empty(B, Cn, H * W, device=x.device, dtype=torch.float32)
        K.copy_slab(d3, dx)
        dwq, dbq, dwk, dbk, dwv, dbv, dg = _pam_backward(route, saved, x, wq, wk, wv, gamma_p, d3, dx, prec, has_bias)
        return dx.view(B, Cn, H, W), dwq, dbq, dwk, dbk, dwv, dbv, dg


class CamFn(Function):

    @staticmethod
    def forward(ctx, x, gamma_c):
        x = _c(x)
        out = torch.empty_like(x)
        ctx.prec = _prec("cam_apply")
        att = _cam_forward(x, gamma_c, _as3(out), ctx.prec)
        ctx.save_for_backward(x, gamma_c, att)
        return out

    @staticmethod
    def backward(ctx, dout):
        x, gamma_c, att = ctx.saved_tensors
        B, Cn, H, W = x.shape
        d3 = _as3(_c(dout))
        dx = torch.empty(B, Cn, H * W, device=x.device, dtype=torch.float32)
        K.copy_slab(d3, dx)
        dg = _cam_backward(att, x, gamma_c, d3, dx, ctx.prec)
        return dx.view(B, Cn, H, W), dg


class DualAttentionFn(Function):

    @staticmethod
    def forward(ctx, x, wq, bq, wk, bk, wv, bv, gamma_p, gamma_c):
        x = _c(x)
        B, Cn, H, W = x.shape
        prec, cprec = _prec("conv1x1"), _prec("cam_apply")
        feats = torch.empty(B, 2 * Cn, H, W, device=x.device, dtype=torch.float32)
        route, saved = _pam_forward(x, wq, bq, wk, bk, wv, bv, gamma_p, _as3(feats[:, :Cn]), prec)
        att = _cam_forward(x, gamma_c, _as3(feats[:, Cn:]), cprec)
        ctx.save_for_backward(x, wq, wk, wv, gamma_p, gamma_c, att, *saved)
        ctx.cfg = (prec, route, (bq is not None, bk is not None, bv is not None), cprec)
        return feats

    @staticmethod
    def backward(ctx, dfeat):
        x, wq, wk, wv, gamma_p, gamma_c, att, *saved = ctx.saved_tensors
        prec, route, has_bias, cprec = ctx.cfg
        B, Cn, H, W = x.shape
        dfeat = _c(dfeat)
        d_pam, d_cam = _as3(dfeat[:, :Cn]), _as3(dfeat[:, Cn:])
        dx = torch.empty(B, Cn, H * W, device=x.device, dtype=torch.float32)
        K.copy_slab(d_pam, dx)
        K.copy_slab(d_cam, dx, accumulate=True)
        dgc = _cam_backward(att, x, gamma_c, d_cam, dx, cprec)
        dwq, dbq, dwk, dbk, dwv, dbv, dgp = _pam_backward(route, saved, x, wq, wk, wv, gamma_p, d_pam, dx, prec, has_bias)
        return dx.view(B, Cn, H, W), dwq, dbq, dwk, dbk, dwv, dbv, dgp, dgc


def _as3(t: torch.Tensor) -> torch.Tensor:
    B, Cn, H, W = t.shape
    return t.as_strided((B, Cn, H * W), (t.stride(0), H * W, 1), t.storage_offset())


def _axpy_dev3(src: torch.Tensor, s: torch.Tensor, dst3: torch.Tensor) -> None:
    B = src.shape[0]
    if dst3.is_contiguous():
        K.scale_dev(src, s, out=dst3, accumulate=True)
        return
    for b in range(B):
        K.scale_dev(src[b], s, out=dst3[b], accumulate=True)


def _compact(t: torch.Tensor, rows: int, cols: int) -> torch.Tensor:
    B, Rp, Np = t.shape
    if Rp == rows and Np == cols:
        return t
    if Np == cols:
        return t[:, :rows]
    out = torch.empty(B, rows, cols, device=t.device, dtype=torch.float32)
    K.copy_rows(t, Rp * Np, Np, out, rows * cols, cols, B, rows, cols)
    return out


class BicubicFn(Function):
    @staticmethod
    def forward(ctx, x, Ho: int, Wo: int, rsh: float, rsw: float):
        x = _c(x)
        ctx.cfg = (x.shape[2], x.shape[3], rsh, rsw)
        return K.bicubic_fwd(x, Ho, Wo, rsh, rsw)

    @staticmethod
    def backward(ctx, dy):
        Hi, Wi, rsh, rsw = ctx.cfg
        return K.bicubic_bwd(_c(dy), Hi, Wi, rsh, rsw), None, None, None, None


def bicubic_up2(x):
    return BicubicFn.apply(x, 2 * x.shape[2], 2 * x.shape[3], 0.5, 0.5)


class BilinearFn(Function):
    @staticmethod
    def forward(ctx, x, Ho: int, Wo: int):
        x = _c(x)
        ctx.cfg = (x.shape[2], x.shape[3])
        return K.bilinear_fwd(x, Ho, Wo)

    @staticmethod
    def backward(ctx, dy):
        Hi, Wi = ctx.cfg
        return K.bilinear_bwd(_c(dy), Hi, Wi), None, None


class SkipFuseFn(Function):

    @staticmethod
    def forward(ctx, x, *wf):
        prec = _prec("conv1x1")
        n = len(wf) // 2
        ws, fs = wf[:n], [_c(f) for f in wf[n:]]
        x = _c(x)
        B, Co, Ho, Wo = x.shape
        s = K.conv2d_fwd(fs[0], ws[0], None, 1, 0, prec)
        for w, f in zip(ws[1:], fs[1:]):
            if f.shape[2:] != fs[0].shape[2:]:
                raise L.GandanetError("SkipFuseFn: all skip features must share one resolution")
            K.conv2d_fwd(f, w, None, 1, 0, prec, out=s, accumulate=True)
        out = K.bilinear_fwd(s, Ho, Wo, res=x)
        ctx.save_for_backward(*ws, *fs)
        ctx.cfg = (prec, n)
        return out

    @staticmethod
    def backward(ctx, dout):
        prec, n = ctx.cfg
        saved = ctx.saved_tensors
        ws, fs = saved[:n], saved[n:]
        dout = _c(dout)
        Hi, Wi = fs[0].shape[2], fs[0].shape[3]
        ds = K.bilinear_bwd(dout, Hi, Wi)
        gw = [K.conv2d_wgrad(ds, f, 1, 1, 0, prec) for f in fs]
        gf = [K.conv2d_dgrad(ds, w, (Hi, Wi), 1, 0, prec) for w in ws]
        return (dout, *gw, *gf)


class ShiftSum9Fn(Function):

    @staticmethod
    def forward(ctx, u, bias):
        ctx.has_bias = bias is not None
        return K.shift_sum9_fwd(_c(u), bias)

    @staticmethod
    def backward(ctx, dy):
        dy = _c(dy)
        return K.shift_sum9_bwd(dy), (K.dot(dy, None).view(1) if ctx.has_bias else None)


class MaxPool2Fn(Function):
    @staticmethod
    def forward(ctx, x):
        x = _c(x)
        ctx.save_for_backward(x)
        return K.maxpool2_fwd(x)

    @staticmethod
    def backward(ctx, dy):
        (x,) = ctx.saved_tensors
        return K.maxpool2_bwd(x, _c(dy))


class LinearFn(Function):
    @staticmethod
    def forward(ctx, x, w, bias, act: int):
        prec = _prec("disc")
        if prec == L.PREC_X3:
            prec = L.PREC_FP32
        x = _c(x)
        Bn, Kin = x.shape
        Nout = w.shape[0]
        y = torch.empty(Bn, Nout, device=x.device, dtype=torch.float32)
        K.gemm_nt(B=1, M=Bn, N=Nout, kseg=1, klen=Kin, a=x, a_bs=0, a_ss=0, lda=Kin, bm=w, b_bs=0, b_ss=0, ldb=Kin,
                  c=y, c_bs=0, ldc=Nout, precision=prec, bias=bias)
        if act != ACT_NONE:
            K.act_fwd(y, act, out=y)
        ctx.save_for_backward(x, w, y if act != ACT_NONE else None)
        ctx.cfg = (act, prec, bias is not None)
        return y

    @staticmethod
    def backward(ctx, dy):
        x, w, y = ctx.saved_tensors
        act, prec, has_bias = ctx.cfg
        dy = _c(dy)
        if act != ACT_NONE:
            dy = K.act_bwd(y, dy, act)
        Bn, Kin = x.shape
        Nout = w.shape[0]
        dx = dw = db = None
        if ctx.needs_input_grad[0]:
            dx = torch.empty(Bn, Kin, device=x.device, dtype=torch.float32)
            K.conv_nn(B=1, M=Bn, Ck=Nout, ks=1, stride=1, pad=0, transposed=False, Hi=1, Wi=Kin, Ho=1, Wo=Kin, a=dy,
                      a_bs=0, a_sm=Nout, a_sc=1, a_st=0, x=w, x_bs=0, y=dx, y_bs=0, precision=prec)
        if ctx.needs_input_grad[1]:
            dw = torch.empty(Nout, Kin, device=x.device, dtype=torch.float32)
            K.conv_nn(B=1, M=Nout, Ck=Bn, ks=1, stride=1, pad=0, transposed=False, Hi=1, Wi=Kin, Ho=1, Wo=Kin, a=dy,
                      a_bs=0, a_sm=1, a_sc=Nout, a_st=0, x=x, x_bs=0, y=dw, y_bs=0, precision=prec)
# ... 320 lines not shown
```

### include/gandanet.h

```cpp
#ifndef GANDANET_H
#define GANDANET_H
#include <stddef.h>
#include <stdint.h>
#ifdef __cplusplus
extern "C" {
#endif

#define GD_VERSION 100
void gd_set_deterministic(int on);
int gd_get_deterministic(void);
int gd_set_det_reduce(int mode);
int gd_get_det_reduce(void);
int gd_version(void);
int gd_last_error(char* buf, int n);
int gd_sizeof_conv_desc(void);
int gd_sizeof_gemm_nt_desc(void);

enum { GD_PREC_FP32 = 0,
       GD_PREC_BF16 = 1,
       GD_PREC_X3 = 2     };
enum { GD_ACT_NONE = 0, GD_ACT_RELU = 1, GD_ACT_LEAKY02 = 2, GD_ACT_SIGMOID = 3 };

typedef struct gd_conv_desc {
    int B;
    int M;
    int Mstore;
    int Ck;
    int ks;
    int stride, pad;
    int transposed;
    int Hi, Wi;
    int Ho, Wo;
    const float* a; long a_bs, a_sm, a_sc, a_st;
    const float* x; long x_bs;
    const float* in_scale; const float* in_shift; int in_relu;
    void* y; long y_bs;
    int out_layout;
    int out_bf16;
    int ldo;
    const float* alpha; const float* bias; const float* res; long res_bs;
    int act; int accumulate;
    int precision;
    int sub_oy, sub_ox, sub_step;
} gd_conv_desc;
int gd_conv2d(const gd_conv_desc* d, void* stream);

size_t gd_conv3x3_ws_bytes(int M, int Ck);
int gd_conv3x3_eligible(const gd_conv_desc* d);
int gd_conv3x3(const gd_conv_desc* d, void* ws, size_t ws_bytes, void* stream);
int gd_conv3x3_wgrad(const float* dy, long dy_bs, const void* dy_bf16, const float* x, long x_bs, const void* x_nhwc16,
                     int x_ld, const float* in_scale, const float* in_shift, int in_relu, int B, int Cout, int Cin, int H,
                     int W, int stride, int accumulate, float* dw, void* stream);
int gd_conv3x3_wgrad_ws(const float* dy, long dy_bs, const void* dy_bf16, const float* x, long x_bs, const void* x_nhwc16,
                        int x_ld, const float* in_scale, const float* in_shift, int in_relu, int B, int Cout, int Cin, int H,
                        int W, int stride, int accumulate, float* dw, void* stream, void* ws, size_t ws_bytes);
int gd_conv3x3_wgrad_plan(int B, int Cout, int Cin, int H, int W, int stride, size_t ws_bytes, int* splits, size_t* ws_needed);

typedef struct gd_gemm_nt_desc {
    int B, M, N;
    int kseg; long klen;
    const float* a; long a_bs, a_ss, lda;
    const float* bm; long b_bs, b_ss, ldb;
    int im2col, ks, stride, pad, Hi, Wi, Ho, Wo;
    const float* in_scale; const float* in_shift; int in_relu;
    float* c; long c_bs, ldc;
    const float* alpha;
    const float* bias;
    int accumulate;
    int splits;
    int precision;
} gd_gemm_nt_desc;
int gd_gemm_nt(const gd_gemm_nt_desc* d, void* stream);
int gd_gemm_nt_ws(const gd_gemm_nt_desc* d, void* stream, void* ws, size_t ws_bytes);
int gd_gemm_nt_plan(const gd_gemm_nt_desc* d, size_t ws_bytes, int* splits, size_t* ws_needed);

size_t gd_bn_stats_ws_floats(int B, int C, long HW);
int gd_bn_stats(const float* x, long x_bs, int B, int C, long HW, float eps, float momentum,
                float* mean, float* invstd, float* running_mean, float* running_var, float* ws, void* stream);
int gd_bn_fold(const float* gamma, const float* beta, const float* mean, const float* invstd, int C,
               float* scale, float* shift, void* stream);
int gd_bn_stats_local(const float* x, long x_bs, int B, int C, long HW, float* stats, float* ws, void* stream);
int gd_bn_stats_merge(const float* stats_all, int world, int C, float eps, float momentum, float* mean, float* invstd,
                      float* running_mean, float* running_var, void* stream);
int gd_bn_act_bwd_dx(const float* dy, long dy_bs, const float* x, long x_bs, const float* scale, const float* shift,
                     const float* mean, const float* invstd, const float* dgamma_sum, const float* dbeta_sum, float inv_n,
                     int B, int C, long HW, int act, float* dx, long dx_bs, int accumulate_dx, void* stream);
int gd_bn_fold_eval(const float* gamma, const float* beta, const float* running_mean, const float* running_var,
                    float eps, int C, float* scale, float* shift, float* invstd_out, void* stream);
int gd_channel_sum(const float* x, long x_bs, int B, int C, long HW, float* out, int accumulate, float* ws,
                   void* stream);
int gd_affine_act(const float* x, long x_bs, const float* scale, const float* shift, int B, int C, long HW,
                  int act, float* y, long y_bs, void* stream);
int gd_bn_act_bwd(const float* dy, long dy_bs, const float* x, long x_bs, const float* scale, const float* shift,
                  const float* mean, const float* invstd, const float* gamma, int B, int C, long HW, int act,
                  int train, float* dgamma, float* dbeta, float* dx, long dx_bs, int accumulate_dx, float* ws,
                  void* stream);

int gd_bicubic_fwd(const float* x, int BC, int Hi, int Wi, float* y, int Ho, int Wo, float rscale_h,
                   float rscale_w, void* stream);
int gd_bicubic_bwd(const float* dy, int BC, int Hi, int Wi, float* dx, int Ho, int Wo, float rscale_h,
                   float rscale_w, void* stream);
int gd_shift_sum9_fwd(const float* u, const float* bias, float* y, int B, int H, int W, void* stream);
int gd_shift_sum9_bwd(const float* dy, float* du, int B, int H, int W, void* stream);
int gd_combine_inputs(const float* lr, int C1, int H1, int W1, float rs1, const float* aux, int C2, int H2, int W2,
                      float rs2, float* out, int B, int Ho, int Wo, void* stream);
int gd_bilinear_fwd(const float* x, int BC, int Hi, int Wi, float* y, int Ho, int Wo, int accumulate,
                    const float* res, void* stream);
int gd_bilinear_bwd(const float* dy, int BC, int Hi, int Wi, float* dx, int Ho, int Wo, void* stream);
int gd_maxpool2_fwd(const float* x, int BC, int Hi, int Wi, float* y, void* stream);
int gd_maxpool2_bwd(const float* x, const float* dy, int BC, int Hi, int Wi, float* dx, void* stream);

int gd_act_fwd(const float* x, float* y, long n, int act, void* stream);
int gd_act_bwd(const float* y, const float* dy, float* dx, long n, int act, void* stream);
int gd_axpby(const float* x, float a, float* y, float b, long n, void* stream);
int gd_scale_dev(const float* x, const float* s_dev, float* y, long n, int accumulate, void* stream);
int gd_copy_rows(const float* src, long s_bs, long s_ld, float* dst, long d_bs, long d_ld, int B, int R, int Cc,
                 void* stream);
int gd_copy_slab(const float* src, long s_bs, float* dst, long d_bs, int B, long chw, int accumulate, void* stream);
int gd_softmax_rows(const float* x, float* y, long rows, int cols, float sign, void* stream);
int gd_softmax_rows_bwd(const float* p, const float* dp, float* dx, long rows, int cols, float sign, void* stream);
int gd_dot(const float* a, const float* b, long n, float* out, int accumulate, float* ws, void* stream);
int gd_transpose(const float* s, float* t, int B, int R, int Cc, void* stream);
int gd_add_transpose(const float* a, float* out, int B, int n, void* stream);

int gd_bce_logits(const float* z, long n, float label, float* out, float* dz, float* ws, void* stream);
int gd_bce_logits_target(const float* z, const float* t, long n, float* out, float* dz, float* dt, float* ws,
                         void* stream);
int gd_leaky_fwd(const float* x, float* y, long n, float slope, void* stream);
int gd_leaky_bwd(const float* x, const float* dy, float* dx, long n, float slope, void* stream);
int gd_mse(const float* a, const float* b, long n, float* out, float* da, float* ws, void* stream);
int gd_l1(const float* a, const float* b, long n, float* out, float* da, float* ws, void* stream);
int gd_tv(const float* x, int B, int C, int H, int W, float weight, float* out, float* dx, float* ws, void* stream);
int gd_ssim(const float* a, const float* b, int BC, int H, int W, int window, float* out, float* ws, void* stream);
int gd_ssim_samples(const float* a, const float* b, int B, int C, int H, int W, int window, float* out, float* ws,
                    void* stream);
int gd_ssim_bwd(const float* a, const float* b, const float* gscale, int B, int C, int H, int W, int window,
                float* coef_ws, float* da, float* db, void* stream);

int gd_adamw(float* p, const float* g, float* m, float* v, long n, int step, float lr, float beta1, float beta2,
             float eps, float weight_decay, float grad_scale, void* stream);

int gd_conv3x3_nhwc_pack(const float* w, int Cout, int Cin, int transposed, void* ws, size_t ws_bytes, void* stream);
int gd_conv3x3_nhwc(const void* x, const void* wpack, const float* bias, const void* mask, const void* res, void* y, int B,
                    int H, int W, int K, int M, int relu, int split, void* stream);
int gd_conv3x3_nhwc_f32out(const void* x, const void* wpack, const float* bias, float* y32, long y_bs, int B, int H, int W, int K,
                           int M, int relu, void* stream);
int gd_nhwc_stem_fwd(const float* img, int B, int Ci, int H, int W, const float* w, const float* bias, int Co, int relu,
                     void* y, int split, void* stream);
int gd_nhwc_stem_bwd(const void* g, int B, int Ci, int H, int W, const float* w, int Co, float* dimg, int split, void* stream);
int gd_nhwc_maxpool2_fwd(const void* x, int B, int H, int W, int C, void* y, int split, void* stream);
int gd_nhwc_maxpool2_bwd(const void* x, const void* dy, int B, int H, int W, int C, int relu_mask, void* dx, int split, void* stream);
int gd_nhwc_l1(const void* a, const void* b, long n, float* out, int accumulate, float* ws, int split_c, void* stream);
int gd_nhwc_l1_grad(const void* a, const void* b, long n, const float* upstream, int relu_mask, void* g, int split_c, void* stream);

int gd_disc_stem_fwd(const float* img, int B, int Ci, int H, int W, const float* w, const float* bias, int Co, float slope,
                     void* y, int split, void* stream);
int gd_disc_stem_wgrad(const void* g, const float* img, int B, int Ci, int H, int W, int Co, float* dw, float* db, int split, void* stream);
int gd_disc_stem_wgrad_ws(const void* g, const float* img, int B, int Ci, int H, int W, int Co, float* dw, float* db, int split,
                          void* stream, void* ws, size_t ws_bytes);
int gd_disc_stem_dgrad(const void* g, int B, int Ci, int H, int W, const float* w, int Co, float* dimg, int split, void* stream);
int gd_conv3x3_nhwc_s2(const void* x, const void* wpack, const float* bias, void* y, int B, int H, int W, int K, int M, int act,
                       float slope, int split, void* stream);
int gd_conv3x3_nhwc_s2_dgrad(const void* dy, const void* wpack_t, const void* act_out, float slope, void* dx, int B, int H,
                             int W, int K, int M, int split, void* stream);
int gd_nhwc_flatten_fwd(const void* y, int B, int HW, int C, float* f, int split, void* stream);
int gd_nhwc_flatten_bwd(const float* df, const void* y, float slope, int B, int HW, int C, void* g, int split, void* stream);
int gd_nhwc_to_nchw16(const void* g, int B, int HW, int C, void* gt, float* csum, int split, void* stream);
int gd_nhwc_to_nchw16_ws(const void* g, int B, int HW, int C, void* gt, float* csum, int split, void* stream, void* ws,
                         size_t ws_bytes);

int gd_pam_flash_fwd(const void* qt, const void* kt, const void* v, int B, int N, int Npad, int C, int Cp,
                     int v_ones, int f16, const float* gamma, const float* x, long x_bs, float* out, long out_bs,
                     float* o_attn, float* lse, const float* k_sqnorm_max, void* stream);
size_t gd_pam_fwd_shift_ws_bytes(int B, int Npad);
int gd_pam_flash_fwd_shift(const void* qt, const void* kt, const void* v, int B, int N, int Npad, int C, int Cp, int v_ones,
                           const float* gamma, const float* x, long x_bs, float* out, long out_bs, float* o_attn, float* lse,
                           int nsample, void* ws, size_t ws_bytes, void* stream);
int gd_pam_key_sqnorm_max(const void* kt, int B, int N, int Npad, int f16, float* out, void* stream);
#define GD_PAM_BWD_K64_ATOMIC 0
#define GD_PAM_BWD_K64_PARTS 1
#define GD_PAM_BWD_K32_PARTS 2
#define GD_PAM_BWD_TWO_KERNEL 3
size_t gd_pam_bwd_scratch_bytes(int Npad, int form);
int gd_pam_flash_bwd(const void* qt, const void* kt, const void* kn, const void* vt, const void* dot_,
                     const float* lse, const float* delta, int B, int N, int Npad, int Cp, int f16, int form,
                     float* dqn, float* dkn, float* dv, long out_bs, void* scratch, size_t scratch_bytes, void* stream);
int gd_pam_wide_fwd(const void* qt, const void* kt, const void* v, int B, int N, int Npad, int C, int Cp, int D, int f16,
                    const float* gamma, const float* x, long x_bs, float* out, long out_bs, float* o_attn, float* lse,
                    void* stream);
size_t gd_pam_wide_scratch_bytes(int Npad, int D, int deterministic);
int gd_pam_wide_bwd(const void* qt, const void* kt, const void* kn, const void* vt, const void* dot_, const float* lse,
                    const float* delta, int B, int N, int Npad, int Cp, int D, int f16, int deterministic, float* dqn,
                    float* dkn, float* dv, void* scratch, size_t scratch_bytes, void* stream);
int gd_pam_f32_fwd(const float* q, long q_bs, const float* k, long k_bs, const float* v, long v_bs, int B, int N, int Npad,
                   int C, int r, const float* gamma, const float* x, long x_bs, float* out, long out_bs, float* o_attn,
                   float* lse, void* stream);
int gd_pam_f32_bwd(const float* q, long q_bs, const float* k, long k_bs, const float* v, long v_bs, const float* gdo,
                   long gdo_bs, const float* lse, const float* delta, int B, int N, int Npad, int C, int r, float* dq,
                   float* dk, float* dv, void* stream);

size_t gd_hist_match_ws_bytes(long ns, long nt);
int gd_hist_match(const float* src, const float* ref, int B, long ns, long nt, double weight, double* out, void* ws,
                  size_t ws_bytes, void* stream);
int gd_blend_region(float* gen, const float* grace, const float* mask, int BC, int H, int W, int sr, int er, int sc,
                    int ec, void* stream);
int gd_augment_d4(const float* src, float* dst, int B, int C, int H, int W, const int* ops, const float* noise,
                  float noise_scale, void* stream);
int gd_bcast_mul(const float* x, const float* att, float* y, int B, int C, long HW, int mode, void* stream);
int gd_row_dot(const float* a, const float* b, float* out, long rows, long n, void* stream);
int gd_chan_maxmean_fwd(const float* x, float* y, int* idx, int B, int C, long HW, void* stream);
int gd_chan_maxmean_bwd(const float* dy, const int* idx, float* dx, int B, int C, long HW, void* stream);
int gd_chan_dot(const float* a, long a_bs, const float* o, long o_bs, int B, int C, int N, const float* gamma,
                float* d_raw, float* delta, void* stream);
int gd_pack_16_split(const float* s, long s_bs, int B, int R, int Cc, const float* row_scale, const float* row_shift, int relu,
                     void* plain, long p_bs, int ldp, long p_cs, int p_ncopy, int p_pattern, void* tr, long t_bs, int ldt,
                     long t_cs, int t_ncopy, int t_pattern, void* stream);
int gd_pack_16_split_masked(const float* s, long s_bs, int B, int R, int Cc, const float* row_scale, const float* row_shift,
                            int relu, void* plain, long p_bs, int ldp, long p_cs, int p_ncopy, int p_pattern, void* tr, long t_bs,
                            int ldt, long t_cs, int t_ncopy, int t_pattern, const float* mask, long m_bs, void* stream);
int gd_split3_weights(const float* w, long A, long Bn, long Cn, float* out, void* stream);
int gd_pam_f16_scale(const float* dout, long dout_bs, int B, int C, int N, const float* gamma, float* delta, float* scales,
                     float* ws, void* stream);
int gd_pack_bf16(const float* s, long s_bs, int B, int R, int Cc, const float* scale_dev, float scale_imm, void* plain,
                 int Rp_plain, int ld_plain, void* transposed, int Ccp_t, int ld_t, int perm16, int ones_row,
                 void* stream);
int gd_pack_16(const float* s, long s_bs, int B, int R, int Cc, const float* scale_dev, float scale_imm, void* plain,
               int Rp_plain, int ld_plain, void* transposed, int Ccp_t, int ld_t, int perm16, int ones_row, int f16,
               void* stream);
int gd_pack_16_affine(const float* s, long s_bs, int B, int R, int Cc, const float* row_scale, const float* row_shift, int relu,
                      void* plain, int Rp_plain, int ld_plain, void* transposed, int Ccp_t, int ld_t, int f16, void* stream);

int gd_comm_unique_id(char* id128);
int gd_comm_init(int rank, int world, const char* id128);
int gd_comm_world(void);
int gd_allreduce(void* buf, size_t n, int dtype, void* stream);
int gd_reduce_scatter(const void* send, void* recv, size_t recv_n, int dtype, void* stream);
int gd_allgather(const void* send, void* recv, size_t send_n, int dtype, void* stream);
int gd_comm_destroy(void);

#ifdef __cplusplus
}
#endif
#endif
```

Measured before the change: 38.50 samples/s.

## Fuse attention backward: two-segment K conv, fused chan_dot+pack, single weight concat

Adds an optional second K-segment (a2/x2) and a second residual (res2) to the conv GEMM kernels. CAM backward can then compute att^T·d_cam + sym·x plus both residuals in one launch, replacing separate copies and an accumulating second GEMM. PAM backward fuses the channel dot with the bf16 transposed pack of dOut, and three-slab weight concatenation becomes one kernel. The goal is fewer launches and fewer passes over large activations, at the cost of more kernel template variants and a per-thread strided pack loop.

```diff
diff --git a/gan-danet_amd/_lib.py b/gan-danet_amd/_lib.py
--- a/gan-danet_amd/_lib.py
+++ b/gan-danet_amd/_lib.py
@@ -26,6 +26,9 @@
         ("alpha", c_fp), ("bias", c_fp), ("res", c_fp), ("res_bs", C.c_long),
         ("act", C.c_int), ("accumulate", C.c_int), ("precision", C.c_int),
         ("sub_oy", C.c_int), ("sub_ox", C.c_int), ("sub_step", C.c_int),
+        ("a2", c_fp), ("a2_bs", C.c_long), ("a2_sm", C.c_long), ("a2_sc", C.c_long), ("Ck2", C.c_int),
+        ("x2", c_fp), ("x2_bs", C.c_long),
+        ("res2", c_fp), ("res2_bs", C.c_long),
     ]
 
 
@@ -117,6 +120,8 @@
     "gd_pam_f32_fwd": (_i, [_p, _l, _p, _l, _p, _l, _i, _i, _i, _i, _i, _p, _p, _l, _p, _l, _p, _p, _p]),
     "gd_pam_f32_bwd": (_i, [_p, _l, _p, _l, _p, _l, _p, _l, _p, _p, _i, _i, _i, _i, _i, _p, _p, _p, _p]),
     "gd_chan_dot": (_i, [_p, _l, _p, _l, _i, _i, _i, _p, _p, _p, _p]),
+    "gd_cat_rows3": (_i, [_p, _i, _i, _p, _i, _i, _p, _i, _i, _p, _i, _i, _p]),
+    "gd_chan_dot_pack": (_i, [_p, _l, _p, _l, _i, _i, _i, _p, _p, _p, _p, _i, _i, _p]),
     "gd_pam_f16_scale": (_i, [_p, _l, _i, _i, _i, _p, _p, _p, _p, _p]),
     "gd_conv3x3_nhwc_pack": (_i, [_p, _i, _i, _i, _p, _sz, _p]),
     "gd_conv3x3_nhwc": (_i, [_p, _p, _p, _p, _p, _p, _i, _i, _i, _i, _i, _i, _i, _p]),
diff --git a/gan-danet_amd/csrc/gemm_conv.hip b/gan-danet_amd/csrc/gemm_conv.hip
--- a/gan-danet_amd/csrc/gemm_conv.hip
+++ b/gan-danet_amd/csrc/gemm_conv.hip
@@ -13,7 +13,7 @@
 constexpr int BN = TILE_BN;
 constexpr int BK = TILE_BK;
 
-template <int BM, int MODE>
+template <int BM, int MODE, bool SEG2 = false>
 __global__ __launch_bounds__(256) void conv_nn_kernel(const gd_conv_desc d) {
     constexpr bool BF16 = MODE != gd::MODE_F32;
     constexpr bool X3 = MODE == gd::MODE_X3;
@@ -66,12 +66,31 @@
 
     const int ktiles_per_tap = (d.Ck + BK - 1) / BK;
     const int ntaps = d.ks * d.ks;
-    const int T = ntaps * ktiles_per_tap;
+    const int T1 = ntaps * ktiles_per_tap;
+    const int T = SEG2 ? T1 + (d.Ck2 + BK - 1) / BK : T1;
 
     float ra[KPT_A];
     float rb[KPT_B];
 
     auto load_tile = [&](int t) {
+        if constexpr (SEG2) {
+            if (t >= T1) {
+                const int c0 = (t - T1) * BK;
+                const float* ap = d.a2 + (long)b * d.a2_bs + (long)(m0 + am) * d.a2_sm;
+#pragma unroll
+                for (int i = 0; i < KPT_A; ++i) {
+                    const int c = c0 + akg * KPT_A + i;
+                    ra[i] = (a_row_ok && c < d.Ck2) ? ap[(long)c * d.a2_sc] : 0.f;
+                }
+                const float* xp = d.x2 + (long)b * d.x2_bs + (long)oy * d.Wi + ox;
+#pragma unroll
+                for (int i = 0; i < KPT_B; ++i) {
+                    const int c = c0 + bkh * KPT_B + i;
+                    rb[i] = (p_ok && c < d.Ck2) ? xp[(long)c * HiWi] : 0.f;
+                }
+                return;
+            }
+        }
         const int tap = t / ktiles_per_tap;
         const int c0 = (t - tap * ktiles_per_tap) * BK;
         const int kh = tap / d.ks, kw = tap - kh * d.ks;
@@ -201,6 +220,8 @@
             for (int e = 0; e < 16; ++e) {
                 const int m = m0 + wm * TM * 32 + i * 32 + gd::acc_row(e, h);
                 rsv[e] = (d.res && m < d.M) ? d.res[(long)b * d.res_bs + (long)m * HoWo + pn] : 0.f;
+                if constexpr (SEG2)
+                    if (d.res2 && m < d.M) rsv[e] += d.res2[(long)b * d.res2_bs + (long)m * HoWo + pn];
             }
 #pragma unroll
             for (int e = 0; e < 16; ++e) {
@@ -506,7 +527,7 @@
         }
 }
 
-template <int BM, bool X3 = false>
+template <int BM, bool X3 = false, bool SEG2 = false>
 __global__ __launch_bounds__(256) void conv1x1_tr_plain_kernel(const gd_conv_desc d) {
     constexpr int LDA = BK + 8;
     constexpr int A_PL = BM * LDA, X_PL = BK * XLD;
@@ -542,8 +563,37 @@
 
     float ra[KPT_A];
     float4 rx[4];
-    const int T = (d.Ck + BK - 1) / BK;
+    const int T1 = (d.Ck + BK - 1) / BK;
+    const int T = SEG2 ? T1 + (d.Ck2 + BK - 1) / BK : T1;
     auto load_tile = [&](int t) {
+        if constexpr (SEG2) {
+            if (t >= T1) {
+                const int c0 = (t - T1) * BK;
+                const float* ap = d.a2 + (long)b * d.a2_bs + (long)(m0 + am) * d.a2_sm;
+#pragma unroll
+                for (int i = 0; i < KPT_A; ++i) {
+                    const int c = c0 + akg * KPT_A + i;
+                    ra[i] = (a_row_ok && c < d.Ck2) ? ap[(long)c * d.a2_sc] : 0.f;
+                }
+#pragma unroll
+                for (int i = 0; i < 4; ++i) {
+                    const int c = c0 + xr0 + 8 * i;
+                    float4 v = make_float4(0.f, 0.f, 0.f, 0.f);
+                    if (c < d.Ck2) {
+                        const float* p = d.x2 + (long)b * d.x2_bs + (long)c * HW + pq;
+                        if (q_full) {
+                            v = *reinterpret_cast<const float4*>(p);
+                        } else {
+                            if (pq + 0 < HW) v.x = p[0];
+                            if (pq + 1 < HW) v.y = p[1];
+                            if (pq + 2 < HW) v.z = p[2];
+                        }
+                    }
+                    rx[i] = v;
+                }
+                return;
+            }
+        }
         const int c0 = t * BK;
 #pragma unroll
         for (int i = 0; i < KPT_A; ++i) {
@@ -708,6 +758,8 @@
             for (int e = 0; e < 16; ++e) {
                 const int m = m0 + wm * TM * 32 + i * 32 + gd::acc_row(e, h);
                 rsv[e] = (d.res && m < d.M) ? d.res[(long)b * d.res_bs + (long)m * HW + pn] : 0.f;
+                if constexpr (SEG2)
+                    if (d.res2 && m < d.M) rsv[e] += d.res2[(long)b * d.res2_bs + (long)m * HW + pn];
             }
 #pragma unroll
             for (int e = 0; e < 16; ++e) {
@@ -729,6 +781,7 @@
 
 static bool conv1x1_tr_eligible(const gd_conv_desc& d) {
     const long HW = (long)d.Ho * d.Wo;
+    if (d.a2 && (d.x2_bs % 4 != 0 || ((uintptr_t)d.x2 % 16) != 0)) return false;
     return d.ks == 1 && d.stride == 1 && d.pad == 0 && (d.precision == GD_PREC_BF16 || d.precision == GD_PREC_X3) && d.out_layout == 0 && !d.out_bf16 &&
            (d.Mstore == 0 || d.Mstore == d.M) && d.Hi == d.Ho && d.Wi == d.Wo && HW % 4 == 0 && d.x_bs % 4 == 0 &&
            ((uintptr_t)d.x % 16) == 0;
@@ -740,7 +793,14 @@
     const long hs = (d.Ho - d.sub_oy + sstep - 1) / sstep, ws = (d.Wo - d.sub_ox + sstep - 1) / sstep;
     if (hs <= 0 || ws <= 0) return 0;
     dim3 grid(gd_cdiv(hs * ws, BN), gd_cdiv(d.Mstore, BM), d.B);
-    if (d.precision == GD_PREC_BF16)
+    if (d.a2) {
+        if (d.precision == GD_PREC_BF16)
+            hipLaunchKernelGGL((conv_nn_kernel<BM, gd::MODE_BF16, true>), grid, dim3(256), 0, s, d);
+        else if (d.precision == GD_PREC_X3)
+            hipLaunchKernelGGL((conv_nn_kernel<BM, gd::MODE_X3, true>), grid, dim3(256), 0, s, d);
+        else
+            hipLaunchKernelGGL((conv_nn_kernel<BM, gd::MODE_F32, true>), grid, dim3(256), 0, s, d);
+    } else if (d.precision == GD_PREC_BF16)
         hipLaunchKernelGGL((conv_nn_kernel<BM, gd::MODE_BF16>), grid, dim3(256), 0, s, d);
     else if (d.precision == GD_PREC_X3)
         hipLaunchKernelGGL((conv_nn_kernel<BM, gd::MODE_X3>), grid, dim3(256), 0, s, d);
@@ -764,6 +824,14 @@
     GD_CHECK_ARG(d.out_layout == 0 || (d.out_layout == 1 && d.ldo >= d.Mstore), "gd_conv2d: bad output layout");
     GD_CHECK_ARG(!(d.out_bf16 && d.accumulate), "gd_conv2d: accumulate needs an fp32 output");
     GD_CHECK_ARG((long)d.Ho * d.Wo < (1L << 31) && d.B <= 65535, "gd_conv2d: image too large for one launch");
+    if (d.a2) {
+        GD_CHECK_ARG(d.x2 && d.Ck2 > 0, "gd_conv2d: the second K-segment needs a2, x2 and Ck2 > 0");
+        GD_CHECK_ARG(d.ks == 1 && d.stride == 1 && d.pad == 0 && !d.transposed && !d.in_scale && d.Hi == d.Ho && d.Wi == d.Wo,
+                     "gd_conv2d: a second K-segment is for plain 1x1 / stride 1 products only");
+    } else {
+        GD_CHECK_ARG(!d.x2 && !d.res2, "gd_conv2d: x2 / res2 come with a second K-segment (a2)");
+    }
+    GD_CHECK_ARG(!d.res2 || d.res, "gd_conv2d: res2 needs res");
     GD_CHECK_ARG(d.sub_step >= 0 && d.sub_oy >= 0 && d.sub_ox >= 0 && (d.sub_step > 1 || (d.sub_oy == 0 && d.sub_ox == 0)),
                  "gd_conv2d: bad output sub-lattice");
     if (!d.transposed) {
@@ -784,6 +852,18 @@
         if (ns != 1 && ns != 2 && ns != 4) ns = 1;
         dim3 grid(gd_cdiv(HWl, BN * ns), gd_cdiv(d.M, bm), d.B);
 #define GD_C1X1(BM_, NS_) hipLaunchKernelGGL((conv1x1_tr_kernel<BM_, NS_>), grid, dim3(256), 0, s, d)
+        if (d.a2) {
+            dim3 g2(gd_cdiv(HWl, BN), gd_cdiv(d.M, bm), d.B);
+            if (d.precision == GD_PREC_X3) {
+                if (bm == 32) hipLaunchKernelGGL((conv1x1_tr_plain_kernel<32, true, true>), g2, dim3(256), 0, s, d);
+                else if (bm == 64) hipLaunchKernelGGL((conv1x1_tr_plain_kernel<64, true, true>), g2, dim3(256), 0, s, d);
+                else hipLaunchKernelGGL((conv1x1_tr_plain_kernel<128, true, true>), g2, dim3(256), 0, s, d);
+            } else {
+                if (bm == 32) hipLaunchKernelGGL((conv1x1_tr_plain_kernel<32, false, true>), g2, dim3(256), 0, s, d);
+                else if (bm == 64) hipLaunchKernelGGL((conv1x1_tr_plain_kernel<64, false, true>), g2, dim3(256), 0, s, d);
+                else hipLaunchKernelGGL((conv1x1_tr_plain_kernel<128, false, true>), g2, dim3(256), 0, s, d);
+            }
+        } else
         if (d.precision == GD_PREC_X3) {
             if (bm == 32) hipLaunchKernelGGL((conv1x1_tr_plain_kernel<32, true>), grid, dim3(256), 0, s, d);
             else if (bm == 64) hipLaunchKernelGGL((conv1x1_tr_plain_kernel<64, true>), grid, dim3(256), 0, s, d);
diff --git a/gan-danet_amd/csrc/pointwise.hip b/gan-danet_amd/csrc/pointwise.hip
--- a/gan-danet_amd/csrc/pointwise.hip
+++ b/gan-danet_amd/csrc/pointwise.hip
@@ -448,6 +448,54 @@
     delta[(long)b * N + i] = s * (*gamma);
 }
 
+__global__ __launch_bounds__(256) void cat_rows3_kernel(const float* __restrict__ s0, int n0, int lo0, const float* __restrict__ s1,
+                                                       int n1, int lo1, const float* __restrict__ s2, int n2, int lo2,
+                                                       float* __restrict__ dst, int R, int Cc) {
+    const long total = (long)R * Cc;
+    for (long i = (long)blockIdx.x * 256 + threadIdx.x; i < total; i += (long)gridDim.x * 256) {
+        const int r = (int)(i / Cc);
+        const long c = i - (long)r * Cc;
+        float v = 0.f;
+        if (s0 && r >= lo0 && r < lo0 + n0) v = s0[(long)(r - lo0) * Cc + c];
+        else if (s1 && r >= lo1 && r < lo1 + n1) v = s1[(long)(r - lo1) * Cc + c];
+        else if (s2 && r >= lo2 && r < lo2 + n2) v = s2[(long)(r - lo2) * Cc + c];
+        dst[i] = v;
+    }
+}
+
+__global__ __launch_bounds__(256) void chan_dot_pack_kernel(const float* __restrict__ a, long a_bs, const float* __restrict__ o,
+                                                           long o_bs, int C, int N, const float* __restrict__ gamma,
+                                                           float* __restrict__ draw, float* __restrict__ delta,
+                                                           unsigned short* __restrict__ tr, int Npad, int ldt, int fma_form) {
+    const int b = blockIdx.y;
+    const int i = blockIdx.x * 256 + threadIdx.x;
+    if (i >= Npad) return;
+    const bool live = i < N;
+    const float* ap = a + (long)b * a_bs + i;
+    const float* op = o + (long)b * o_bs + i;
+    const float k = *gamma;
+    uint4* row = reinterpret_cast<uint4*>(tr + ((long)b * Npad + i) * ldt);
+    float s = 0.f;
+    for (int c0 = 0; c0 < ldt; c0 += 8) {
+        float v[8];
+#pragma unroll
+        for (int j = 0; j < 8; ++j) {
+            const int c = c0 + j;
+            v[j] = 0.f;
+            if (live && c < C) {
+                const float av = ap[(long)c * N];
+                s = fmaf(av, op[(long)c * N], s);
+                v[j] = fma_form ? fmaf(av, k, 0.f) : k * av;
+            }
+        }
+        row[c0 >> 3] = make_uint4(gd_pack_bf2(v[0], v[1]), gd_pack_bf2(v[2], v[3]), gd_pack_bf2(v[4], v[5]), gd_pack_bf2(v[6], v[7]));
+    }
+    if (live) {
+        draw[(long)b * N + i] = s;
+        delta[(long)b * N + i] = s * k;
+    }
+}
+
 __global__ __launch_bounds__(256) void absmax_kernel(const float* __restrict__ a, long a_bs, long chw, float* __restrict__ ws) {
     __shared__ float red[8];
     const float* ap = a + (long)blockIdx.y * a_bs;
@@ -915,6 +963,27 @@
     GD_LAUNCH_CHECK();
     return 0;
 }
+extern "C" int gd_cat_rows3(const float* s0, int n0, int lo0, const float* s1, int n1, int lo1, const float* s2, int n2, int lo2,
+                            float* dst, int R, int Cc, void* stream) {
+    GD_CHECK_ARG(dst && R > 0 && Cc > 0 && n0 >= 0 && n1 >= 0 && n2 >= 0 && lo0 >= 0 && lo1 >= 0 && lo2 >= 0, "gd_cat_rows3: bad arguments");
+    GD_CHECK_ARG((!s0 || lo0 + n0 <= R) && (!s1 || lo1 + n1 <= R) && (!s2 || lo2 + n2 <= R), "gd_cat_rows3: a block passes the last row");
+    const long total = (long)R * Cc;
+    hipLaunchKernelGGL(cat_rows3_kernel, dim3(grid_for(total) > 1024 ? 1024 : grid_for(total)), dim3(256), 0, GD_S, s0, n0, lo0, s1, n1,
+                       lo1, s2, n2, lo2, dst, R, Cc);
+    GD_LAUNCH_CHECK();
+    return 0;
+}
+extern "C" int gd_chan_dot_pack(const float* a, long a_bs, const float* o, long o_bs, int B, int C, int N, const float* gamma,
+                                float* d_raw, float* delta, void* tr, int Npad, int ldt, void* stream) {
+    GD_CHECK_ARG(a && o && gamma && d_raw && delta && tr && B > 0 && B <= 65535 && C > 0 && N > 0, "gd_chan_dot_pack: bad arguments");
+    GD_CHECK_ARG(Npad >= N && ldt >= C && ldt % 8 == 0 && ((uintptr_t)tr % 16) == 0,
+                 "gd_chan_dot_pack: tr needs Npad >= N rows of ldt >= C channels, ldt % 8 == 0, 16-byte aligned");
+    const int fma_form = N % 4 == 0 && a_bs % 4 == 0 && ((uintptr_t)a % 16) == 0;
+    hipLaunchKernelGGL(chan_dot_pack_kernel, dim3(gd_cdiv(Npad, 256), B), dim3(256), 0, GD_S, a, a_bs, o, o_bs, C, N, gamma, d_raw,
+                       delta, (unsigned short*)tr, Npad, ldt, fma_form);
+    GD_LAUNCH_CHECK();
+    return 0;
+}
 
 extern "C" int gd_pam_f16_scale(const float* dout, long dout_bs, int B, int C, int N, const float* gamma, float* delta,
                                 float* scales, float* ws, void* stream) {
diff --git a/gan-danet_amd/kern.py b/gan-danet_amd/kern.py
--- a/gan-danet_amd/kern.py
+++ b/gan-danet_amd/kern.py
@@ -115,7 +115,9 @@
             y: Tensor, y_bs: int, precision: int, Mstore: int = 0, in_scale: Optional[Tensor] = None,
             in_shift: Optional[Tensor] = None, in_relu: bool = False, out_layout: int = 0, out_bf16: bool = False,
             ldo: int = 0, alpha: Optional[Tensor] = None, bias: Optional[Tensor] = None,
-            res: Optional[Tensor] = None, res_bs: int = 0, act: int = 0, accumulate: bool = False) -> None:
+            res: Optional[Tensor] = None, res_bs: int = 0, act: int = 0, accumulate: bool = False,
+            a2: Optional[Tensor] = None, a2_bs: int = 0, a2_sm: int = 0, a2_sc: int = 0, Ck2: int = 0,
+            x2: Optional[Tensor] = None, x2_bs: int = 0, res2: Optional[Tensor] = None, res2_bs: int = 0) -> None:
     d = L.ConvDesc()
     d.B, d.M, d.Mstore, d.Ck, d.ks, d.stride, d.pad = B, M, max(M, Mstore), Ck, ks, stride, pad
     d.transposed = int(transposed)
@@ -127,6 +129,8 @@
     d.out_layout, d.out_bf16, d.ldo = out_layout, int(out_bf16), ldo
     d.alpha, d.bias, d.res, d.res_bs = _ptr(alpha), _ptr(bias), _ptr(res), res_bs
     d.act, d.accumulate, d.precision = act, int(accumulate), precision
+    d.a2, d.a2_bs, d.a2_sm, d.a2_sc, d.Ck2 = _ptr(a2), a2_bs, a2_sm, a2_sc, Ck2
+    d.x2, d.x2_bs, d.res2, d.res2_bs = _ptr(x2), x2_bs, _ptr(res2), res2_bs
     if USE_CONV3X3_FAST and lib().gd_conv3x3_eligible(C.byref(d)):
         nbytes = int(lib().gd_conv3x3_ws_bytes(M, Ck))
         ws = torch.empty(nbytes // 2, device=x.device, dtype=torch.bfloat16)
@@ -727,6 +731,34 @@
     return d_raw, delta
 
 
+def cat_rows3(blocks, R: int) -> Tensor:
+    t0 = blocks[0][0]
+    cc = t0[0].numel()
+    out = torch.empty((R, *t0.shape[1:]), device=t0.device, dtype=torch.float32)
+    args = []
+    for t, lo in blocks:
+        _dense(t, "cat_rows3 block")
+        if t[0].numel() != cc:
+            raise L.GandanetError("cat_rows3: blocks differ in row length")
+        args += [_ptr(t), t.shape[0], lo]
+    args += [None, 0, 0] * (3 - len(blocks))
+    L.check(lib().gd_cat_rows3(*args, _ptr(out), R, cc, _stream()), "gd_cat_rows3")
+    return out
+
+
+def chan_dot_pack(a: Tensor, o: Tensor, gamma: Tensor, t_shape):
+    abs_, obs = _bview(a), _bview(o)
+    B, Cn = a.shape[0], a.shape[1]
+    N = a[0, 0].numel()
+    npad, ldt = t_shape
+    d_raw = torch.empty(B, N, device=a.device, dtype=torch.float32)
+    delta = torch.empty_like(d_raw)
+    tr = torch.empty(B, npad, ldt, device=a.device, dtype=torch.bfloat16)
+    L.check(lib().gd_chan_dot_pack(_ptr(a), abs_, _ptr(o), obs, B, Cn, N, _ptr(gamma), _ptr(d_raw), _ptr(delta), _ptr(tr),
+                                   npad, ldt, _stream()), "gd_chan_dot_pack")
+    return d_raw, delta, tr
+
+
 def pam_f16_scale(dout: Tensor, gamma: Tensor, delta: Tensor) -> Tensor:
     bs = _bview(dout, "dOut")
     B, Cn = dout.shape[0], dout.shape[1]
diff --git a/gan-danet_amd/ops.py b/gan-danet_amd/ops.py
--- a/gan-danet_amd/ops.py
+++ b/gan-danet_amd/ops.py
@@ -88,6 +88,7 @@
 CONV_WIDE_NHWC = os.environ.get("GD_CONV_WIDE_NHWC", "1") != "0"
 DENSE_NHWC = os.environ.get("GD_DENSE_NHWC", "1") != "0"
 PAM_CAT = os.environ.get("GD_PAM_CAT", "1") != "0"
+ATTN_BWD_FUSED = os.environ.get("GD_ATTN_BWD_FUSED", "1") != "0"
 WIDE_MIN_CIN = int(os.environ.get("GD_WIDE_MIN_CIN", "128"))
 
 
@@ -399,14 +400,8 @@
     x3 = x.view(B, Cn, N)
     route = _pam_route(B, Cn, r, N)
     if route != "chain" and PAM_CAT and (bq is None) == (bk is None) == (bv is None):
-        wc = torch.empty(2 * r + Cn, Cn, 1, 1, device=x.device, dtype=torch.float32)
-        for w_, lo in ((wq, 0), (wk, r), (wv, 2 * r)):
-            K.copy_slab(_c(w_).view(1, w_.shape[0], Cn), wc.view(1, 2 * r + Cn, Cn)[:, lo:lo + w_.shape[0]])
-        bc = None
-        if bq is not None:
-            bc = torch.empty(2 * r + Cn, device=x.device, dtype=torch.float32)
-            for b_, lo in ((bq, 0), (bk, r), (bv, 2 * r)):
-                K.copy_slab(b_.view(1, -1, 1), bc.view(1, -1, 1)[:, lo:lo + b_.numel()])
+        wc = K.cat_rows3(((_c(wq), 0), (_c(wk), r), (_c(wv), 2 * r)), 2 * r + Cn)
+        bc = None if bq is None else K.cat_rows3(((_c(bq), 0), (_c(bk), r), (_c(bv), 2 * r)), 2 * r + Cn)
         y3 = K.conv2d_fwd(x, wc, bc, 1, 0, prec).view(B, 2 * r + Cn, N)
         q, k, v = y3[:, :r], y3[:, r:2 * r], y3[:, 2 * r:]
     else:
@@ -507,14 +502,18 @@
     elif route in ("narrow", "wide"):
         qt, kt, kn, vt, o_attn, lse = pam_saved
         Np, Cp = _npad(N), _cp(Cn)
-        d_raw, delta = K.chan_dot(d_pam, o_attn, gamma_p)
-        dgamma_p = K.dot(d_raw, None)
         f16 = qt.dtype == torch.float16
         s_up, s_inv = gamma_p, None
-        if f16:
-            scales = K.pam_f16_scale(d_pam, gamma_p, delta)
-            s_up, s_inv = scales[0:1], scales[1:2]
-        _, dot_ = K.pack_bf16(d_pam, Cn, N, scale=s_up, t_shape=(Np, Cp), f16=f16)
+        if ATTN_BWD_FUSED and not f16:
+            d_raw, delta, dot_ = K.chan_dot_pack(d_pam, o_attn, gamma_p, (Np, Cp))
+            dgamma_p = K.dot(d_raw, None)
+        else:
+            d_raw, delta = K.chan_dot(d_pam, o_attn, gamma_p)
+            dgamma_p = K.dot(d_raw, None)
+            if f16:
+                scales = K.pam_f16_scale(d_pam, gamma_p, delta)
+                s_up, s_inv = scales[0:1], scales[1:2]
+            _, dot_ = K.pack_bf16(d_pam, Cn, N, scale=s_up, t_shape=(Np, Cp), f16=f16)
         if route == "wide":
             D = qt.shape[2]
             dqn = torch.empty(B, D, Np, device=x.device, dtype=torch.float32)
@@ -526,9 +525,7 @@
             dcat = torch.empty(B, R, Np, device=x.device, dtype=torch.float32)
             K.pam_flash_bwd(qt, kt, kn, vt, dot_, lse, delta, B, N, Np, Cp, dcat[:, 0:32], dcat[:, 32:64], dcat[:, 64:],
                             r_alg=r, c_alg=Cn, f16=f16, out_bs=R * Np)
-            wcat = torch.zeros(R, Cn, 1, 1, device=x.device, dtype=torch.float32)
-            for w_, lo in ((wq, 0), (wk, 32), (wv, 64)):
-                K.copy_slab(_c(w_).view(1, w_.shape[0], Cn), wcat.view(1, R, Cn)[:, lo:lo + w_.shape[0]])
+            wcat = K.cat_rows3(((_c(wq), 0), (_c(wk), 32), (_c(wv), 64)), R)
             dcat4 = dcat.view(B, R, H, W)
             dwc = K.conv2d_wgrad(dcat4, x, 1, 1, 0, prec, alpha=s_inv)
             dbc = K.channel_sum(dcat4) if any(has_bias) else None
@@ -576,7 +573,7 @@
     return att
 
 
-def _cam_backward(att, x, gamma_c, d_cam, dx, prec=L.PREC_FP32):
+def _cam_backward(att, x, gamma_c, d_cam, dx, prec=L.PREC_FP32, fused=False, d_pam=None):
     B, Cn, H, W = x.shape
     N = H * W
     x3 = x.view(B, Cn, N)
@@ -587,6 +584,13 @@
     dgamma_c = K.dot(att, da)
     de = K.softmax_rows_bwd(att, da, -1.0)
     sym = K.add_transpose(de)
+    if fused:
+        res, res2 = (d_cam, None) if d_pam is None else (d_pam, d_cam)
+        K.conv_nn(B=B, M=Cn, Ck=Cn, ks=1, stride=1, pad=0, transposed=False, Hi=1, Wi=N, Ho=1, Wo=N, a=att,
+                  a_bs=Cn * Cn, a_sm=1, a_sc=Cn, a_st=0, x=d_cam, x_bs=d_bs, a2=sym, a2_bs=Cn * Cn, a2_sm=Cn, a2_sc=1,
+                  Ck2=Cn, x2=x3, x2_bs=Cn * N, y=dx, y_bs=Cn * N, precision=prec, alpha=gamma_c, res=res,
+                  res_bs=K._bview(res), res2=res2, res2_bs=0 if res2 is None else K._bview(res2))
+        return dgamma_c
     K.conv_nn(B=B, M=Cn, Ck=Cn, ks=1, stride=1, pad=0, transposed=False, Hi=1, Wi=N, Ho=1, Wo=N, a=att,
               a_bs=Cn * Cn, a_sm=1, a_sc=Cn, a_st=0, x=d_cam, x_bs=d_bs, y=dx, y_bs=Cn * N,
               precision=prec, alpha=gamma_c, accumulate=True)
@@ -637,8 +641,11 @@
         B, Cn, H, W = x.shape
         d3 = _as3(_c(dout))
         dx = torch.empty(B, Cn, H * W, device=x.device, dtype=torch.float32)
-        K.copy_slab(d3, dx)
-        dg = _cam_backward(att, x, gamma_c, d3, dx, ctx.prec)
+        if ATTN_BWD_FUSED:
+            dg = _cam_backward(att, x, gamma_c, d3, dx, ctx.prec, fused=True)
+        else:
+            K.copy_slab(d3, dx)
+            dg = _cam_backward(att, x, gamma_c, d3, dx, ctx.prec)
         return dx.view(B, Cn, H, W), dg
 
 
@@ -664,9 +671,12 @@
         dfeat = _c(dfeat)
         d_pam, d_cam = _as3(dfeat[:, :Cn]), _as3(dfeat[:, Cn:])
         dx = torch.empty(B, Cn, H * W, device=x.device, dtype=torch.float32)
-        K.copy_slab(d_pam, dx)
-        K.copy_slab(d_cam, dx, accumulate=True)
-        dgc = _cam_backward(att, x, gamma_c, d_cam, dx, cprec)
+        if ATTN_BWD_FUSED:
+            dgc = _cam_backward(att, x, gamma_c, d_cam, dx, cprec, fused=True, d_pam=d_pam)
+        else:
+            K.copy_slab(d_pam, dx)
+            K.copy_slab(d_cam, dx, accumulate=True)
+            dgc = _cam_backward(att, x, gamma_c, d_cam, dx, cprec)
         dwq, dbq, dwk, dbk, dwv, dbv, dgp = _pam_backward(route, saved, x, wq, wk, wv, gamma_p, d_pam, dx, prec, has_bias)
         return dx.view(B, Cn, H, W), dwq, dbq, dwk, dbk, dwv, dbv, dgp, dgc
 
diff --git a/include/gandanet.h b/include/gandanet.h
--- a/include/gandanet.h
+++ b/include/gandanet.h
@@ -42,6 +42,9 @@
     int act; int accumulate;
     int precision;
     int sub_oy, sub_ox, sub_step;
+    const float* a2; long a2_bs, a2_sm, a2_sc; int Ck2;
+    const float* x2; long x2_bs;
+    const float* res2; long res2_bs;
 } gd_conv_desc;
 int gd_conv2d(const gd_conv_desc* d, void* stream);
 
@@ -212,6 +215,10 @@
 int gd_chan_maxmean_bwd(const float* dy, const int* idx, float* dx, int B, int C, long HW, void* stream);
 int gd_chan_dot(const float* a, long a_bs, const float* o, long o_bs, int B, int C, int N, const float* gamma,
                 float* d_raw, float* delta, void* stream);
+int gd_cat_rows3(const float* s0, int n0, int lo0, const float* s1, int n1, int lo1, const float* s2, int n2, int lo2,
+                 float* dst, int R, int Cc, void* stream);
+int gd_chan_dot_pack(const float* a, long a_bs, const float* o, long o_bs, int B, int C, int N, const float* gamma,
+                     float* d_raw, float* delta, void* tr, int Npad, int ldt, void* stream);
 int gd_pack_16_split(const float* s, long s_bs, int B, int R, int Cc, const float* row_scale, const float* row_shift, int relu,
                      void* plain, long p_bs, int ldp, long p_cs, int p_ncopy, int p_pattern, void* tr, long t_bs, int ldt,
                      long t_cs, int t_ncopy, int t_pattern, void* stream);
```

Result: no change. 38.65 samples/s, median of 6 (+0.4%).
